# tranorrepository/cluster_tools

Measured on AMD Instinct MI355X. Metric: Gvoxels/s RAG+edge features (boundary map, uint64 labels, float32), higher is better.
Workload: dtype u64 labels / f32 samples / f64 stats; 1 GPU; BASELINE configs[2]: 2048^3 boundary map, cell 16, z-slab sharded; edges=15831246, parallelism=z-slab x1, step=rag_features

## Files before the change

cluster_tools_amd/_lib.py:

```python
from __future__ import annotations

import ctypes
import os
import sys
import threading

_HERE = os.path.dirname(os.path.abspath(__file__))
LIB_PATH = os.environ.get('CTG_LIB') or os.path.join(_HERE, 'libctg.so')

CTG_OK = 0
CTG_MEM_HOST = 0
CTG_MEM_DEVICE = 1
CTG_DATA_NONE = 0
CTG_DATA_F32 = 1
CTG_DATA_U8 = 2
CTG_KEEP_STATS = 1
CTG_NO_ADJ_FILTER = 2
CTG_NO_NODES = 4
CTG_DEFER_STATS = 8
CTG_ERR_STALE = -5
CTG_ERR_MISSING = -6
CTG_ASSIGN_DENSE = 0
CTG_ASSIGN_SPARSE = 1
CTG_CC_GREATER = 0
CTG_CC_LESS = 1
CTG_CC_EQUAL = 2
CTG_EDT_SRC_NONZERO = 0
CTG_EDT_SRC_GREATER = 1
CTG_EDT_SRC_EQUAL = 2
CTG_EDT_TO_BACKGROUND = 1
CTG_EDT_2D = 2
CTG_EDT_OUT_D2 = 4
CTG_WS_2D = 1
CTG_MAX_CHANNELS = 24
CTG_N_FEATURES = 10
CTG_NBINS = 40
CTG_WIDE_RECORD_WORDS = 48
CTG_MORPH_COLS = 11
CTG_REGION_COLS = 5
CTG_REGION_SUMS = 0
CTG_REGION_FEATURES = 1
CTG_MGPU_SAMPLES = 1024
CTG_MGPU_ROW_WORDS = 28
CTG_MGPU_MAX_WORLD = 32
CTG_IO_N5 = 0
CTG_IO_ZARR_DOT = 1
CTG_IO_ZARR_SLASH = 2
CTG_IO_RAW = 0
CTG_IO_GZIP = 1
CTG_IO_ZLIB = 2
CTG_SORT_WORDS = 12
CTG_SORT_PATH_GROUP = 5

_lock = threading.Lock()
_lib = None

c_i64p = ctypes.POINTER(ctypes.c_int64)
c_i32p = ctypes.POINTER(ctypes.c_int32)
c_u64p = ctypes.POINTER(ctypes.c_uint64)
c_u32p = ctypes.POINTER(ctypes.c_uint32)
c_dblp = ctypes.POINTER(ctypes.c_double)
c_vp = ctypes.c_void_p

PROTOTYPES = {
    'ctg_version': (ctypes.c_int, []),
    'ctg_init': (ctypes.c_int, [ctypes.c_int]),
    'ctg_last_error': (ctypes.c_char_p, []),
    'ctg_device_count': (ctypes.c_int, [ctypes.POINTER(ctypes.c_int)]),
    'ctg_rag_features': (ctypes.c_int, [c_vp, ctypes.c_int, c_vp, ctypes.c_int, ctypes.c_int, c_vp,
                                        c_vp, c_vp, c_vp, ctypes.c_int, ctypes.c_double, ctypes.c_double,
                                        ctypes.c_int, ctypes.c_int, c_vp, ctypes.POINTER(c_vp)]),
    'ctg_rag_blocks': (ctypes.c_int, [c_vp, ctypes.c_int, c_vp, ctypes.c_int, ctypes.c_int, c_vp, c_vp,
                                      ctypes.c_int, ctypes.c_int64, ctypes.c_int64, ctypes.c_int, ctypes.c_double,
                                      ctypes.c_double, ctypes.c_int, ctypes.c_int, c_vp, ctypes.POINTER(c_vp)]),
    'ctg_result_num_blocks': (ctypes.c_int, [c_vp]),
    'ctg_result_block_offsets': (ctypes.c_int, [c_vp, c_vp, c_vp]),
    'ctg_host_alloc': (c_vp, [ctypes.c_int64]),
    'ctg_host_free': (None, [c_vp]),
    'ctg_unique_labels': (ctypes.c_int, [c_vp, c_vp, c_vp, c_vp, ctypes.c_int, c_vp, ctypes.POINTER(c_vp)]),
    'ctg_merge_stats': (ctypes.c_int, [c_vp, c_vp, c_vp, ctypes.c_int64, ctypes.c_double, ctypes.c_double,
                                       ctypes.c_int, ctypes.c_int, c_vp, ctypes.POINTER(c_vp)]),
    'ctg_mgpu_slab': (ctypes.c_int, [ctypes.c_int64, ctypes.c_int, ctypes.c_int, c_vp, ctypes.c_int, c_vp]),
    'ctg_mgpu_sample': (ctypes.c_int, [c_vp, c_vp, c_vp]),
    'ctg_mgpu_split': (ctypes.c_int, [c_vp, c_vp, ctypes.c_int, c_vp, c_vp]),
    'ctg_mgpu_pack': (ctypes.c_int, [c_vp, c_vp, ctypes.c_int, ctypes.c_int, c_vp, c_vp]),
    'ctg_mgpu_merge': (ctypes.c_int, [c_vp, c_vp, c_vp, ctypes.c_int, ctypes.c_int, ctypes.c_double,
                                      ctypes.c_double, c_vp, ctypes.POINTER(c_vp)]),
    'ctg_merge_feature_rows': (ctypes.c_int, [c_vp, c_vp, ctypes.c_int64, ctypes.c_int64, ctypes.c_int64, c_vp,
                                              ctypes.c_int, c_vp]),
    'ctg_unique_pairs': (ctypes.c_int, [c_vp, ctypes.c_int64, ctypes.c_int, c_vp, ctypes.POINTER(c_vp)]),
    'ctg_unique_values': (ctypes.c_int, [c_vp, ctypes.c_int64, ctypes.c_int, c_vp, ctypes.POINTER(c_vp)]),
    'ctg_label_overlaps': (ctypes.c_int, [c_vp, ctypes.c_int, c_vp, ctypes.c_int, c_vp, c_vp, c_vp, ctypes.c_int,
                                          ctypes.c_uint64, ctypes.c_int, c_vp, ctypes.POINTER(c_vp)]),
    'ctg_merge_overlaps': (ctypes.c_int, [c_vp, c_vp, ctypes.c_int64, ctypes.c_int, c_vp, ctypes.POINTER(c_vp)]),
    'ctg_max_overlaps': (ctypes.c_int, [c_vp, ctypes.c_uint64, ctypes.c_uint64, c_vp, c_vp, ctypes.c_int, c_vp]),
    'ctg_result_copy_counts': (ctypes.c_int, [c_vp, c_vp, ctypes.c_int]),
    'ctg_morphology': (ctypes.c_int, [c_vp, ctypes.c_int, c_vp, c_vp, c_vp, c_vp, ctypes.c_int, c_vp,
                                      ctypes.POINTER(c_vp)]),
    'ctg_merge_morphology': (ctypes.c_int, [c_vp, ctypes.c_int64, ctypes.c_int, c_vp, ctypes.POINTER(c_vp)]),
    'ctg_result_copy_moments': (ctypes.c_int, [c_vp, c_vp, ctypes.c_int]),
    'ctg_morphology_rows': (ctypes.c_int, [c_vp, ctypes.c_uint64, ctypes.c_uint64, c_vp, c_vp, ctypes.c_int, c_vp]),
    'ctg_region_features': (ctypes.c_int, [c_vp, ctypes.c_int, c_vp, ctypes.c_int, c_vp, c_vp, c_vp, ctypes.c_int,
                                           ctypes.c_uint64, ctypes.c_int, c_vp, ctypes.POINTER(c_vp)]),
    'ctg_merge_region_features': (ctypes.c_int, [c_vp, ctypes.c_int64, ctypes.c_int, c_vp, ctypes.POINTER(c_vp)]),
    'ctg_region_rows': (ctypes.c_int, [c_vp, ctypes.c_uint64, ctypes.c_uint64, ctypes.c_int, ctypes.c_double, c_vp,
                                       c_vp, ctypes.c_int, c_vp]),
    'ctg_result_copy_region': (ctypes.c_int, [c_vp, c_vp, c_vp, c_vp, ctypes.c_int]),
    'ctg_assignment_dense': (ctypes.c_int, [c_vp, ctypes.c_int64, ctypes.c_int, c_vp, ctypes.POINTER(c_vp)]),
    'ctg_assignment_sparse': (ctypes.c_int, [c_vp, c_vp, ctypes.c_int64, ctypes.c_int, c_vp, ctypes.POINTER(c_vp)]),
    'ctg_assignment_info': (ctypes.c_int, [c_vp, c_i64p, c_u64p, ctypes.POINTER(ctypes.c_int)]),
    'ctg_assignment_free': (None, [c_vp]),
    'ctg_apply_assignment': (ctypes.c_int, [c_vp, c_vp, ctypes.c_int, ctypes.c_int64, c_vp, c_vp, ctypes.c_int64,
                                            ctypes.c_int, c_vp, c_vp, c_vp, ctypes.c_int, c_vp]),
    'ctg_threshold_components': (ctypes.c_int, [c_vp, ctypes.c_int, c_vp, c_vp, c_vp, c_vp, ctypes.c_float,
                                                ctypes.c_int, ctypes.c_int, ctypes.c_int, c_vp, ctypes.c_int, c_vp,
                                                c_u64p]),
    'ctg_merge_assignments': (ctypes.c_int, [c_vp, ctypes.c_int64, ctypes.c_uint64, c_vp, ctypes.c_int, c_vp, c_u64p]),
    'ctg_distance_transform': (ctypes.c_int, [c_vp, ctypes.c_int, ctypes.c_int, c_vp, c_vp, c_vp, ctypes.c_double,
                                              ctypes.c_uint64, c_vp, ctypes.c_int, c_vp, ctypes.c_int, c_vp, c_vp]),
    'ctg_seeded_watershed': (ctypes.c_int, [c_vp, c_vp, ctypes.c_int, c_vp, c_vp, c_vp, ctypes.c_int, ctypes.c_uint64,
                                            c_vp, ctypes.c_int, c_vp, c_vp]),
    'ctg_map_edge_ids': (ctypes.c_int, [c_vp, ctypes.c_int64, c_vp, ctypes.c_int64, c_vp, ctypes.c_int, c_vp]),
    'ctg_result_num_edges': (ctypes.c_int64, [c_vp]),
    'ctg_result_num_nodes': (ctypes.c_int64, [c_vp]),
    'ctg_result_copy_edges': (ctypes.c_int, [c_vp, c_vp, ctypes.c_int]),
    'ctg_result_copy_nodes': (ctypes.c_int, [c_vp, c_vp, ctypes.c_int]),
    'ctg_result_copy_features': (ctypes.c_int, [c_vp, c_vp, ctypes.c_int]),
    'ctg_result_copy_stats': (ctypes.c_int, [c_vp, c_vp, c_vp, ctypes.c_int]),
    'ctg_result_device_edges': (c_vp, [c_vp]),
    'ctg_result_device_features': (c_vp, [c_vp]),
    'ctg_result_info': (ctypes.c_int, [c_vp, c_i64p, c_i64p]),
    'ctg_free': (None, [c_vp]),
    'ctg_synth_volume': (ctypes.c_int, [c_vp, c_vp, c_vp, ctypes.c_int64, c_vp, ctypes.c_int, ctypes.c_uint64,
                                        ctypes.c_uint64, ctypes.c_double, c_vp]),
    'ctg_synth_affinities': (ctypes.c_int, [c_vp, c_vp, c_vp, ctypes.c_int, c_vp, c_vp]),
    'ctg_filter_conv_axis': (ctypes.c_int, [c_vp, c_vp, c_vp, ctypes.c_int, ctypes.c_int, c_vp, ctypes.c_int, c_vp]),
    'ctg_filter_combine': (ctypes.c_int, [ctypes.c_int, c_vp, c_vp, c_vp, c_vp, ctypes.c_int64, c_vp]),
    'ctg_sym_eigenvalues': (ctypes.c_int, [c_vp, ctypes.c_int, ctypes.c_int64, c_vp, c_vp]),
    'ctg_trim': (ctypes.c_int, []),
    'ctg_io_read_box': (ctypes.c_int, [ctypes.c_char_p, ctypes.c_int, ctypes.c_int, ctypes.c_int, ctypes.c_int,
                                       c_vp, c_vp, ctypes.c_int, c_vp, c_vp, c_vp, ctypes.c_int, c_vp]),
    'ctg_io_read_varlen': (ctypes.c_int, [ctypes.c_char_p, ctypes.c_int, ctypes.c_int, ctypes.c_int64, c_vp,
                                          ctypes.c_int, c_vp, c_vp, ctypes.c_int]),
    'ctg_io_free': (None, [c_vp]),
    'ctg_io_cache_clear': (None, []),
    'ctg_io_cache_stats': (None, [ctypes.c_void_p]),
    'ctg_io_cache_drop': (None, [ctypes.c_char_p]),
    'ctg_io_write_chunks': (ctypes.c_int, [ctypes.c_char_p, ctypes.c_int, ctypes.c_int, ctypes.c_int, ctypes.c_int,
                                           ctypes.c_int64, c_vp, c_vp, c_vp, c_vp, ctypes.c_int, ctypes.c_int,
                                           ctypes.c_int, ctypes.c_int]),
    'ctg_set_profiling': (ctypes.c_int, [ctypes.c_int]),
    'ctg_last_timings': (ctypes.c_int, [c_dblp, ctypes.c_int]),
    'ctg_last_sort': (ctypes.c_int, [c_i64p, ctypes.c_int]),
    'ctg_diag_bounds': (ctypes.c_int, [c_vp]),
}


class BlockDesc(ctypes.Structure):
    _fields_ = [('label_offset', ctypes.c_int64), ('data_offset', ctypes.c_int64),
                ('shape', ctypes.c_int64 * 3), ('own_begin', ctypes.c_int64 * 3), ('own_end', ctypes.c_int64 * 3),
                ('graph_begin', ctypes.c_int64 * 3), ('graph_end', ctypes.c_int64 * 3)]


class CtgError(RuntimeError):
    """Raised for every non-zero ctg status (pybind11 raises RuntimeError for
    nifty's C++ exceptions; cluster_tasks.py:114-159 treats both as a failed
    job)."""


def load():
    global _lib
    with _lock:
        if _lib is not None:
            return _lib
        if not os.path.exists(LIB_PATH):
            raise CtgError(
                "libctg.so not found at %s: build it with `python -c 'import __graft_entry__ as g; g.build()'` "
                "or `make -C cluster_tools_amd/csrc` (the HIP path has no CPU fallback)" % LIB_PATH)
        lib = ctypes.CDLL(LIB_PATH)
        for name, (res, args) in PROTOTYPES.items():
            if os.environ.get('CTG_LIB') and not hasattr(lib, name):
                continue
            fn = getattr(lib, name)
            fn.restype = res
            fn.argtypes = args
        _lib = lib
        return lib


def check(rc, what=''):
    if rc != CTG_OK:
        msg = load().ctg_last_error()
        msg = msg.decode() if msg else 'unknown error'
        raise CtgError('%s failed (status %d): %s' % (what or 'ctg call', rc, msg))


_inited = set()


def init_device(device=None):
    lib = load()
    if device is None:
        torch = sys.modules.get('torch')
        if torch is not None and torch.cuda.is_initialized():
            device = torch.cuda.current_device()
        else:
            device = int(os.environ.get('CTG_DEVICE', '0'))
    check(lib.ctg_init(int(device)), 'ctg_init(%d)' % device)
    _inited.add(int(device))
    return int(device)
```

cluster_tools_amd/csrc/ctg_api.hip:

```cpp
#include <hip/hip_runtime.h>
#include <cstdlib>
#include <cstring>
#include <rocprim/device/device_radix_sort.hpp>
#include <rocprim/device/device_select.hpp>

#include <algorithm>
#include <cstdio>

#include "ctg_api.h"

namespace ctg {

static thread_local std::string g_err;
void set_error(const std::string& msg) { g_err = msg; }

ResultPtr new_result(int device) {
    ResultPtr r(new ctg_result());
    r->device = device;
    return r;
}

ResultPtr empty_result(int device) {
    ResultPtr r = new_result(device);
    r->edges = (uint64_t*)dev_alloc(16);
// ... 42 lines not shown
    DevBuf<uint64_t> sorted(std::max<int64_t>(n, 1) * 8);
    if (!sorted) return hipErrorOutOfMemory;
    hipError_t e = with_temp(w.temp, [&](void* t, size_t& tb) {
        return rocprim::radix_sort_keys(t, tb, in, (uint64_t*)sorted, (size_t)n, 0u, end_bit, s);
    });
    if (e != hipSuccess) return e;
    return with_temp(w.temp, [&](void* t, size_t& tb) {
        return rocprim::unique(t, tb, (uint64_t*)sorted, out, count_dev, (size_t)n, rocprim::equal_to<uint64_t>(), s);
    });
}

int read_word(Workspace& w, SmallSlot i, hipStream_t s, int64_t* v) {
    CTG_CHECK(hipMemcpyAsync(w.small_host + i, w.small + i, 4, hipMemcpyDeviceToHost, s));
    CTG_CHECK(hipStreamSynchronize(s));
    *v = w.small_host[i];
    return CTG_OK;
}

int read_phase_times(Workspace& w, hipStream_t s) {
    CTG_CHECK(hipStreamSynchronize(s));
    float ms = 0.f;
    for (int i = 0; i < 6; ++i) {
        hipEventElapsedTime(&ms, w.ev[i], w.ev[i + 1]);
        w.last_ms[i] = ms;
    }
    hipEventElapsedTime(&ms, w.ev[0], w.ev[6]);
    w.last_ms[6] = ms;
    return CTG_OK;
}

hipError_t map_back(const ctg_result* U, ctg_result* r, hipStream_t s) {
    hipError_t e = launch_gather_labels(U->nodes, r->edges, 2 * r->n_edges, s);
    if (e == hipSuccess) e = launch_gather_labels(U->nodes, r->nodes, r->n_nodes, s);
    return e;
}

}

using namespace ctg;

static int reduce_pairs(ApiCall& c, ReduceJob& J, const uint64_t* dk, const char* who, ctg_result** out) {
    Workspace& w = c.w();
    hipStream_t s = c.s;
    DensePairs dp;
    StreamWait wait{s};
    CTG_CHECK(hipMemsetAsync(w.counters, 0, sizeof(Counters), s));
    CTG_CHECK(launch_max_pairs(J.n, dk, &w.counters->max_v, s));
    CTG_CHECK(hipMemcpyAsync(w.counters_host, w.counters, sizeof(Counters), hipMemcpyDeviceToHost, s));
    CTG_CHECK(hipStreamSynchronize(s));
    J.pairs = dk;
    J.max_v = w.counters_host->max_v;
    if (J.max_v >> 32) {
        const int rc = dp.build(dk, J.n, s);
        if (rc) return rc;
        J.pairs = dp.dense;
        J.max_v = (uint64_t)std::max<int64_t>(dp.U->n_nodes - 1, 0);
    }
    c.r = new_result(c.dev);
    hipError_t e = reduce_records(w, J, s, c.r.get());
    if (e == hipSuccess) e = dp.map_back(c.r.get(), s);
    if (e == hipSuccess) e = hipStreamSynchronize(s);
    const int rc = hip_status(e, who, CTG_ERR_HIP);
    if (rc) return rc;
    wait.disarm();
    return c.end(false, out);
}

extern "C" {

int ctg_version(void) { return 1; }

const char* ctg_last_error(void) { return g_err.c_str(); }

int ctg_device_count(int* count) {
    CTG_CHECK(hipGetDeviceCount(count));
    return CTG_OK;
}

int ctg_init(int device) {
    int n = 0;
    std::lock_guard<std::recursive_mutex> init_lock(device_mutex(device));
    CTG_CHECK(hipGetDeviceCount(&n));
    if (device < 0 || device >= n) {
        set_error("ctg_init: invalid device " + std::to_string(device));
        return CTG_ERR_ARG;
    }
    CTG_CHECK(hipSetDevice(device));
    CTG_CHECK(ws_init(ws(device)));
    return CTG_OK;
}

int ctg_diag_bounds(uint64_t* out) {
#ifdef CTG_DIAG
    if (!out) return CTG_ERR_ARG;
    CTG_CHECK(hipDeviceSynchronize());
    hipError_t (*take[8])(unsigned long long*) = {bounds_take_api,    bounds_take_scan, bounds_take_sort,
                                                   bounds_take_reduce, bounds_take_mgpu, bounds_take_overlap,
                                                   bounds_take_morph,  bounds_take_region};
    out[0] = out[1] = out[2] = out[3] = 0;
    int found = 0;
    for (int f = 0; f < 8; ++f) {
        unsigned long long h[3] = {0, 0, 0};
        CTG_CHECK(take[f](h));
        if (h[0] && !found) {
            out[0] = (uint64_t)f + 1;
            out[1] = h[0];
            out[2] = h[1];
            out[3] = h[2];
            found = 1;
        }
    }
    return found;
#else
    (void)out;
    set_error("ctg_diag_bounds: bounds checks exist only in CTG_DIAG builds (make variant EXTRA=-DCTG_DIAG)");
    return CTG_ERR_UNSUPPORTED;
#endif
}

int ctg_set_profiling(int on) {
    ws(current_device()).profiling = on;
    return CTG_OK;
}

int ctg_last_timings(double* ms, int n) {
    Workspace& w = ws(current_device());
    for (int i = 0; i < n && i < 8; ++i) ms[i] = w.last_ms[i];
    return CTG_OK;
}

int ctg_last_sort(int64_t* out, int n) {
    if (!out || n < 0) {
        set_error("ctg_last_sort: null argument");
        return CTG_ERR_ARG;
    }
    const SortReport& r = ws(current_device()).last_sort;
    int64_t v[CTG_SORT_WORDS];
    v[CTG_SORT_PATH] = r.path;
    v[CTG_SORT_PACKED] = r.packed;
    v[CTG_SORT_GROUP_TRIED] = r.group_tried;
    v[CTG_SORT_GROUP_DONE] = r.group_done;
    v[CTG_SORT_GROUP_WHY] = r.group_tried && !r.group_done ? (int)r.group.why : 0;
    v[CTG_SORT_GROUP_SHIFT] = r.group.shift;
    v[CTG_SORT_GROUP_BUCKETS] = r.group.nbk;
    v[CTG_SORT_GROUP_LARGEST] = r.largest;
    v[CTG_SORT_IB] = r.ib;
    v[CTG_SORT_NB] = r.nb;
    v[CTG_SORT_UB] = r.ub;
    v[CTG_SORT_N] = r.n;
    for (int i = 0; i < n && i < CTG_SORT_WORDS; ++i) out[i] = v[i];
    return CTG_OK;
}

int ctg_result_num_blocks(const ctg_result* r) { return r ? (int)std::max<size_t>(r->edge_off.size(), 1) - 1 : -1; }

int ctg_result_block_offsets(const ctg_result* r, int64_t* edge_off, int64_t* node_off) {
    if (!r || r->edge_off.empty()) {
        set_error("ctg_result_block_offsets: not a batched-blocks result");
        return CTG_ERR_ARG;
    }
    const size_t nb = r->edge_off.size();
    if (edge_off) std::memcpy(edge_off, r->edge_off.data(), nb * 8);
    if (node_off) {
        if (r->node_off.size() == nb) std::memcpy(node_off, r->node_off.data(), nb * 8);
        else std::memset(node_off, 0, nb * 8);
    }
    return CTG_OK;
}

int ctg_unique_labels(const uint64_t* labels, const int64_t* shape, const int64_t* begin, const int64_t* end,
                      int mem, void* stream, ctg_result** out) {
    ApiCall c;
    if (!labels || !shape || !out) {
        set_error("ctg_unique_labels: null argument");
        return CTG_ERR_ARG;
    }
    *out = nullptr;
    CallBox box;
    int rc = box_of("ctg_unique_labels", shape, begin, end, 0, &box);
    if (rc || (rc = c.begin(stream)) != CTG_OK) return rc;
    Workspace& w = c.w();
    hipStream_t s = c.s;
    const int64_t V = shape[0] * shape[1] * shape[2];
    const void* dl = nullptr;
    if ((rc = stage_in(w.stage[0], labels, (size_t)V * 8, mem, s, &dl)) != CTG_OK) return rc;
    if (box.voxels == 0) return c.empty(empty_result, out);
    c.r = new_result(c.dev);
    DevBuf<uint64_t> nodes;
    rc = unique_candidates(
        w, candidate_cap_first(box.voxels), box.voxels, 64u, s, "ctg_unique_labels: out of device memory",
        "ctg_unique_labels: candidate buffer overflow",
        [&](uint64_t* cand, unsigned long long* count, int64_t cap) {
            return launch_unique_tiles((const uint64_t*)dl, shape, box.b, box.e, cand, count, cap, s);
        },
        nodes, &c.r->n_nodes);
    if (rc) return rc;
    c.r->nodes = nodes.release();
    c.r->edges = (uint64_t*)dev_alloc(16);
    return c.end(false, out);
}

int ctg_unique_values(const uint64_t* values, int64_t n, int mem, void* stream, ctg_result** out) {
    ApiCall c;
    if (!out || n < 0 || (n > 0 && !values)) {
        set_error("ctg_unique_values: bad arguments");
        return CTG_ERR_ARG;
    }
    *out = nullptr;
    int rc = c.begin(stream);
    if (rc) return rc;
    if (n == 0) return c.empty(empty_result, out);
    Workspace& w = c.w();
    hipStream_t s = c.s;
    ResultPtr& r = c.r = new_result(c.dev);
    r->edges = (uint64_t*)dev_alloc(16);
    r->nodes = (uint64_t*)dev_alloc(n * 8);
    if (!r->nodes) {
        set_error("ctg_unique_values: out of device memory");
        return CTG_ERR_NOMEM;
    }
    DevInput<uint64_t> in;
    StreamWait wait{s};
    if ((rc = in.put(values, (size_t)n * 8, mem, s, "ctg_unique_values")) != CTG_OK) return rc;
    CTG_CHECK(sort_unique_u64(w, in, n, r->nodes, w.small + SLOT_NODES, s));
    if ((rc = read_word(w, SLOT_NODES, s, &r->n_nodes)) != CTG_OK) return rc;
    wait.disarm();
    return c.end(false, out);
}

int ctg_merge_stats(const uint64_t* keys, const double* sums, const uint32_t* records, int64_t n, double hist_lo,
                    double hist_hi, int keep_stats, int mem, void* stream, ctg_result** out) {
    ApiCall c;
    if (!out || n < 0 || (n > 0 && (!keys || !sums || !records))) {
        set_error("ctg_merge_stats: bad arguments");
        return CTG_ERR_ARG;
    }
    *out = nullptr;
    int rc = c.begin(stream);
    if (rc) return rc;
    if (n == 0) return c.empty(empty_result, out);
    hipStream_t s = c.s;
    DevInput<uint64_t> dk;
    DevInput<double> ds;
    DevInput<uint32_t> dr;
    StreamWait wait{s};
    rc = dk.put(keys, (size_t)n * 16, mem, s, "ctg_merge_stats");
    if (!rc) rc = ds.put(sums, (size_t)n * 16, mem, s, "ctg_merge_stats");
    if (!rc) rc = dr.put(records, (size_t)n * WREC_WORDS * 4, mem, s, "ctg_merge_stats");
    if (rc) return rc;
    ReduceJob J{};
    J.n = n;
    J.R.key = nullptr;
    J.R.sums = (double2*)ds.p;
    J.R.hist = (uint32_t*)dr.p;
    J.R.cap = n;
    J.wide = 1;
    J.stats = 1;
    J.need_adj = 1;
    J.ignore_label = 0;
    J.keep_stats = keep_stats;
    J.scale = (double)NBINS / (hist_hi - hist_lo);
    J.offset = hist_lo;
    if ((rc = reduce_pairs(c, J, dk, "ctg_merge_stats", out)) == CTG_OK) wait.disarm();
    return rc;
}

int ctg_merge_feature_rows(const uint64_t* ids, const double* rows, int64_t n, int64_t id_begin, int64_t id_end,
                           double* out, int mem, void* stream) {
    ApiCall c;
    if (n < 0 || id_end < id_begin || (n > 0 && (!ids || !rows)) || (id_end > id_begin && !out)) {
        set_error("ctg_merge_feature_rows: bad arguments");
        return CTG_ERR_ARG;
    }
    if (id_end - id_begin > 0xFFFFFFFFll || n > 0xFFFFFFFFll) {
        set_error("ctg_merge_feature_rows: more than 2^32 edges or rows in one call");
        return CTG_ERR_UNSUPPORTED;
    }
    const int64_t E = id_end - id_begin;
    if (E == 0) return CTG_OK;
    int rc = c.begin(stream);
    if (rc) return rc;
    Workspace& w = c.w();
    hipStream_t s = c.s;
    const bool host = mem == CTG_MEM_HOST;
    DevInput<uint64_t> di;
    DevInput<double> dr;
    DevBuf<double> own_o;
    StreamWait wait{s};
    double* dout = out;
    rc = di.put(ids, (size_t)n * 8, mem, s, "ctg_merge_feature_rows");
    if (!rc) rc = dr.put(rows, (size_t)n * N_FEATURES * 8, mem, s, "ctg_merge_feature_rows");
    if (rc) return rc;
    if (host && !(dout = own_o.alloc(E * N_FEATURES * 8))) {
        set_error("ctg_merge_feature_rows: out of device memory");
        return CTG_ERR_NOMEM;
    }
    CTG_CHECK(hipMemsetAsync(dout, 0, E * N_FEATURES * 8, s));
    if (n) {
        DevBuf<uint32_t> k_in(n * 4), k_out(n * 4), i_in(n * 4), i_out(n * 4);
        if (!k_in || !k_out || !i_in || !i_out) {
            set_error("ctg_merge_feature_rows: out of device memory");
            return CTG_ERR_NOMEM;
        }
        CTG_CHECK(hipMemsetAsync(w.small + SLOT_BAD_ID, 0, 4, s));
        CTG_CHECK(launch_row_keys(n, di, (uint64_t)id_begin, (uint64_t)id_end, k_in, i_in, w.small + SLOT_BAD_ID, s));
        const unsigned kb = (unsigned)bits_for((uint64_t)std::max<int64_t>(E - 1, 1));
// ... 198 lines not shown
```

cluster_tools_amd/csrc/ctg_api_scan.hip:

```cpp
#include <hip/hip_runtime.h>
#include <cstdio>
#include <cstdlib>
#include <cstring>

#include "ctg_api.h"

using namespace ctg;

struct ScanSwitches {
    int tile_z = 0;
    bool rec_fresh = false;
    int tile_z_narrow = 0;
    bool tail_tiles = true;
    int narrow_rows = -1;
    bool skip_adj = true;
    bool nn3 = true;
    int ablate = 0;
};

static ScanSwitches scan_switches(bool whole_array, bool boundary_map) {
    ScanSwitches sw;
    if (const char* t = getenv("CTG_TILE_Z")) sw.tile_z = std::max(1, atoi(t));
    sw.rec_fresh = getenv("CTG_REC_FRESH") != nullptr;
    if (!whole_array) return sw;
    if (const char* t = getenv("CTG_TILE_Z_NARROW")) sw.tile_z_narrow = std::max(1, atoi(t));
    if (const char* t = getenv("CTG_TAIL_TILES")) sw.tail_tiles = t[0] != '0';
    if (boundary_map)
        if (const char* t = getenv("CTG_NARROW_ROWS")) sw.narrow_rows = atoi(t) ? 1 : 0;
    if (const char* t = getenv("CTG_SKIP_ADJ")) sw.skip_adj = atoi(t) != 0;
    if (const char* t = getenv("CTG_NN3")) sw.nn3 = t[0] != '0';
#ifdef CTG_DIAG
    if (const char* t = getenv("CTG_ABLATE")) sw.ablate = atoi(t);
#endif
    return sw;
}

static int stage_volumes(Workspace& w, const void* labels, size_t lbytes, const void* data, size_t dbytes, int mem,
                         hipStream_t s, const void** dl, const void** dd) {
    const int rc = stage_in(w.stage[0], labels, lbytes, mem, s, dl);
    return rc ? rc : stage_in(w.stage[1], data, dbytes, mem, s, dd);
}

static ChannelClass scan_common(ScanParams& P, const void* dl, const void* dd, int label_bits, int data_kind,
                                int n_channels, const int32_t* offsets, double hist_lo, double hist_hi) {
    std::memset(&P, 0, sizeof(P));
    P.labels = dl;
    P.data = dd;
    P.label_bits = label_bits;
    P.data_kind = dd ? data_kind : CTG_DATA_NONE;
    P.n_channels = dd ? n_channels : 0;
    for (int c = 0; c < P.n_channels; ++c)
        for (int k = 0; k < 3; ++k) P.offsets[c][k] = offsets[3 * c + k];
    const ChannelClass cc = classify_channels(P.offsets, P.n_channels);
    P.lr_mask = cc.lr_mask;
    P.scale = (double)NBINS / (hist_hi - hist_lo);
    P.offset = hist_lo;
    P.fast40 = (hist_lo == 0.0 && P.scale == 40.0) ? 1 : 0;
    P.check_planes = 8;
    P.xcd_remap = 1;
    return cc;
}

static int scan_records(Workspace& w, const ScanParams& P, int64_t V, hipStream_t s, const ScanSwitches& sw, Ev& ev,
                        RegionPrefix& pre, bool* overflow, const char* who) {
    *overflow = false;
    if (sw.rec_fresh) {
        CTG_CHECK(hipStreamSynchronize(s));
        free_records(w);
    }
    int64_t need = record_slots_first(w.rec.cap, V);
#ifdef CTG_DIAG
    static const char* wg_path = getenv("CTG_WG_TIMES");
    ScanParams PW = P;
    size_t wg_n = 0;
    if (wg_path && !P.blocks) {
        const int64_t rows = std::min(scan_tile_rows(), scan_tile_rows_narrow());
        const int64_t tz = std::max(1, std::min(std::min(P.tile_z, P.tile_z_narrow > 0 ? P.tile_z_narrow : P.tile_z),
                                                std::max(8, P.tile_z / 4)));
        wg_n = (size_t)((P.shape[2] + 63) / 64) * (size_t)((P.shape[1] + rows - 1) / rows) *
               (size_t)((P.shape[0] + tz - 1) / tz);
        CTG_CHECK(hipMalloc(&PW.wg_times, wg_n * 16));
        CTG_CHECK(hipMemsetAsync(PW.wg_times, 0, wg_n * 16, s));
    }
#else
    const ScanParams& PW = P;
#endif
    for (int attempt = 0; attempt < 4; ++attempt) {
        CTG_CHECK(ensure_records(w, need, 0));
        CTG_CHECK(hipMemsetAsync(w.counters, 0, sizeof(Counters), s));
        ev.mark(0);
        CTG_CHECK(launch_face_scan(PW, w.rec, w.counters, s));
        ev.mark(1);
        CTG_CHECK(hipMemcpyAsync(w.counters_host, w.counters, sizeof(Counters), hipMemcpyDeviceToHost, s));
        CTG_CHECK(hipStreamSynchronize(s));
        if (w.counters_host->label_overflow) {
            *overflow = true;
            return CTG_OK;
        }
        const RegionFold f = fold_regions(w.counters_host->rcount);
        pre = f.pre;
        w.counters_host->n_records = f.total;
        if (f.total >= (1ull << 32)) {
            set_error(std::string(who) + ": more than 2^32 records");
            return CTG_ERR_NOMEM;
        }
        if ((int64_t)f.fullest <= w.rec.rcap) break;
        need = record_slots_regrow(f.fullest);
        if (attempt == 3) {
            set_error(std::string(who) + ": record buffer overflow");
            return CTG_ERR_NOMEM;
        }
    }
    if (P.ablate & 256)
        fprintf(stderr, "stamps total %llu fold %llu flush %llu wait %llu drain %llu floor %llu\n",
                w.counters_host->pad[2], w.counters_host->pad[3], w.counters_host->pad[4], w.counters_host->pad[5],
                w.counters_host->pad[7], w.counters_host->pad[0]);
#ifdef CTG_DIAG
    if (PW.wg_times) {
        std::vector<unsigned long long> h(wg_n * 2);
        CTG_CHECK(hipMemcpy(h.data(), PW.wg_times, wg_n * 16, hipMemcpyDeviceToHost));
        CTG_CHECK(hipFree(PW.wg_times));
        if (FILE* f = fopen(wg_path, "wb")) {
            fwrite(h.data(), 16, wg_n, f);
            fclose(f);
        }
        fprintf(stderr, "wg_times %s: %zu slots, flushes %llu, records %llu\n", wg_path, wg_n,
                w.counters_host->pad[6], w.counters_host->n_records);
    }
#endif
    w.last_records = (int64_t)w.counters_host->n_records;
    w.last_direct = (int64_t)w.counters_host->n_direct;
    return CTG_OK;
}

static ReduceJob scan_job(const Workspace& w, const ScanParams& P, const RegionPrefix& pre, bool scanned,
                          int ignore_label, int flags, ctg_result* r) {
    ReduceJob J{};
    J.n = r->n_records = scanned ? (int64_t)w.counters_host->n_records : 0;
    r->n_direct = scanned ? (int64_t)w.counters_host->n_direct : 0;
    J.keys = w.rec.key;
    J.regions = &pre;
    J.R = w.rec;
    J.stats = P.data_kind != CTG_DATA_NONE;
    J.ignore_label = ignore_label;
    J.keep_stats = (flags & CTG_KEEP_STATS) ? 1 : 0;
    J.max_v = scanned ? w.counters_host->max_v : 0;
    J.scale = P.scale;
    J.offset = P.offset;
    return J;
}

static int keep_zero_first(ctg_result* U, hipStream_t s) {
    uint64_t first = 0;
    if (U->n_nodes > 0) {
        CTG_CHECK(hipMemcpyAsync(&first, U->nodes, 8, hipMemcpyDeviceToHost, s));
        CTG_CHECK(hipStreamSynchronize(s));
    }
    if (U->n_nodes > 0 && first == 0) return CTG_OK;
    DevBuf<uint64_t> t((size_t)(U->n_nodes + 1) * 8);
    if (!t) {
        set_error("out of device memory for the dense relabelling table");
        return CTG_ERR_NOMEM;
    }
    CTG_CHECK(hipMemsetAsync(t, 0, 8, s));
    if (U->n_nodes)
        CTG_CHECK(hipMemcpyAsync(t + 1, U->nodes, (size_t)U->n_nodes * 8, hipMemcpyDeviceToDevice, s));
    dev_free(U->nodes);
    U->nodes = t.release();
    U->n_nodes += 1;
    return CTG_OK;
}

template <class Rerun>
static int rag_dense_relabel(const uint64_t* l64, int64_t n, const int64_t* shape, int ignore_label, int64_t limit,
                             const char* who, const char* limit_msg, void* stream, Rerun&& rerun, ctg_result** out) {
    hipStream_t s = (hipStream_t)stream;
    ResultPtr U, r;
    int rc = nested(U, [&](ctg_result** u) {
        return shape ? ctg_unique_labels(l64, shape, nullptr, nullptr, CTG_MEM_DEVICE, stream, u)
                     : ctg_unique_values(l64, n, CTG_MEM_DEVICE, stream, u);
    });
    if (rc) return rc;
    if (ignore_label && (rc = keep_zero_first(U.get(), s)) != CTG_OK) return rc;
    if (U->n_nodes > limit) {
        set_error(std::string(who) + limit_msg);
        return CTG_ERR_UNSUPPORTED;
    }
    DevBuf<uint32_t> dense(std::max<int64_t>(n, 1) * 4);
    if (!dense) {
        set_error(std::string(who) + ": out of device memory for the dense relabelling");
        return CTG_ERR_NOMEM;
    }
    CTG_CHECK(launch_remap_dense(l64, n, U->nodes, U->n_nodes, dense, s));
    rc = nested(r, [&](ctg_result** rr) { return rerun((const uint32_t*)dense, rr); });
    dense.reset();
    if (rc) return rc;
    CTG_CHECK(map_back(U.get(), r.get(), s));
    CTG_CHECK(hipStreamSynchronize(s));
    *out = r.release();
    return CTG_OK;
}

static int validate_features(const void* labels, int label_bits, const void* data, int data_kind, int n_channels,
                             const int32_t* offsets, const int64_t* shape, const int64_t* own_begin,
                             const int64_t* own_end, double hist_lo, double hist_hi, ctg_result** out) {
    const char* bad = nullptr;
    if (!out || !shape || !labels) {
        set_error("ctg_rag_features: null argument");
        return CTG_ERR_ARG;
    }
    *out = nullptr;
    if (label_bits != 32 && label_bits != 64) bad = "label_bits must be 32 or 64";
    else if (n_channels < 0 || n_channels > CTG_MAX_CHANNELS || (n_channels > 0 && !offsets))
        bad = "bad channel/offset arguments";
    else if (data && data_kind != CTG_DATA_F32 && data_kind != CTG_DATA_U8)
        bad = "data_kind must be CTG_DATA_F32 or CTG_DATA_U8";
    else if (!(hist_hi > hist_lo)) bad = "hist_hi must be > hist_lo";
    else
        for (int k = 0; k < 3; ++k)
            if (shape[k] < 0 || (own_begin && (own_begin[k] < 0)) || (own_end && own_end[k] < 0))
                bad = "negative shape/own_begin/own_end";
    if (!bad) return CTG_OK;
    set_error(std::string("ctg_rag_features: ") + bad);
    return CTG_ERR_ARG;
}

static void plan_whole_tiles(ScanParams& P, const int64_t* shape, const int64_t* own_begin, const int64_t* own_end,
                             const ScanSwitches& sw) {
    for (int k = 0; k < 3; ++k) {
        P.shape[k] = shape[k];
        P.own_begin[k] = own_begin ? own_begin[k] : 0;
        P.own_end[k] = own_end ? std::min(own_end[k], shape[k]) : shape[k];
    }
    const TileDepths td = scan_tile_depths(shape, scan_tile_rows(), scan_tile_rows_narrow());
    P.tile_z = td.tile_z;
    P.tile_z_narrow = td.tile_z_narrow;
    if (sw.tile_z) P.tile_z_narrow = P.tile_z = sw.tile_z;
    if (sw.tile_z_narrow) P.tile_z_narrow = sw.tile_z_narrow;
    P.ablate = sw.ablate;
    P.tail_tiles = sw.tail_tiles;
}

static int density_probe(Workspace& w, ScanParams& P, int mode, hipStream_t s) {
    P.narrow_rows = mode;
    if (mode != 2) return CTG_OK;
    P.density = w.small + SLOT_DENSITY;
    CTG_CHECK(hipMemsetAsync(w.small + SLOT_DENSITY, 0, 2 * sizeof(uint32_t), s));
    CTG_CHECK(launch_density(P.labels, P.label_bits, P.shape, 512, w.small + SLOT_DENSITY, s));
    return CTG_OK;
}

struct AdjFilter {
    hipStream_t s;
    ResultPtr graph;
    DevBuf<unsigned long long> bloom;
    StreamWait wait{s, false};
};

static int adjacency_filter(ScanParams& P, const int64_t* shape, const int64_t* own_begin, const int64_t* own_end,
                            double hist_lo, double hist_hi, void* stream, AdjFilter& f) {
    hipStream_t s = f.s;
    int rc = nested(f.graph, [&](ctg_result** g) {
        return ctg_rag_features(P.labels, P.label_bits, nullptr, CTG_DATA_NONE, 0, nullptr, shape, own_begin, own_end, 0,
                                hist_lo, hist_hi, 0, CTG_MEM_DEVICE, stream, g);
    });
    if (rc) return rc;
    const ctg_result* g = f.graph.get();
    uint64_t mx = 0;
    if (g->n_edges > 0) {
        CTG_CHECK(hipMemcpyAsync(&mx, g->nodes + g->n_nodes - 1, 8, hipMemcpyDeviceToHost, s));
        CTG_CHECK(hipStreamSynchronize(s));
    }
    if (mx >> 32) return CTG_OK;
    const uint32_t blocks = bloom_blocks(g->n_edges);
    if (!f.bloom.alloc((size_t)blocks * 64)) {
        set_error("ctg_rag_features: out of memory (adjacency filter)");
        return CTG_ERR_NOMEM;
    }
    f.wait.arm();
    if ((rc = hip_status(launch_build_bloom(g->edges, g->n_edges, f.bloom, blocks - 1, s), "ctg_rag_features",
                         CTG_ERR_HIP)) != CTG_OK)
        return rc;
    P.bloom = f.bloom;
    P.bloom_mask = blocks - 1;
    return CTG_OK;
}

static void plan_scan_channels(ScanParams& P, const ChannelClass& cc, int flags, const ScanSwitches& sw) {
    const ChannelPlan cp = plan_channels(cc, P.n_channels, !(flags & CTG_NO_ADJ_FILTER), P.bloom != nullptr,
                                         sw.skip_adj, sw.nn3);
    P.skip_adj_marks = cp.skip_adj_marks;
    P.nn3 = cp.nn3;
    P.nn_mix = cp.nn_mix;
    if (cp.nn3 || cp.nn_mix)
        for (int a = 0; a < 3; ++a) P.nn_ch[a] = cc.nn_ch[a];
    if (cp.nn_mix) {
        P.n_loop = cc.n_loop;
        for (int i = 0; i < cc.n_loop; ++i) P.loop_ch[i] = cc.loop_ch[i];
    }
}

static int64_t single_label_index(const ScanParams& P) {
    for (int k = 0; k < 3; ++k)
        if (P.own_begin[k] >= P.own_end[k]) return -1;
    return (P.own_begin[0] * P.shape[1] + P.own_begin[1]) * P.shape[2] + P.own_begin[2];
}
static hipError_t widen_single_label(const ScanParams& P, int64_t at, hipStream_t s, ctg_result* r) {
    if (P.label_bits != 32 || r->n_records != 0 || at < 0) return hipSuccess;
    uint32_t l32 = 0;
    hipError_t e = hipMemcpyAsync(&l32, (const uint32_t*)P.labels + at, 4, hipMemcpyDeviceToHost, s);
    if (e == hipSuccess) e = hipStreamSynchronize(s);
    const uint64_t l64 = l32;
    if (e == hipSuccess) e = hipMemcpyAsync(r->nodes, &l64, 8, hipMemcpyHostToDevice, s);
    if (e == hipSuccess) e = hipStreamSynchronize(s);
    r->n_nodes = 1;
    return e;
}

static int block_plan_error(const BlockPlan& plan) {
    const std::string block = "ctg_rag_blocks: block " + std::to_string(plan.bad_block);
    if (plan.error == BlockPlan::BOX_OUTSIDE) set_error(block + ": box outside its array");
    else if (plan.error == BlockPlan::ARRAY_OUTSIDE) set_error(block + ": array outside the arena");
    else set_error("ctg_rag_blocks: too many tiles in one call");
    return CTG_ERR_ARG;
}

struct BlockTables {
    hipStream_t s;
    DevBuf<BlockGeom> geom;
    DevBuf<uint32_t> prefix;
    StreamWait wait{s};
};

static int upload_block_tables(const BlockPlan& plan, int n_blocks, hipStream_t s, BlockTables& t, ScanParams& P) {
    P.tile_z = plan.tile_z;
    P.tag_shift = plan.tag_shift;
    P.label_hi_mask = plan.label_hi_mask;
    P.n_blocks = n_blocks;
    P.batch_tiles = plan.prefix[n_blocks];
    t.geom.alloc(sizeof(BlockGeom) * n_blocks);
    t.prefix.alloc((n_blocks + 1) * 4);
    if (!t.geom || !t.prefix) {
        set_error("ctg_rag_blocks: out of device memory");
        return CTG_ERR_NOMEM;
    }
    CTG_CHECK(hipMemcpyAsync(t.geom, plan.geom.data(), sizeof(BlockGeom) * n_blocks, hipMemcpyHostToDevice, s));
    CTG_CHECK(hipMemcpyAsync(t.prefix, plan.prefix.data(), (n_blocks + 1) * 4, hipMemcpyHostToDevice, s));
    P.blocks = t.geom;
    P.tile_prefix = t.prefix;
    return CTG_OK;
}

static hipError_t block_edge_offsets(const ScanParams& P, int tag_bits, uint64_t umask, hipStream_t s, ctg_result* r) {
    const int n_blocks = P.n_blocks;
    r->edge_off.assign(n_blocks + 1, 0);
    r->edge_off[n_blocks] = r->n_edges;
    if (!tag_bits || !r->n_edges) return hipSuccess;
    DevBuf<int64_t> bounds((n_blocks + 1) * 8);
    if (!bounds) return hipErrorOutOfMemory;
    CTG_TRY(launch_block_bounds(r->n_edges, r->edges, 2, n_blocks, P.tag_shift, bounds, s));
    CTG_TRY(hipMemcpyAsync(r->edge_off.data(), bounds, (n_blocks + 1) * 8, hipMemcpyDeviceToHost, s));
    CTG_TRY(launch_clear_bits(r->n_edges, r->edges, 2, umask, s));
    return hipStreamSynchronize(s);
}

static int block_nodes(Workspace& w, const ScanParams& P, const BlockPlan& plan, hipStream_t s, ctg_result* r) {
    const int n_blocks = P.n_blocks;
    const int64_t n_tiles = plan.uprefix.back();
    const char* nomem = "ctg_rag_blocks: out of device memory for the block nodes";
    DevBuf<uint32_t> dprefix((n_blocks + 1) * 4);
    DevBuf<int64_t> bounds((n_blocks + 1) * 8);
    if (!dprefix || !bounds) {
        set_error(nomem);
        return CTG_ERR_NOMEM;
    }
    CTG_CHECK(hipMemcpyAsync(dprefix, plan.uprefix.data(), (n_blocks + 1) * 4, hipMemcpyHostToDevice, s));
    DevBuf<uint64_t> nodes;
    int64_t N = 0;
    const int rc = unique_candidates(
        w, candidate_cap_first(plan.own_voxels), INT64_MAX, 32u + (unsigned)plan.tag_bits, s, nomem,
        "ctg_rag_blocks: node candidate buffer overflow",
        [&](uint64_t* cand, unsigned long long* count, int64_t cap) {
            return launch_unique_blocks(P.labels, P.label_bits, P.blocks, dprefix, n_blocks, n_tiles, cand, count, cap, s);
        },
        nodes, &N);
    if (rc) return rc;
    CTG_CHECK(launch_block_bounds(N, nodes, 1, n_blocks, 32, bounds, s));
    r->node_off.assign(n_blocks + 1, 0);
    CTG_CHECK(hipMemcpyAsync(r->node_off.data(), bounds, (n_blocks + 1) * 8, hipMemcpyDeviceToHost, s));
    CTG_CHECK(launch_clear_bits(N, nodes, 1, 0xFFFFFFFFull, s));
    CTG_CHECK(hipStreamSynchronize(s));
    dev_free(r->nodes);
    r->nodes = nodes.release();
    r->n_nodes = N;
    return CTG_OK;
}

static int features_dense_reentry(const void* dl, int label_bits, const void* dd, int data_kind, int n_channels,
                                  const int32_t* offsets, const int64_t* shape, const int64_t* own_begin,
                                  const int64_t* own_end, int ignore_label, double hist_lo, double hist_hi, int flags,
                                  void* stream, ctg_result** out) {
    if (label_bits != 64) {
        set_error("ctg_rag_features: internal label overflow on 32-bit labels");
        return CTG_ERR_HIP;
    }
    const int64_t V = shape[0] * shape[1] * shape[2];
    return rag_dense_relabel(
        (const uint64_t*)dl, V, shape, ignore_label, 0xFFFFFFFFll, "ctg_rag_features",
        ": more than 2^32 distinct labels in one array", stream,
        [&](const uint32_t* dense, ctg_result** r) {
            return ctg_rag_features(dense, 32, dd, data_kind, n_channels, offsets, shape, own_begin, own_end,
                                    ignore_label, hist_lo, hist_hi, flags, CTG_MEM_DEVICE, stream, r);
        },
        out);
}

static int blocks_dense_reentry(const void* dl, int label_bits, const void* dd, int data_kind, int n_channels,
                                const int32_t* offsets, const ctg_block_desc* blocks, int n_blocks,
                                int64_t labels_len, int64_t data_len, int ignore_label, double hist_lo,
                                double hist_hi, int flags, int tag_shift, void* stream, ctg_result** out) {
    hipStream_t s = (hipStream_t)stream;
    const uint64_t* l64 = (const uint64_t*)dl;
    DevBuf<uint64_t> wide;
    if (label_bits == 32) {
        if (!wide.alloc(std::max<int64_t>(labels_len, 1) * 8)) {
            set_error("ctg_rag_blocks: out of device memory widening the labels");
            return CTG_ERR_NOMEM;
        }
        CTG_CHECK(launch_u32_to_u64(labels_len, (const uint32_t*)dl, wide, s));
        l64 = wide;
    }
    return rag_dense_relabel(
        l64, labels_len, nullptr, ignore_label, (int64_t)(1ull << tag_shift), "ctg_rag_blocks",
        ": too many distinct labels for one batch of blocks: call with fewer blocks", stream,
        [&](const uint32_t* dense, ctg_result** r) {
            const int rc = ctg_rag_blocks(dense, 32, dd, data_kind, n_channels, offsets, blocks, n_blocks, labels_len,
                                          data_len, ignore_label, hist_lo, hist_hi, flags, CTG_MEM_DEVICE, stream, r);
            wide.reset();
            return rc;
        },
        out);
}

extern "C" {

int ctg_rag_features(const void* labels, int label_bits, const void* data, int data_kind, int n_channels,
                     const int32_t* offsets, const int64_t* shape, const int64_t* own_begin,
                     const int64_t* own_end, int ignore_label,
                     double hist_lo, double hist_hi, int flags, int mem, void* stream, ctg_result** out) {
    const char* who = "ctg_rag_features";
    ApiCall c;
    int rc = validate_features(labels, label_bits, data, data_kind, n_channels, offsets, shape, own_begin, own_end,
                               hist_lo, hist_hi, out);
    if (rc || (rc = c.begin(stream)) != CTG_OK) return rc;
    Workspace& w = c.w();
    hipStream_t s = c.s;
    const int64_t V = shape[0] * shape[1] * shape[2];
    const size_t dbytes = data ? (size_t)V * (n_channels > 0 ? n_channels : 1) * (data_kind == CTG_DATA_U8 ? 1 : 4) : 0;
    const void *dl = nullptr, *dd = nullptr;
    if ((rc = stage_volumes(w, labels, (size_t)V * (label_bits / 8), data, dbytes, mem, s, &dl, &dd)) != CTG_OK) return rc;
    const bool boundary_map = data && n_channels == 0;
    const ScanSwitches sw = scan_switches(true, boundary_map);

    ScanParams P;
    const ChannelClass cc = scan_common(P, dl, dd, label_bits, data_kind, n_channels, offsets, hist_lo, hist_hi);
    plan_whole_tiles(P, shape, own_begin, own_end, sw);
    if ((rc = density_probe(w, P, narrow_rows_mode(boundary_map, V, sw.narrow_rows), s)) != CTG_OK) return rc;
    AdjFilter adj{s};
    if (cc.long_range && !(flags & CTG_NO_ADJ_FILTER) && V > 0 &&
        (rc = adjacency_filter(P, shape, own_begin, own_end, hist_lo, hist_hi, stream, adj)) != CTG_OK)
        return rc;
    plan_scan_channels(P, cc, flags, sw);

    Ev ev{w, s};
    ev.mark(0);
    if (V == 0) return c.empty(empty_result, out);
    RegionPrefix pre{};
    bool overflow = false;
    if ((rc = scan_records(w, P, V, s, sw, ev, pre, &overflow, who)) != CTG_OK) return rc;
    if (overflow)
        return features_dense_reentry(dl, label_bits, dd, data_kind, n_channels, offsets, shape, own_begin, own_end,
                                      ignore_label, hist_lo, hist_hi, flags, stream, out);
    c.r = new_result(c.dev);
    ReduceJob J = scan_job(w, P, pre, true, ignore_label, flags, c.r.get());
    J.need_adj = need_adj_whole(P.n_channels, P.skip_adj_marks, !(flags & CTG_NO_ADJ_FILTER), P.bloom != nullptr);
    J.defer_stats = (flags & CTG_DEFER_STATS) ? 1 : 0;
    J.min_u = w.counters_host->max_nu ? (uint64_t)(uint32_t)~(uint32_t)w.counters_host->max_nu : 0;
    const int64_t single = single_label_index(P);
    J.single_label_ptr = label_bits == 64 && single >= 0 ? (const uint64_t*)dl + single : nullptr;
    hipError_t e = reduce_records(w, J, s, c.r.get());
    if (e == hipSuccess) e = widen_single_label(P, single, s, c.r.get());
    if ((rc = hip_status(e, who, CTG_ERR_HIP)) != CTG_OK) return rc;
    c.r->partial_adj = J.need_adj == 2 ? 1 : 0;
    return c.end(true, out);
}

int ctg_rag_blocks(const void* labels, int label_bits, const void* data, int data_kind, int n_channels,
                   const int32_t* offsets, const ctg_block_desc* blocks, int n_blocks, int64_t labels_len,
                   int64_t data_len, int ignore_label, double hist_lo, double hist_hi, int flags, int mem,
                   void* stream, ctg_result** out) {
    const char* who = "ctg_rag_blocks";
    ApiCall c;
    if (!out || !labels || !blocks || n_blocks < 1 || n_blocks > (1 << 20) || labels_len < 0 ||
        (label_bits != 32 && label_bits != 64) || (data && data_kind != CTG_DATA_F32 && data_kind != CTG_DATA_U8) ||
        n_channels < 0 || n_channels > CTG_MAX_CHANNELS || (n_channels > 0 && !offsets) || !(hist_hi > hist_lo)) {
        set_error("ctg_rag_blocks: bad arguments");
        return CTG_ERR_ARG;
    }
    *out = nullptr;
    const ScanSwitches sw = scan_switches(false, false);
    const BlockPlan plan = plan_blocks(blocks, n_blocks, data != nullptr, n_channels, labels_len, data_len,
                                       scan_max_x(), scan_tile_rows(), unique_tile_y(), sw.tile_z);
    if (plan.error == BlockPlan::BOX_OUTSIDE || plan.error == BlockPlan::ARRAY_OUTSIDE) return block_plan_error(plan);
    int rc = c.begin(stream);
    if (rc) return rc;
    Workspace& w = c.w();
    hipStream_t s = c.s;
    const void *dl = nullptr, *dd = nullptr;
    if ((rc = stage_volumes(w, labels, (size_t)labels_len * (label_bits / 8), data,
                            data ? (size_t)data_len * (data_kind == CTG_DATA_U8 ? 1 : 4) : 0, mem, s, &dl, &dd)) != CTG_OK)
        return rc;
    if (plan.error != BlockPlan::OK) return block_plan_error(plan);

    ScanParams P;
    scan_common(P, dl, dd, label_bits, data_kind, n_channels, offsets, hist_lo, hist_hi);
    BlockTables tables{s};
    if ((rc = upload_block_tables(plan, n_blocks, s, tables, P)) != CTG_OK) return rc;

    Ev ev{w, s};
    ev.mark(0);
    RegionPrefix pre{};
    bool overflow = false;
    const bool scanned = P.batch_tiles > 0;
    if (scanned && (rc = scan_records(w, P, plan.voxels, s, sw, ev, pre, &overflow, who)) != CTG_OK) return rc;
    if (overflow)
        return blocks_dense_reentry(dl, label_bits, dd, data_kind, n_channels, offsets, blocks, n_blocks, labels_len,
                                    data_len, ignore_label, hist_lo, hist_hi, flags, P.tag_shift, stream, out);
    c.r = new_result(c.dev);
    ctg_result* r = c.r.get();
    ReduceJob J = scan_job(w, P, pre, scanned, ignore_label, flags, r);
    J.need_adj = need_adj_blocks(P.n_channels);
    J.ub = plan.tag_bits ? 32 : 0;
    J.umask = plan.tag_bits ? (1ull << P.tag_shift) - 1ull : ~0ull;
    J.skip_nodes = 1;
    hipError_t e = reduce_records(w, J, s, r);
    if (e == hipSuccess) e = block_edge_offsets(P, plan.tag_bits, J.umask, s, r);
    if ((rc = hip_status(e, who, CTG_ERR_HIP)) != CTG_OK) return rc;
    if (flags & CTG_NO_NODES) r->node_off.assign(n_blocks + 1, 0);
    else if ((rc = block_nodes(w, P, plan, s, r)) != CTG_OK) return rc;
    return c.end(scanned, out);
}

}
```

cluster_tools_amd/csrc/ctg_internal.h:

```cpp
#pragma once
#include <hip/hip_runtime.h>
#include <cstdint>
#include <cstddef>
#include <memory>
#include <atomic>
#include <mutex>
#include <string>
#include <utility>
#include <vector>

#include "../../include/ctg.h"
#include "ctg_buffers.h"
#include "ctg_plan.h"

namespace ctg {

#ifdef CTG_DIAG
static __device__ unsigned long long ctg_oob[4];
__device__ __forceinline__ void oob_note(unsigned long long* d, uint64_t i, uint64_t n, int line) {
    if (i >= n && atomicCAS(d, 0ull, (unsigned long long)line) == 0ull) {
        d[1] = i;
        d[2] = n;
    }
}
#define CTG_IDX(i, n) ::ctg::oob_note(::ctg::ctg_oob, (uint64_t)(i), (uint64_t)(n), __LINE__)
#define CTG_BOUNDS_TAKE(tag)                                                      \
    hipError_t bounds_take_##tag(unsigned long long* h) {                       \
        hipError_t e_ = hipMemcpyFromSymbol(h, HIP_SYMBOL(ctg_oob), 24);          \
        if (e_ != hipSuccess || h[0] == 0) return e_;                             \
        const unsigned long long z_[4] = {0, 0, 0, 0};                            \
        return hipMemcpyToSymbol(HIP_SYMBOL(ctg_oob), z_, 32);                    \
    }
#else
#define CTG_IDX(i, n) ((void)0)
#define CTG_BOUNDS_TAKE(tag)
#endif

constexpr int WAVE = 64;
#ifndef CTG_SCAN_THREADS
#define CTG_SCAN_THREADS 512
#endif
constexpr int SCAN_THREADS = CTG_SCAN_THREADS;
constexpr int TILE_Y = 8;
#ifndef CTG_TABLE_CAP
#define CTG_TABLE_CAP SCAN_THREADS
#endif
constexpr int TABLE_CAP = CTG_TABLE_CAP;
static_assert(TABLE_CAP % 4 == 0 && TABLE_CAP <= SCAN_THREADS, "table capacity");
constexpr int NBINS = 40;
constexpr int NSLOTS = NBINS + 2;
constexpr int HWORDS = 21;
constexpr int NREC_WORDS = 24;
constexpr int NREC_STRIDE = 32;
constexpr int NREC_OFF = 4;
constexpr int NREC_PIV = 28;
constexpr int WREC_WORDS = 48;
constexpr int WREC_PIV = 45;
constexpr uint32_t PIV_EMPTY = 0xFFFFFFFFu;
constexpr uint32_t ADJ_FLAG = 0x80000000u;
constexpr uint64_t EMPTY_KEY = ~0ull;
constexpr int N_FEATURES = 10;
constexpr int64_t RECORD_LIMIT = 0xFFFFFFFFll;

__host__ __device__ inline uint32_t f2ord(float f) {
    uint32_t b;
    __builtin_memcpy(&b, &f, 4);
    return (b & 0x80000000u) ? ~b : (b | 0x80000000u);
}
__host__ __device__ inline float ord2f(uint32_t o) {
    uint32_t b = (o & 0x80000000u) ? (o & 0x7FFFFFFFu) : ~o;
    float f;
    __builtin_memcpy(&f, &b, 4);
    return f;
}
constexpr uint32_t ORD_POS_INF = 0xFF800000u;
constexpr uint32_t ORD_NEG_INF = 0x007FFFFFu;

__host__ __device__ inline int hist_slot(double x, double scale, double offset) {
    double m = scale * (x - offset);
    if (m == (double)NBINS) return NBINS;
    if (!(m < (double)NBINS)) return (m != m) ? 0 : NBINS + 1;
    if (m <= -1.0) return 0;
    return (int)m + 1;
}

__host__ __device__ inline uint32_t hash_key(uint64_t k) {
    k ^= k >> 33;
    k *= 0xff51afd7ed558ccdull;
    k ^= k >> 33;
    return (uint32_t)k;
}

#ifdef __HIPCC__
__device__ __forceinline__ uint64_t shfl_up_u64(uint64_t v) {
    const uint32_t lo = __shfl_up((uint32_t)v, 1, WAVE), hi = __shfl_up((uint32_t)(v >> 32), 1, WAVE);
    return ((uint64_t)hi << 32) | lo;
}
__device__ __forceinline__ uint64_t shfl_down_u64(uint64_t v, int o) {
    const uint32_t lo = __shfl_down((uint32_t)v, o, WAVE), hi = __shfl_down((uint32_t)(v >> 32), o, WAVE);
    return ((uint64_t)hi << 32) | lo;
}
__device__ __forceinline__ uint64_t bcast0_u64(uint64_t v) {
    const uint32_t lo = __shfl((uint32_t)v, 0, WAVE), hi = __shfl((uint32_t)(v >> 32), 0, WAVE);
    return ((uint64_t)hi << 32) | lo;
}
#endif

__host__ __device__ inline uint64_t bloom_hash(uint64_t k) {
    k ^= k >> 33;
    k *= 0xff51afd7ed558ccdull;
    k ^= k >> 29;
    k *= 0xc4ceb9fe1a85ec53ull;
    return k ^ (k >> 32);
}
__host__ __device__ inline uint64_t bloom_bits(uint64_t h) {
    return (1ull << (h & 63)) | (1ull << ((h >> 6) & 63)) | (1ull << ((h >> 12) & 63)) | (1ull << ((h >> 18) & 63));
}
__host__ __device__ inline uint32_t bloom_block(uint32_t owner, uint32_t block_mask) {
    return ((uint32_t)(bloom_hash(owner) >> 24) & block_mask) * 8u;
}
__host__ __device__ inline uint32_t bloom_word(uint32_t block, uint64_t h) { return block + ((uint32_t)(h >> 40) & 7u); }

struct RecordBuf {
    uint64_t* key = nullptr;
    double2* sums = nullptr;
    uint32_t* hist = nullptr;
    int64_t cap = 0;
    int64_t rcap = 0;
};

struct ScanParams {
    const void* labels;
    const void* data;
    int label_bits;
    int data_kind;
    int n_channels;
    int offsets[CTG_MAX_CHANNELS][3];
    int64_t shape[3];
    int64_t own_begin[3];
    int64_t own_end[3];
    double scale, offset;
    double u8_scale;
    int tile_z;
    int tile_z_narrow;
    int check_planes;
    int fast40;
    int ablate;
    const unsigned long long* bloom;
    uint32_t bloom_mask;
    int64_t ntiles[3];
    int xcd_remap;
    int skip_adj_marks;
    int nn3;
    int nn_ch[3];
    int nn_mix;
    int n_loop;
    int loop_ch[CTG_MAX_CHANNELS];
    uint32_t lr_mask;
    int narrow_rows;
    const uint32_t* density;
    const BlockGeom* blocks;
    const uint32_t* tile_prefix;
    int n_blocks;
    int64_t batch_tiles;
    int tag_shift;
    uint32_t label_hi_mask;
    unsigned long long* wg_times;
    int tail_tiles;
    int64_t main_tiles;
    int tail_z0, tile_z_tail;
};

struct Counters {
    unsigned long long n_records;
    unsigned long long n_direct;
    unsigned long long label_overflow;
    unsigned long long max_v;
    unsigned long long max_nu;
    unsigned long long pad[8];
    unsigned long long rcount[NREG];
};

struct Perm {
    const uint32_t* p32;
    const uint64_t* p64;
    int ib;
    __device__ __forceinline__ uint32_t operator()(uint32_t r) const {
        return p64 ? (uint32_t)(p64[r] & ((1ull << ib) - 1ull)) : p32[r];
    }
};

struct DeferredStats {
    int on = 0;
    const uint32_t* offs = nullptr;
    const uint32_t* runs = nullptr;
    Perm perm{nullptr, nullptr, 0};
    const uint32_t* hist = nullptr;
    uint64_t gen = 0;
    int64_t n_runs = 0, n_rec = 0, rec_cap = 0;
};

struct ReduceOut {
    uint64_t* edges;
    double* feats;
    uint32_t* keep;
    uint32_t* wstats;
    double2* wsums;
    uint32_t* count_out;
    int ablate;
    int64_t n_rec;
};

constexpr int BK_SMALL_WORDS = 5 * 4096 + 16;
constexpr int GS_SMALL_WORDS = 5 * 65536 + 16;

enum SmallSlot : int {
    SLOT_RUNS = 0,
    SLOT_EDGES = 1,
    SLOT_NODES = 2,
    SLOT_BAD_ID = 3,
    SLOT_DENSITY = 4,
    SLOT_GROUP_SORT = 16,
    SLOT_MERGE = 20,
    SLOT_HEAVY = 40,
    SMALL_WORDS = 64
};
struct MergeCounts {
    uint32_t keys;
    uint32_t rows;
};
static_assert(SLOT_RUNS >= 0 && SLOT_RUNS + 1 <= SLOT_EDGES && SLOT_EDGES + 1 <= SLOT_NODES &&
                  SLOT_NODES + 1 <= SLOT_BAD_ID && SLOT_BAD_ID + 1 <= SLOT_DENSITY &&
                  SLOT_DENSITY + 2 <= SLOT_GROUP_SORT && SLOT_GROUP_SORT + 1 <= SLOT_MERGE &&
                  SLOT_MERGE + (int)(sizeof(MergeCounts) / 4) <= SLOT_HEAVY && SLOT_HEAVY + 1 <= SMALL_WORDS,
              "the scalar slots overlap or pass SMALL_WORDS");

struct Workspace {
    std::atomic<bool> ready{false};
    int device = -1;
    uint64_t gen = 1;
    RecordBuf rec;
    SortScratch sort;
    GrowBuf temp;
    Counters* counters = nullptr;
    Counters* counters_host = nullptr;
    unsigned int* small = nullptr;
    unsigned int* small_host = nullptr;
    uint32_t* bsort = nullptr;
    uint32_t* gsort = nullptr;
    uint64_t* mgpu_spl = nullptr;
    hipEvent_t mgpu_spl_ev = nullptr;
    GrowBuf stage[2];
    hipStream_t copy_stream = nullptr;
    hipEvent_t ev[7] = {};
    double last_ms[8] = {0};
    int64_t last_records = 0, last_direct = 0;
    SortReport last_sort;
    int profiling = 0;
};

Workspace& ws(int device);
hipError_t ws_init(Workspace& w);
int current_device();
void set_error(const std::string& msg);
void free_records(Workspace& w);
hipError_t ensure_records(Workspace& w, int64_t need, int wide);

std::recursive_mutex& device_mutex(int device);
struct DevLock {
    std::lock_guard<std::recursive_mutex> g;
    DevLock() : g(device_mutex(current_device())) {}
};

template <class F>
hipError_t with_temp(GrowBuf& temp, F&& call) {
    size_t bytes = 0;
    hipError_t e = call(nullptr, bytes);
    if (e != hipSuccess) return e;
    if (!temp.reserve(bytes + 256)) return hipErrorOutOfMemory;
    bytes = temp.bytes;
    return call(temp.p, bytes);
}

struct Ev {
    Workspace& w;
    hipStream_t s;
    void mark(int i) {
        if (w.profiling) hipEventRecord(w.ev[i], s);
    }
};

hipError_t launch_face_scan(const ScanParams& P, const RecordBuf& R, Counters* C, hipStream_t s);
int64_t scan_max_x();
int scan_tile_rows();
int scan_tile_rows_narrow();
hipError_t launch_density(const void* L, int label_bits, const int64_t* shape, int n_rows, uint32_t* out,
                          hipStream_t s);
hipError_t launch_unique_tiles(const uint64_t* L, const int64_t* shape, const int64_t* b, const int64_t* e,
                               uint64_t* out, unsigned long long* count, int64_t cap, hipStream_t s);
hipError_t launch_unique_blocks(const void* L, int label_bits, const BlockGeom* blocks, const uint32_t* tile_prefix,
                                int n_blocks, int64_t n_tiles, uint64_t* out, unsigned long long* count, int64_t cap,
                                hipStream_t s);
int unique_tile_y();
hipError_t bucket_sort_keys(const uint64_t* keys, uint64_t* tmp, uint64_t* out, int64_t n, int lo_bit, int hi_bit,
                            uint64_t kmin, uint64_t kmax, uint32_t* small, GrowBuf& temp, uint32_t* nbk_out,
                            hipStream_t s);
hipError_t bucket_runs(const uint64_t* sorted, int64_t n, int lo_bit, uint32_t nbk, uint32_t* small, uint64_t* uniq,
                       uint32_t* runs, uint32_t* roffs, uint32_t* dE, hipStream_t s);
hipError_t bucket_sort_pairs(const uint64_t* keys, const uint32_t* vals, uint64_t* ktmp, uint32_t* vtmp,
                             uint64_t* kout, uint32_t* vout, int64_t n, int hi_bit, uint32_t* small, GrowBuf& temp,
                             uint32_t* nbk_out, hipStream_t s);
hipError_t group_sort_runs(const uint64_t* key, int64_t rcap, const RegionPrefix& pre, int64_t n, int nb, int ub,
                           int ib, uint64_t min_label, uint64_t max_label, uint32_t* small, uint32_t* host_word,
                           uint64_t* items, uint32_t* perm, uint64_t* uniq, uint32_t* runs, uint32_t* roffs,
                           uint32_t* dE, bool* done, SortReport* rep, hipStream_t s);
hipError_t launch_pack_keys(int64_t n, const uint64_t* key, int nb, uint64_t* sk, uint32_t* idx, hipStream_t s);
hipError_t launch_pack_regions(const uint64_t* key, int64_t rcap, const RegionPrefix& pre, int nb, int ib, uint64_t* sk,
                               uint32_t* idx, hipStream_t s);
hipError_t launch_pack_pairs(int64_t n, const uint64_t* uv, int nb, uint64_t* sk, uint32_t* idx, hipStream_t s);
hipError_t launch_max_pairs(int64_t n, const uint64_t* uv, unsigned long long* out, hipStream_t s);
hipError_t launch_reduce(int64_t E, const uint32_t* dE, const uint64_t* uniq, const uint32_t* runs,
                         const uint32_t* offs, const uint32_t* perm32, const uint64_t* perm64, int ib,
                         const RecordBuf& R, int wide, int stats, int nb, uint64_t umask, int need_adj,
                         int ignore_label, double scale, double offset, const ReduceOut& O, hipStream_t s,
                         uint32_t* heavy = nullptr, uint32_t* n_heavy = nullptr);
hipError_t launch_block_bounds(int64_t n, const uint64_t* col, int stride, int n_blocks, int shift, int64_t* bounds,
                               hipStream_t s);
hipError_t launch_clear_bits(int64_t n, uint64_t* col, int stride, uint64_t mask, hipStream_t s);
hipError_t launch_compact(int64_t E, const uint32_t* dE, const uint32_t* keep, const uint32_t* pos,
                          const ReduceOut& in, const ReduceOut& out, uint32_t* dkept, hipStream_t s);
hipError_t launch_endpoints(int64_t E, const uint64_t* uniq, int nb, uint32_t* out, hipStream_t s);
hipError_t launch_u32_to_u64(int64_t n, const uint32_t* in, uint64_t* out, hipStream_t s);
hipError_t launch_mark_nodes(int64_t E, const uint32_t* dE, const uint64_t* uniq, int nb, uint32_t* bits,
                             int64_t W, uint32_t wbase, hipStream_t s);
hipError_t launch_bits_to_nodes(int64_t W, const uint32_t* bits, const uint32_t* off, uint64_t* nodes, uint32_t* dN,
                                int64_t cap, uint32_t wbase, hipStream_t s);
hipError_t launch_build_bloom(const uint64_t* edges, int64_t E, unsigned long long* words, uint32_t mask,
                              hipStream_t s);
hipError_t launch_find_edges(const uint64_t* ge, int64_t n, const uint64_t* q, int64_t m, int64_t* out,
                             hipStream_t s);
hipError_t launch_remap_dense(const uint64_t* L, int64_t V, const uint64_t* U, int64_t n, uint32_t* out,
                              hipStream_t s);
hipError_t launch_gather_labels(const uint64_t* U, uint64_t* x, int64_t n, hipStream_t s);
hipError_t launch_remap_dense64(const uint64_t* L, int64_t V, const uint64_t* U, int64_t n, uint64_t* out,
                                hipStream_t s);
hipError_t launch_row_keys(int64_t n, const uint64_t* ids, uint64_t begin, uint64_t end, uint32_t* key,
                           uint32_t* idx, uint32_t* bad, hipStream_t s);
hipError_t launch_merge_feature_rows(int64_t n, const uint32_t* key, const uint32_t* idx, const double* rows,
                                     double* out, hipStream_t s);
hipError_t launch_synth(uint64_t* labels, float* boundary, const int64_t* shape, int64_t z_offset,
                        const int64_t* gshape, int cell, uint64_t seed, uint64_t label_offset, double noise_amp,
                        hipStream_t s);
hipError_t launch_synth_aff(const float* b, float* out, const int64_t* shape, int n_channels, const int32_t* off,
                            hipStream_t s);
#ifdef CTG_DIAG
hipError_t bounds_take_api(unsigned long long* h);
hipError_t bounds_take_reduce(unsigned long long* h);
hipError_t bounds_take_sort(unsigned long long* h);
hipError_t bounds_take_mgpu(unsigned long long* h);
hipError_t bounds_take_scan(unsigned long long* h);
hipError_t bounds_take_overlap(unsigned long long* h);
hipError_t bounds_take_morph(unsigned long long* h);
hipError_t bounds_take_region(unsigned long long* h);
#endif

}

struct ctg_result {
    int device = -1;
    std::vector<int64_t> edge_off, node_off;
    int64_t n_edges = 0;
    int64_t n_nodes = 0;
    uint64_t* edges = nullptr;
    uint64_t* nodes = nullptr;
    double* features = nullptr;
    uint32_t* stats = nullptr;
    double2* stat_sums = nullptr;
    uint64_t* counts = nullptr;
    int64_t* row_off = nullptr;
    uint64_t* moments = nullptr;
    uint64_t* reg_count = nullptr;
    double* reg_sum = nullptr;
    float* reg_minmax = nullptr;
    int64_t n_records = 0;
    int64_t n_direct = 0;
    int partial_adj = 0;
    ctg::DeferredStats defer;
    std::vector<void*> owned;
};

struct ctg_assignment {
    int device = -1;
    int kind = CTG_ASSIGN_DENSE;
    int64_t n = 0;
    uint64_t max_value = 0;
    uint64_t* table = nullptr;
    uint64_t size = 0;
};

namespace ctg {

struct ResultFree {
    void operator()(ctg_result* r) const { ctg_free(r); }
};
using ResultPtr = std::unique_ptr<ctg_result, ResultFree>;
ResultPtr new_result(int device);
ResultPtr empty_result(int device);

struct ReduceJob {
    int64_t n;
    const uint64_t* keys;
    const uint64_t* pairs;
    RecordBuf R;
    int wide, stats, need_adj, ignore_label, keep_stats;
    uint64_t max_v;
    uint64_t min_u = 0;
    double scale, offset;
    const uint64_t* single_label_ptr;
    const RegionPrefix* regions;
    int ub = 0;
    uint64_t umask = ~0ull;
    int skip_nodes = 0;
    int defer_stats = 0;
};
hipError_t reduce_records(Workspace& w, const ReduceJob& J, hipStream_t s, ctg_result* res);

hipError_t overlap_tables(Workspace& w, const void* A, int abits, const void* B, int bbits, const int64_t* shape,
                          const int64_t* b, const int64_t* e, int with_ignore, uint64_t ignore, hipStream_t s,
                          ctg_result* r, unsigned* overflow);
hipError_t overlap_reduce(Workspace& w, const uint64_t* key, const uint64_t* cnt, int64_t n, hipStream_t s,
                          ctg_result* r);
template <typename ValueT>
hipError_t sort_and_number(Workspace& w, const uint64_t* key, const ValueT* val, int64_t n, unsigned end_bit,
                           hipStream_t s, uint64_t* ks, ValueT* vs, uint64_t* scan, uint64_t* last);
hipError_t launch_overlap_pack(int64_t n, const uint64_t* pairs, uint64_t* key, hipStream_t s);
hipError_t launch_overlap_map_back(int64_t E, uint64_t* pairs, const uint64_t* Ua, int64_t na, const uint64_t* Ub,
                                   int64_t nb, hipStream_t s);
hipError_t launch_overlap_find(const uint64_t* U, int64_t n, uint64_t x, uint32_t* out, hipStream_t s);
hipError_t launch_overlap_argmax(const ctg_result* r, uint64_t lb, uint64_t le, uint64_t* out_l, uint64_t* out_c,
                                 hipStream_t s);

constexpr int MORPH_WORDS = 10;
hipError_t morph_tables(Workspace& w, const void* A, int bits, const int64_t* shape, const int64_t* b,
                        const int64_t* e, const int64_t* origin, hipStream_t s, ctg_result* r, unsigned* overflow);
hipError_t morph_merge(Workspace& w, const double* rows, int64_t n, hipStream_t s, ctg_result* r, int* bad);
// ... 155 lines not shown
```

cluster_tools_amd/csrc/ctg_plan.h:

```cpp
#pragma once
#include <algorithm>
#include <cstdint>
#include <cstdlib>
#include <vector>

#include "../../include/ctg.h"

#ifndef CTG_HD
#ifdef __HIPCC__
#define CTG_HD __host__ __device__
#else
#define CTG_HD
#endif
#endif

namespace ctg {

constexpr int TILE_X = 64;

inline int bits_for(uint64_t v) {
    int b = 1;
    while (b < 64 && (v >> b)) ++b;
    return b;
}
inline int bits_u(int64_t v) { return v <= 0 ? 0 : bits_for((uint64_t)v); }

struct CallBox {
    enum Error { OK, OUTSIDE, TOO_LARGE } error;
    int64_t b[3], e[3];
    int64_t voxels;
};

inline CallBox call_box(const int64_t* shape, const int64_t* begin, const int64_t* end, int64_t max_voxels) {
    CallBox c{};
    for (int k = 0; k < 3; ++k) {
        c.b[k] = begin ? begin[k] : 0;
        c.e[k] = end ? end[k] : shape[k];
        if (shape[k] < 0 || c.b[k] < 0 || c.e[k] > shape[k] || c.b[k] > c.e[k]) {
            c.error = CallBox::OUTSIDE;
            return c;
        }
    }
    c.voxels = (c.e[0] - c.b[0]) * (c.e[1] - c.b[1]) * (c.e[2] - c.b[2]);
    c.error = max_voxels > 0 && c.voxels >= max_voxels ? CallBox::TOO_LARGE : CallBox::OK;
    return c;
}

struct VolBox {
    int64_t s_z, s_y;
    int64_t base;
    uint32_t n[3];
};

inline VolBox vol_box(const int64_t* shape, const CallBox& c) {
    VolBox v{};
    v.s_z = shape[1] * shape[2];
    v.s_y = shape[2];
    v.base = c.b[0] * v.s_z + c.b[1] * v.s_y + c.b[2];
    for (int k = 0; k < 3; ++k) v.n[k] = (uint32_t)(c.e[k] - c.b[k]);
    return v;
}

struct TileDepths {
    int tile_z;
    int tile_z_narrow;
};

inline TileDepths scan_tile_depths(const int64_t* shape, int64_t rows_wide, int64_t rows_narrow) {
    constexpr int NARROW_TILE_Z = 16;
    const int64_t cols = ((shape[2] + TILE_X - 1) / TILE_X) * ((shape[1] + rows_wide - 1) / rows_wide);
    int tz = cols * ((shape[0] + 63) / 64) >= 32768 ? 64 : 32;
    if (cols * ((shape[0] + 127) / 128) >= 6144) tz = 128;
    while (tz > 8 && cols * ((shape[0] + tz - 1) / tz) < 1024) tz /= 2;
    const int64_t cols_n = ((shape[2] + TILE_X - 1) / TILE_X) * ((shape[1] + rows_narrow - 1) / rows_narrow);
    int tzn = std::min(tz, NARROW_TILE_Z);
    while (tzn < tz && cols_n * ((shape[0] + tzn - 1) / tzn) > 65536) tzn *= 2;
    return {tz, tzn};
}

inline int narrow_rows_mode(bool boundary_map, int64_t V, int nr_switch) {
    if (!boundary_map || (V < (1ll << 28) && nr_switch < 0)) return 0;
    return nr_switch < 0 ? 2 : (nr_switch ? 1 : 0);
}

struct BlockGeom {
    int64_t label_offset;
    int64_t data_offset;
    int32_t shape[3];
    int32_t own_begin[3], own_end[3];
    int32_t graph_begin[3], graph_end[3];
    int32_t ntx, nty, ntz;
};

struct BlockPlan {
    enum Error { OK, BOX_OUTSIDE, ARRAY_OUTSIDE, TOO_MANY_TILES } error = OK;
    int bad_block = -1;
    int64_t own_voxels = 0, voxels = 0;
    int tile_z = 0;
    int tag_bits = 0, tag_shift = 32;
    uint32_t label_hi_mask = 0;
    std::vector<BlockGeom> geom;
    std::vector<uint32_t> prefix;
    std::vector<uint32_t> uprefix;
};

inline BlockPlan plan_blocks(const ctg_block_desc* blocks, int n_blocks, bool has_data, int n_channels,
                             int64_t labels_len, int64_t data_len, int64_t max_x, int scan_rows, int unique_rows,
                             int tile_z_switch) {
    BlockPlan p;
    const int nch = has_data ? std::max(1, n_channels) : 0;
    int64_t zmax = 1;
    for (int b = 0; b < n_blocks; ++b) {
        const ctg_block_desc& d = blocks[b];
        int64_t V = 1, ov = 1;
        p.bad_block = b;
        for (int k = 0; k < 3; ++k) {
            V *= d.shape[k];
            if (d.shape[k] < 0 || d.shape[k] > (k == 2 ? max_x : 0x7FFFFFFF) || d.own_begin[k] < 0 ||
                d.own_end[k] > d.shape[k] || d.graph_begin[k] < 0 || d.graph_end[k] > d.shape[k]) {
                p.error = BlockPlan::BOX_OUTSIDE;
                return p;
            }
        }
        if (d.label_offset < 0 || d.label_offset + V > labels_len ||
            (has_data && (d.data_offset < 0 || d.data_offset + V * nch > data_len))) {
            p.error = BlockPlan::ARRAY_OUTSIDE;
            return p;
        }
        for (int k = 0; k < 3; ++k) ov *= std::max<int64_t>(0, d.own_end[k] - d.own_begin[k]);
        p.own_voxels += ov;
        p.voxels += V;
        zmax = std::max(zmax, d.shape[0]);
    }
    p.bad_block = -1;
    p.tile_z = tile_z_switch > 0 ? tile_z_switch : (int)std::min<int64_t>(zmax, 128);
    p.tag_bits = bits_u(n_blocks - 1);
    p.tag_shift = 32 - p.tag_bits;
    p.label_hi_mask = p.tag_bits ? ~((1u << p.tag_shift) - 1u) : 0u;
    p.geom.resize(n_blocks);
    p.prefix.assign(n_blocks + 1, 0);
    p.uprefix.assign(n_blocks + 1, 0);
    for (int b = 0; b < n_blocks; ++b) {
        const ctg_block_desc& d = blocks[b];
        BlockGeom& g = p.geom[b];
        g.label_offset = d.label_offset;
        g.data_offset = has_data ? d.data_offset : 0;
        int64_t oe[3];
        for (int k = 0; k < 3; ++k) {
            g.shape[k] = (int32_t)d.shape[k];
            g.own_begin[k] = (int32_t)d.own_begin[k];
            g.own_end[k] = (int32_t)d.own_end[k];
            g.graph_begin[k] = (int32_t)d.graph_begin[k];
            g.graph_end[k] = (int32_t)d.graph_end[k];
            oe[k] = std::max<int64_t>(0, d.own_end[k] - d.own_begin[k]);
        }
        g.ntx = (int32_t)((d.shape[2] + TILE_X - 1) / TILE_X);
        g.nty = (int32_t)((d.shape[1] + scan_rows - 1) / scan_rows);
        g.ntz = (int32_t)((d.shape[0] + p.tile_z - 1) / p.tile_z);
        const int64_t nt = (int64_t)g.ntx * g.nty * g.ntz;
        const int64_t ut = ((oe[2] + 63) / 64) * ((oe[1] + unique_rows - 1) / unique_rows) * ((oe[0] + 15) / 16);
        if ((int64_t)p.prefix[b] + nt > 0x7FFFFFFFll || (int64_t)p.uprefix[b] + ut > 0x7FFFFFFFll) {
            p.error = BlockPlan::TOO_MANY_TILES;
            return p;
        }
        p.prefix[b + 1] = p.prefix[b] + (uint32_t)nt;
        p.uprefix[b + 1] = p.uprefix[b] + (uint32_t)ut;
    }
    return p;
}

constexpr int NREG = 64;

struct RegionPrefix {
    uint32_t off[NREG + 1];
};

inline int64_t record_slots_first(int64_t cap, int64_t V) {
    const int64_t need = std::max<int64_t>(cap, std::max<int64_t>(1 << 16, V / 24));
    return (need + NREG - 1) / NREG * NREG;
}
inline int64_t record_slots_regrow(uint64_t fullest) { return ((int64_t)(fullest * 5 / 4) + 1024) * NREG; }

struct RegionFold {
    RegionPrefix pre;
    uint64_t total, fullest;
};
inline RegionFold fold_regions(const unsigned long long* rcount) {
    RegionFold f{};
    for (int r = 0; r < NREG; ++r) {
        f.pre.off[r] = (uint32_t)f.total;
        f.total += rcount[r];
        f.fullest = std::max<uint64_t>(f.fullest, rcount[r]);
    }
    f.pre.off[NREG] = (uint32_t)f.total;
    return f;
}

inline int64_t candidate_cap_first(int64_t n) {
    return std::max<int64_t>(1, std::min<int64_t>(n, std::max<int64_t>(1 << 16, n / 8)));
}
inline int64_t candidate_cap_regrow(int64_t m, int64_t bound) { return std::min<int64_t>(bound, m + 1024); }

inline uint32_t bloom_blocks(int64_t n_edges) {
    const int64_t bits = n_edges * 48;
    uint32_t blocks = 128;
    while ((int64_t)blocks * 512 < bits) blocks *= 2;
    return blocks;
}

constexpr int64_t TAKE_CHUNK = 4096;

inline uint64_t take_capacity(int64_t n) {
    uint64_t cap = 64;
    while (cap < 2 * (uint64_t)std::max<int64_t>(n, 0)) cap *= 2;
    return cap;
}

inline int take_count_slots(int64_t n_seg) { return n_seg <= 4096 ? 64 : 1; }

struct TakeChunks {
    enum Error { OK, BAD_SEGMENTS, TOO_MANY_CHUNKS } error = OK;
    std::vector<uint32_t> prefix;
};

inline TakeChunks take_chunk_prefix(const int64_t* seg_begin, int64_t n_seg, int64_t n, int64_t chunk) {
    TakeChunks t;
    const int64_t whole[2] = {0, n};
    if (!seg_begin) {
        seg_begin = whole;
        n_seg = 1;
    }
    if (n_seg < 0 || n < 0 || (n_seg == 0 && n != 0) || (n_seg > 0 && (seg_begin[0] != 0 || seg_begin[n_seg] != n))) {
        t.error = TakeChunks::BAD_SEGMENTS;
        return t;
    }
    t.prefix.assign((size_t)n_seg + 1, 0);
// ... 392 lines not shown
```

cluster_tools_amd/csrc/ctg_scan.hip:

```cpp
#include <type_traits>

#include "ctg_stats.h"
#include "ctg_tile_table.h"

#ifndef CTG_ROWS
#define CTG_ROWS 4
#endif

namespace ctg {

enum { MODE_GRAPH = 0, MODE_BOUNDARY = 1, MODE_AFFINITY = 2, MODE_AFF_NN = 3, MODE_AFF_MIX = 4 };

constexpr bool raw_sites(int mode) { return mode != MODE_AFFINITY && mode != MODE_AFF_MIX; }

constexpr bool scalar_loads(int mode) { return raw_sites(mode); }
constexpr int64_t SCALAR_LOAD_SPAN = 0xFFFFFFFFll;

constexpr int ROWS_WIDE = CTG_ROWS;
#ifndef CTG_ROWS_NARROW
#define CTG_ROWS_NARROW 1
#endif
constexpr int ROWS_NARROW = CTG_ROWS_NARROW;
#ifndef CTG_AFF_ROWS
#define CTG_AFF_ROWS CTG_ROWS
// ... 495 lines not shown
#pragma unroll
    for (int i = 0; i < NPER; ++i) {
        mm[i] = make_uint2(ORD_POS_INF, ORD_NEG_INF);
        if (MODE != MODE_GRAPH && slot[i] >= 0)
            mm[i] = make_uint2(__hip_atomic_load(&T.w[slot[i]][22], __ATOMIC_RELAXED, __HIP_MEMORY_SCOPE_WORKGROUP),
                               __hip_atomic_load(&T.w[slot[i]][23], __ATOMIC_RELAXED, __HIP_MEMORY_SCOPE_WORKGROUP));
    }
#if CTG_PAIR_FOLD
    if constexpr ((MODE == MODE_BOUNDARY || MODE == MODE_AFF_NN) && !BATCH) {
        fold_grouped<MODE, FAST40, BATCH, StageT, NPER>(T, e, slot, pv, mm, lane, R, C, scale, offset, ablate);
        return;
    }
#endif
#pragma unroll
    for (int i = 0; i < NPER; ++i)
        if (slot[i] != -2)
            fold_stats<MODE, FAST40, BATCH, StageT>(T, e[i], slot[i], pv[i], mm[i], R, C, scale, offset, need,
                                                    ablate);
}

__device__ __forceinline__ uint64_t stamp_now() {
    uint64_t t;
    asm volatile("s_memtime %0\n\ts_waitcnt lgkmcnt(0)" : "=s"(t)::"memory");
    return t;
}

__device__ __forceinline__ uint32_t swap1(uint32_t v) {
    return (uint32_t)__builtin_amdgcn_update_dpp((int)v, (int)v, 0xB1, 0xf, 0xf, false);
}

__device__ __forceinline__ uint32_t shl1(uint32_t v, uint32_t edge) {
    return (uint32_t)__builtin_amdgcn_update_dpp((int)edge, (int)v, 0x130, 0xf, 0xf, false);
}

#define FLUSH_TABLE table_flush_waves

template <typename LabelT, typename DataT, int MODE, bool FAST40, bool BATCH, int ROWS>
#ifndef CTG_SCAN_MIN_WAVES
#define CTG_SCAN_MIN_WAVES 4
#endif
__global__ __launch_bounds__(SCAN_THREADS, CTG_SCAN_MIN_WAVES) void k_face_scan(ScanParams P, RecordBuf R, Counters* C) {
    constexpr bool BND = MODE == MODE_BOUNDARY;
    constexpr bool AFF = MODE == MODE_AFFINITY || MODE == MODE_AFF_MIX;
    constexpr bool NN3 = MODE == MODE_AFF_NN;
    constexpr bool MIX = MODE == MODE_AFF_MIX;
    constexpr bool NNF = NN3 || MIX;
    constexpr uint32_t NN_MARK = MIX ? MARK_ONE_ADJ : MARK_ONE;
    constexpr bool STATS = MODE != MODE_GRAPH;
    using StageT = typename std::conditional<STATS, uint4, uint2>::type;
    __shared__ Table T;
    constexpr int NP = (ROWS == ROWS_NARROW && ROWS_NARROW != ROWS_WIDE && MODE == MODE_BOUNDARY && !BATCH)
                           ? CTG_NPER_NARROW : NPER;
    constexpr int STAGE_CAP = WAVE * NP;
    __shared__ StageT stage_all[WAVES][STAGE_CAP];
    if constexpr (!BATCH) {
        if (P.narrow_rows == 2) {
            const bool narrow = (uint64_t)P.density[0] * 100u > (uint64_t)P.density[1] * 14u;
            if (narrow != (ROWS == ROWS_NARROW)) return;
        }
    }
    const int tid = threadIdx.x;
    const int lane = tid & (WAVE - 1);
    const int wave = __builtin_amdgcn_readfirstlane(tid >> 6);
    StageT* stage = stage_all[wave];
#ifdef CTG_DIAG
    const unsigned long long t_wg0 = P.wg_times ? __builtin_amdgcn_s_memrealtime() : 0ull;
#endif
    for (int e = tid; e < TABLE_CAP; e += SCAN_THREADS) entry_reset(T, e);
    if (tid == 0) {
        T.used = 0;
        T.ncompact = 0;
        T.maxv = 0;
        T.maxnu = 0;
        T.flush_req = 0;
        T.live = WAVES;
    }
    __syncthreads();

    uint32_t t;
    {
        const uint32_t nwg = gridDim.x, id = blockIdx.x;
        t = id;
        if (P.xcd_remap) {
            const uint32_t xcd = id % 8, j = id / 8;
            const uint32_t M = (uint32_t)min((int64_t)nwg, P.main_tiles);
            const uint32_t mq = M / 8, mr = M % 8, wq = nwg / 8, wr = nwg % 8;
            const uint32_t mx = mq + (xcd < mr ? 1u : 0u), mstart = xcd * mq + min(xcd, mr);
            t = j < mx ? mstart + j : M + (xcd * wq + min(xcd, wr) - mstart) + (j - mx);
        }
    }
    constexpr bool batch = BATCH;
    int Z, Y, X;
    int obz, oez, oby, oey, obx, oex;
    int gbz, gez, gby, gey, gbx, gex;
    uint32_t ntx, nty, tag = 0;
    int64_t l_off = 0, d_off = 0;
    if constexpr (BATCH) {
        int lo = 0, hi = P.n_blocks;
        while (hi - lo > 1) {
            const int mid = (lo + hi) >> 1;
            if (P.tile_prefix[mid] <= t) lo = mid;
            else hi = mid;
        }
        const BlockGeom& G = P.blocks[lo];
        t -= P.tile_prefix[lo];
        Z = G.shape[0]; Y = G.shape[1]; X = G.shape[2];
        obz = G.own_begin[0]; oez = G.own_end[0]; oby = G.own_begin[1]; oey = G.own_end[1];
        obx = G.own_begin[2]; oex = G.own_end[2];
        gbz = G.graph_begin[0]; gez = G.graph_end[0]; gby = G.graph_begin[1]; gey = G.graph_end[1];
        gbx = G.graph_begin[2]; gex = G.graph_end[2];
        ntx = (uint32_t)G.ntx;
        nty = (uint32_t)G.nty;
        l_off = G.label_offset;
        d_off = G.data_offset;
        tag = P.tag_shift < 32 ? (uint32_t)lo << P.tag_shift : 0u;
    } else {
        Z = (int)P.shape[0]; Y = (int)P.shape[1]; X = (int)P.shape[2];
        obz = (int)P.own_begin[0]; oez = (int)P.own_end[0];
        oby = (int)P.own_begin[1]; oey = (int)P.own_end[1];
        obx = (int)P.own_begin[2]; oex = (int)P.own_end[2];
        gbz = gez = gby = gey = gbx = gex = 0;
        ntx = (uint32_t)P.ntiles[0];
        nty = (uint32_t)P.ntiles[1];
    }
    const int64_t sz = (int64_t)Y * X;
    int tdepth = P.tile_z, zbase = 0, zlim = Z;
    if constexpr (!BATCH) {
        if ((int64_t)t >= P.main_tiles) {
            t -= (uint32_t)P.main_tiles;
            tdepth = P.tile_z_tail;
            zbase = P.tail_z0;
        } else {
            zlim = min(Z, P.tail_z0);
        }
    }
    const int tx = (int)(t % ntx);
    const int ty = (int)((t / ntx) % nty);
    const int tz = (int)(t / (ntx * nty));
    const int x0 = tx * TILE_X;
    const int x = x0 + lane;
    const int yw = ty * (ROWS * WAVES) + wave * ROWS;
    const int z0 = zbase + tz * tdepth;
    const int z1 = min(z0 + tdepth, zlim);
    const LabelT* L = (const LabelT*)P.labels + l_off;
    const DataT* D = (const DataT*)P.data + d_off;
    const double scale = P.scale, offset = P.offset;
#ifdef CTG_DIAG
    const int ablate = P.ablate;
#else
    constexpr int ablate = 0;
#endif
    const uint32_t hi_mask = BATCH ? P.label_hi_mask : 0u;
    const bool inx = x < X;
    const bool own_x_lo = x >= obx && x < oex;
    const bool lane_xf = inx && x + 1 < X && x + 1 >= obx && x + 1 < oex;
    const bool lane_yz = inx && own_x_lo;
    const bool g_x_lo = batch && inx && x >= gbx && x < gex;
    const bool glane_xf = g_x_lo && x + 1 < gex;
    const bool glane_yz = g_x_lo;
    const uint64_t m_xf = __builtin_amdgcn_ballot_w64(lane_xf), m_yz = __builtin_amdgcn_ballot_w64(lane_yz);
    const uint64_t m_gxf = __builtin_amdgcn_ballot_w64(glane_xf), m_gyz = __builtin_amdgcn_ballot_w64(glane_yz);
    uint32_t row_x = 0, row_y = 0, grow_x = 0, grow_y = 0;
#pragma unroll
    for (int r = 0; r < ROWS; ++r) {
        const int y = yw + r;
        if (y < Y && y >= oby && y < oey) row_x |= 1u << r;
        if (y + 1 < Y && y + 1 >= oby && y + 1 < oey) row_y |= 1u << r;
        if (batch && y < Y && y >= gby && y < gey) grow_x |= 1u << r;
        if (batch && y + 1 < gey && y >= gby) grow_y |= 1u << r;
    }
    if constexpr (scalar_loads(MODE)) {
        row_x = (uint32_t)__builtin_amdgcn_readfirstlane((int)row_x);
        row_y = (uint32_t)__builtin_amdgcn_readfirstlane((int)row_y);
        grow_x = (uint32_t)__builtin_amdgcn_readfirstlane((int)grow_x);
        grow_y = (uint32_t)__builtin_amdgcn_readfirstlane((int)grow_y);
    }
    const bool adj_marks = AFF && (batch || !P.skip_adj_marks);
    const int xh = x0 + TILE_X;

    uint32_t Lc[ROWS + 1];
    LabelT Ln[ROWS + 1];
    float Dc[ROWS + 1], Dn[ROWS + 1];
    float Dyc[ROWS + 1], Dyn[ROWS + 1], Dzn[ROWS];
    uint32_t XLc = 0;
    LabelT XLn = 0;
    float XDc = 0.f, XDn = 0.f;
    uint32_t ovf = 0;

    auto narrow = [&](LabelT l) -> uint32_t {
        if constexpr (sizeof(LabelT) == 8) ovf |= (uint32_t)(l >> 32);
        if constexpr (BATCH) ovf |= (uint32_t)l & hi_mask;
        return (uint32_t)l;
    };
    const int xcl = min(x, X - 1);
    const int xhc = min(xh, X - 1);
    const int64_t csz = (int64_t)Z * sz;
    const int ywc = min(yw, Y - 1);
    const int rmaxc = Y - 1 - ywc;
    const uint64_t lbase = scalar_loads(MODE) ? uniform64((uint64_t)(L + (int64_t)ywc * X)) : 0;
    const uint64_t dbase = scalar_loads(MODE) && (BND || NN3)
                               ? uniform64((uint64_t)(D + (NN3 ? (int64_t)P.nn_ch[2] * csz : 0) + (int64_t)ywc * X))
                               : 0;
    const uint64_t aybase = scalar_loads(MODE) && NN3 ? uniform64((uint64_t)(D + (int64_t)P.nn_ch[1] * csz + (int64_t)ywc * X)) : 0;
    const uint64_t azbase = scalar_loads(MODE) && NN3 ? uniform64((uint64_t)(D + (int64_t)P.nn_ch[0] * csz + (int64_t)ywc * X)) : 0;
    const uint32_t win = (uint32_t)__builtin_amdgcn_readfirstlane((min(ROWS, rmaxc) + 1) * X);
    const uint32_t xh_el = (uint32_t)(min(min(lane, ROWS - 1), rmaxc) * X + xhc);
    uint32_t rofs[ROWS + 1];
#pragma unroll
    for (int r = 0; r <= ROWS; ++r) rofs[r] = (uint32_t)__builtin_amdgcn_readfirstlane(min(r, rmaxc) * X);
    auto load_plane = [&](int z, LabelT (&Lb)[ROWS + 1], float (&Db)[ROWS + 1], LabelT& XL, float& XD,
                          float (&Dyb)[ROWS + 1], float (&Dzb)[ROWS], bool with_z) {
        if constexpr (scalar_loads(MODE)) {
            const uint64_t pz = (uint64_t)z * (uint64_t)sz;
            const BufRsrc Lr = buf_rsrc(lbase + pz * sizeof(LabelT), win * (uint32_t)sizeof(LabelT));
            const BufRsrc Dr = buf_rsrc(dbase + pz * sizeof(DataT), win * (uint32_t)sizeof(DataT));
            const uint32_t xl = (uint32_t)xcl * (uint32_t)sizeof(LabelT), xd = (uint32_t)xcl * (uint32_t)sizeof(DataT);
#pragma unroll
            for (int r = 0; r <= ROWS; ++r) {
                Lb[r] = buf_label<LabelT>(Lr, xl, rofs[r] * (uint32_t)sizeof(LabelT));
                if constexpr (BND || NN3) Db[r] = buf_val<DataT, false>(Dr, xd, rofs[r] * (uint32_t)sizeof(DataT));
                else Db[r] = 0.f;
            }
            if constexpr (NN3) {
                const BufRsrc Yr = buf_rsrc(aybase + pz * sizeof(DataT), win * (uint32_t)sizeof(DataT));
#pragma unroll
                for (int r = 1; r <= ROWS; ++r)
                    Dyb[r] = buf_val<DataT, true>(Yr, xd, rofs[r] * (uint32_t)sizeof(DataT));
                if (with_z) {
                    const BufRsrc Zr = buf_rsrc(azbase + pz * sizeof(DataT), win * (uint32_t)sizeof(DataT));
#pragma unroll
                    for (int r = 0; r < ROWS; ++r)
                        Dzb[r] = buf_val<DataT, true>(Zr, xd, rofs[r] * (uint32_t)sizeof(DataT));
                }
            }
            XL = buf_label<LabelT>(Lr, xh_el * (uint32_t)sizeof(LabelT), 0u);
            if constexpr (BND || NN3) XD = buf_val<DataT, false>(Dr, xh_el * (uint32_t)sizeof(DataT), 0u);
            else XD = 0.f;
            return;
        }
        const LabelT* Lz = L + (int64_t)z * sz + (int64_t)yw * X;
        const DataT* Dz = BND ? D + (int64_t)z * sz + (int64_t)yw * X
                              : NN3 ? D + (int64_t)P.nn_ch[2] * csz + (int64_t)z * sz + (int64_t)yw * X : nullptr;
        const int rmax = Y - 1 - yw;
#pragma unroll
        for (int r = 0; r <= ROWS; ++r) {
            const int rr = min(r, rmax);
            Lb[r] = Lz[(int64_t)rr * X + xcl];
            if constexpr (BND || NN3) Db[r] = load_val<DataT>(Dz, (int64_t)rr * X + xcl);
            else Db[r] = 0.f;
        }
        if constexpr (NN3) {
            const DataT* Ay = D + (int64_t)P.nn_ch[1] * csz + (int64_t)z * sz + (int64_t)yw * X;
            const DataT* Az = D + (int64_t)P.nn_ch[0] * csz + (int64_t)z * sz + (int64_t)yw * X;
#pragma unroll
            for (int r = 1; r <= ROWS; ++r) Dyb[r] = load_val_stream<DataT>(Ay, (int64_t)min(r, rmax) * X + xcl);
            if (with_z) {
#pragma unroll
                for (int r = 0; r < ROWS; ++r) Dzb[r] = load_val_stream<DataT>(Az, (int64_t)min(r, rmax) * X + xcl);
            }
        }
        const int hr = min(min(lane, ROWS - 1), rmax);
        XL = Lz[(int64_t)hr * X + xhc];
        if constexpr (BND || NN3) XD = load_val<DataT>(Dz, (int64_t)hr * X + xhc);
        else XD = 0.f;
    };

    bool need = false;
    int nbuf = 0;
    uint32_t wsamp = 0;
    const bool stamps = (ablate & 256) != 0;
    uint64_t t_fold = 0, t_flush = 0, t_wait = 0, t_drain = 0, t_floor = 0;
    const uint64_t t_start = stamps ? stamp_now() : 0;
    auto poll = [&]() {
        if (__ballot(need)) {
            if (lane == 0) atomicOr(&T.flush_req, 1u);
            need = false;
        }
        const uint32_t fr = (uint32_t)__builtin_amdgcn_readfirstlane(
            (int)__hip_atomic_load(&T.flush_req, __ATOMIC_RELAXED, __HIP_MEMORY_SCOPE_WORKGROUP));
        if (fr) {
            const uint64_t t0 = stamps ? stamp_now() : 0;
            FLUSH_TABLE<MODE>(T, R, C);
            wsamp = 0;
            if (stamps) t_flush += stamp_now() - t0;
        }
    };
    auto flush_stage = [&]() {
        if (nbuf) {
            if constexpr (STATS) {
                const uint32_t add = (BND || AFF) ? 2u * (uint32_t)nbuf : (uint32_t)nbuf;
                if (wsamp + add > WAVE_SAMPLE_BUDGET) {
                    need = true;
                    poll();
                }
                wsamp += add;
            }
            const uint64_t t0 = stamps ? stamp_now() : 0;
            fold_batch<MODE, FAST40, BATCH, StageT, NP>(T, stage, nbuf, lane, tag, R, C, scale, offset, need,
                                                        ablate);
            nbuf = 0;
            if (stamps) {
                uint64_t a, b, c, d;
                asm volatile("s_memtime %0\n\ts_waitcnt lgkmcnt(0)\n\ts_memtime %1\n\ts_waitcnt lgkmcnt(0)\n\t"
                             "s_memtime %2\n\ts_waitcnt lgkmcnt(0)\n\ts_memtime %3\n\ts_waitcnt lgkmcnt(0)"
                             : "=&s"(a), "=&s"(b), "=&s"(c), "=&s"(d)::"memory");
                t_drain += b - a;
                t_floor += d - c;
            }
            if (stamps) t_fold += stamp_now() - t0;
            poll();
        }
    };
    auto push_m = [&](uint64_t m, bool act, uint32_t a, uint32_t b, uint32_t za, uint32_t zb) {
        const int k = __popcll(m);
        if (nbuf + k > STAGE_CAP) flush_stage();
        const int rank = __builtin_amdgcn_mbcnt_hi((uint32_t)(m >> 32), __builtin_amdgcn_mbcnt_lo((uint32_t)m, 0));
        if (act) {
            const uint32_t u = raw_sites(MODE) ? a : (BATCH ? (min(a, b) | tag) : min(a, b));
            const uint32_t v = raw_sites(MODE) ? b : max(a, b);
            if constexpr (STATS) stage[nbuf + rank] = make_uint4(u, v, za, zb);
            else stage[nbuf + rank] = make_uint2(u, v);
        }
        nbuf += k;
    };
#define PUSH(cmp, lanes, member, ...)                                      \
    do {                                                                   \
        const bool c_ = (cmp);                                             \
        push_m(__builtin_amdgcn_ballot_w64(c_) & (lanes), c_ && (member), __VA_ARGS__); \
    } while (0)

    if (z0 < z1) {
        load_plane(z0, Ln, Dc, XLn, XDc, Dyc, Dzn, false);
#pragma unroll
        for (int r = 0; r <= ROWS; ++r) Lc[r] = narrow(Ln[r]);
        XLc = narrow(XLn);
    }
    __builtin_amdgcn_s_waitcnt(0x0F70);
    for (int z = z0; z < z1; ++z) {
        const bool hz = z + 1 < Z;
        load_plane(hz ? z + 1 : z, Ln, Dn, XLn, XDn, Dyn, Dzn, true);
        const bool zlo = z >= obz && z < oez;
        const bool zup = hz && z + 1 >= obz && z + 1 < oez;
        const bool zg = batch && z >= gbz && z < gez;
        const bool gzup = zg && z + 1 < gez;
        const uint32_t s_xo = (uint32_t)__builtin_amdgcn_readfirstlane((int)(zlo ? row_x : 0u));
        const uint32_t s_yo = (uint32_t)__builtin_amdgcn_readfirstlane((int)(zlo ? row_y : 0u));
        const uint32_t s_zo = (uint32_t)__builtin_amdgcn_readfirstlane((int)(zup ? row_x : 0u));
        const uint32_t s_xg = (uint32_t)__builtin_amdgcn_readfirstlane((int)(zg ? grow_x : 0u));
        const uint32_t s_yg = (uint32_t)__builtin_amdgcn_readfirstlane((int)(zg ? grow_y : 0u));
        const uint32_t s_zg = (uint32_t)__builtin_amdgcn_readfirstlane((int)(gzup ? grow_x : 0u));
        if constexpr (MIX) {
            const int rmax = Y - 1 - yw;
            const DataT* Ax = D + (int64_t)P.nn_ch[2] * csz + (int64_t)z * sz + (int64_t)yw * X;
            const DataT* Ay = D + (int64_t)P.nn_ch[1] * csz + (int64_t)z * sz + (int64_t)yw * X;
#pragma unroll
            for (int r = 0; r < ROWS; ++r) Dc[r] = load_val_stream<DataT>(Ax, (int64_t)min(r, rmax) * X + xcl);
            XDc = load_val<DataT>(Ax, (int64_t)min(min(lane, ROWS - 1), rmax) * X + xhc);
#pragma unroll
            for (int r = 1; r <= ROWS; ++r) Dyc[r] = load_val_stream<DataT>(Ay, (int64_t)min(r, rmax) * X + xcl);
        }
        if (ablate & 8) {
            uint32_t chk = 0;
#pragma unroll
            for (int r = 0; r < ROWS; ++r) chk ^= Lc[r] ^ (uint32_t)Ln[r] ^ __float_as_uint(Dc[r] + Dn[r]);
            if (chk == 0x9E3779B9u && XLc == 7u) atomicAdd(&C->pad[0], 1ull);
        } else {
#pragma unroll
            for (int r = 0; r < ROWS; ++r) {
                const uint32_t lc = Lc[r];
                const uint32_t lx = shl1(lc, (uint32_t)__builtin_amdgcn_readlane((int)XLc, r));
                const bool xo = (s_xo >> r) & 1u, xg = BATCH && ((s_xg >> r) & 1u);
                if ((xo || xg) && (!AFF || adj_marks || NNF)) {
                    const float dx = (BND || NNF) ? __uint_as_float(shl1(__float_as_uint(Dc[r]),
                                                                         (uint32_t)__builtin_amdgcn_readlane(
                                                                             (int)__float_as_uint(XDc), r)))
                                                  : 0.f;
                    const bool own = xo && lane_xf;
                    if constexpr (NNF) {
                        PUSH(lc != lx, m_xf, own, lc, lx, __float_as_uint(dx), NN_MARK);
                    } else {
                        PUSH(lc != lx, (xo ? m_xf : 0ull) | (xg ? m_gxf : 0ull), own || (xg && glane_xf), lc, lx,
                             (own || !BATCH) ? __float_as_uint(Dc[r]) : MARK_ADJ,
                             (AFF || (BATCH && !own)) ? MARK_ADJ : __float_as_uint(dx));
                    }
                }
                const bool yo = (s_yo >> r) & 1u, yg = BATCH && ((s_yg >> r) & 1u);
                if ((yo || yg) && (!AFF || adj_marks || NNF)) {
                    const bool own = yo && lane_yz;
                    if constexpr (NNF) {
                        PUSH(lc != Lc[r + 1], m_yz, own, lc, Lc[r + 1], __float_as_uint(Dyc[r + 1]), NN_MARK);
                    } else {
                        PUSH(lc != Lc[r + 1], (yo ? m_yz : 0ull) | (yg ? m_gyz : 0ull), own || (yg && glane_yz), lc,
                             Lc[r + 1],
                             (own || !BATCH) ? __float_as_uint(Dc[r]) : MARK_ADJ,
                             (AFF || (BATCH && !own)) ? MARK_ADJ : __float_as_uint(Dc[r + 1]));
                    }
                }
            }
            if constexpr (AFF) {
                if (zlo && row_x) {
                    const int64_t iz = (int64_t)z * sz + (int64_t)yw * X + x;
                    const int n_loop = MIX ? P.n_loop : P.n_channels;
                    for (int c0 = 0; c0 < n_loop; c0 += AFF_G) {
                        constexpr int K = AFF_G * ROWS;
                        uint32_t lq[K];
                        float av[K];
                        bool act[K];
#pragma unroll
                        for (int j = 0; j < AFF_G; ++j) {
                            const bool has = c0 + j < n_loop;
                            const int c = MIX ? (has ? P.loop_ch[c0 + j] : 0) : c0 + j;
                            const int qz = has ? z + P.offsets[c][0] : -1, oy = has ? P.offsets[c][1] : 0;
                            const int qx = has ? x + P.offsets[c][2] : -1;
                            const bool okzx = lane_yz && qz >= 0 && qz < Z && qx >= 0 && qx < X;
#pragma unroll
                            for (int r = 0; r < ROWS; ++r) {
                                const int k = j * ROWS + r;
                                const int qy = yw + r + oy;
                                act[k] = (row_x >> r & 1u) && okzx && qy >= 0 && qy < Y;
                                lq[k] = Lc[r];
                                av[k] = 0.f;
                                if (act[k]) {
                                    lq[k] = load_lo(L, (int64_t)qz * sz + (int64_t)qy * X + qx);
                                    av[k] = load_val_stream<DataT>(D, (int64_t)c * Z * sz + iz + (int64_t)r * X);
                                }
                            }
                        }
#pragma unroll
                        for (int k = 0; k < K; ++k) act[k] = act[k] && lq[k] != Lc[k % ROWS];
                        const uint32_t glr = MIX ? (1u << AFF_G) - 1u : (P.lr_mask >> c0) & ((1u << AFF_G) - 1u);
                        if (glr && P.bloom != nullptr && !(ablate & 512)) {
                            uint64_t hb[K];
                            unsigned long long wb[K];
                            uint32_t blk[ROWS];
#pragma unroll
                            for (int r = 0; r < ROWS; ++r) blk[r] = bloom_block(Lc[r], P.bloom_mask);
#pragma unroll
                            for (int k = 0; k < K; ++k) {
                                hb[k] = bloom_hash(((uint64_t)Lc[k % ROWS] << 32) | lq[k]);
                                wb[k] = (act[k] && (glr >> (k / ROWS) & 1u)) ? P.bloom[bloom_word(blk[k % ROWS], hb[k])]
                                                                             : ~0ull;
                            }
#pragma unroll
                            for (int k = 0; k < K; ++k)
                                act[k] = act[k] && (wb[k] & bloom_bits(hb[k])) == bloom_bits(hb[k]);
                        }
#pragma unroll
                        for (int j = 0; j < AFF_G; ++j) {
                            if (c0 + j >= n_loop) break;
                            const uint32_t mk = (P.bloom != nullptr && !(glr >> j & 1u)) ? MARK_ONE_ADJ : MARK_ONE;
                            if (mk == MARK_ONE && P.bloom != nullptr) {
#pragma unroll
                                for (int r = 0; r < ROWS; ++r) {
                                    const int k = j * ROWS + r;
                                    const uint32_t sv = __float_as_uint(av[k]);
                                    const uint32_t nq = swap1(lq[k]), ns = swap1(sv), nact = swap1(act[k] ? 1u : 0u);
                                    const bool pair = act[k] && nact && nq == lq[k] && ns < MARK_ONE_ADJ &&
                                                      sv < MARK_ONE_ADJ;
                                    const bool lead = (lane & 1) == 0;
                                    const bool same_c = swap1(Lc[r]) == Lc[r];
                                    const bool pr = pair && same_c;
                                    PUSH(act[k] && !(pr && !lead), ~0ull, true, Lc[r], lq[k], sv,
                                         (pr && lead) ? ns : MARK_ONE);
                                }
                            } else {
#pragma unroll
                                for (int r = 0; r < ROWS; ++r)
                                    PUSH(act[j * ROWS + r], ~0ull, true, Lc[r], lq[j * ROWS + r],
                                         __float_as_uint(av[j * ROWS + r]), mk);
                            }
                        }
                    }
                }
            }
            if constexpr (MIX) {
                const int rmax = Y - 1 - yw;
                const DataT* Az = D + (int64_t)P.nn_ch[0] * csz + (int64_t)(hz ? z + 1 : z) * sz + (int64_t)yw * X;
#pragma unroll
                for (int r = 0; r < ROWS; ++r) Dzn[r] = load_val_stream<DataT>(Az, (int64_t)min(r, rmax) * X + xcl);
            }
            if (stamps) {
                const uint64_t tw = stamp_now();
                __builtin_amdgcn_s_waitcnt(0x0F70);
                t_wait += stamp_now() - tw;
            }
            if ((s_zo | s_zg) && (!AFF || adj_marks || NNF)) {
#pragma unroll
                for (int r = 0; r < ROWS; ++r) {
                    const bool zo = (s_zo >> r) & 1u, zgr = BATCH && ((s_zg >> r) & 1u);
                    if (zo || zgr) {
                        const bool own = zo && lane_yz;
                        const uint32_t ln = (uint32_t)Ln[r];
                        if constexpr (NNF) {
                            PUSH(Lc[r] != ln, m_yz, own, Lc[r], ln, __float_as_uint(Dzn[r]), NN_MARK);
                        } else {
                            PUSH(Lc[r] != ln, (zo ? m_yz : 0ull) | (zgr ? m_gyz : 0ull), own || (zgr && glane_yz),
                                 Lc[r], ln, (own || !BATCH) ? __float_as_uint(Dc[r]) : MARK_ADJ,
                                 (AFF || (BATCH && !own)) ? MARK_ADJ : __float_as_uint(Dn[r]));
                        }
                    }
                }
            }
        }
        poll();
        __builtin_amdgcn_s_waitcnt(0x0F70);
#pragma unroll
        for (int r = 0; r <= ROWS; ++r) {
            Lc[r] = narrow(Ln[r]);
            Dc[r] = Dn[r];
            if constexpr (NN3) {
                if (r >= 1) Dyc[r] = Dyn[r];
            }
        }
        XLc = narrow(XLn);
        XDc = XDn;
    }
#undef PUSH
    if (__ballot(ovf != 0) && lane == 0) atomicAdd(&C->label_overflow, 1ull);
    flush_stage();
    poll();
    if (lane == 0) atomicSub(&T.live, 1u);
    while (true) {
        const uint32_t fr = (uint32_t)__builtin_amdgcn_readfirstlane(
            (int)__hip_atomic_load(&T.flush_req, __ATOMIC_RELAXED, __HIP_MEMORY_SCOPE_WORKGROUP));
        if (fr) {
            FLUSH_TABLE<MODE>(T, R, C);
            continue;
        }
        const uint32_t lv = (uint32_t)__builtin_amdgcn_readfirstlane(
            (int)__hip_atomic_load(&T.live, __ATOMIC_RELAXED, __HIP_MEMORY_SCOPE_WORKGROUP));
        if (lv == 0) break;
        __builtin_amdgcn_s_sleep(2);
    }
    FLUSH_TABLE<MODE>(T, R, C);
    if (tid == 0 && T.maxv) atomicMax(&C->max_v, T.maxv);
    if (tid == 0 && T.maxnu) atomicMax(&C->max_nu, T.maxnu);
#ifdef CTG_DIAG
    if (P.wg_times && tid == 0) {
        P.wg_times[2 * (size_t)blockIdx.x] = t_wg0;
        P.wg_times[2 * (size_t)blockIdx.x + 1] = __builtin_amdgcn_s_memrealtime();
    }
#endif
    if (stamps && lane == 0) {
        atomicAdd(&C->pad[2], (unsigned long long)(stamp_now() - t_start));
        atomicAdd(&C->pad[3], (unsigned long long)t_fold);
        atomicAdd(&C->pad[4], (unsigned long long)t_flush);
        atomicAdd(&C->pad[5], (unsigned long long)t_wait);
        atomicAdd(&C->pad[7], (unsigned long long)t_drain);
        atomicAdd(&C->pad[0], (unsigned long long)t_floor);
    }
}

template <typename LabelT, typename DataT, int MODE, int NR>
static hipError_t launch_scan_r(const ScanParams& P, const RecordBuf& R, Counters* C, hipStream_t s) {
    ScanParams Q = P;
    int64_t nwg = P.batch_tiles;
    if (!P.blocks) {
        if (NR == ROWS_NARROW && ROWS_NARROW != ROWS_WIDE && P.tile_z_narrow > 0) Q.tile_z = P.tile_z_narrow;
        Q.ntiles[0] = (P.shape[2] + TILE_X - 1) / TILE_X;
        Q.ntiles[1] = (P.shape[1] + NR * WAVES - 1) / (NR * WAVES);
        Q.ntiles[2] = (P.shape[0] + Q.tile_z - 1) / Q.tile_z;
        nwg = Q.ntiles[0] * Q.ntiles[1] * Q.ntiles[2];
        Q.main_tiles = nwg;
        Q.tail_z0 = (int)P.shape[0];
        Q.tile_z_tail = Q.tile_z;
        const int64_t layer = Q.ntiles[0] * Q.ntiles[1], nz = Q.ntiles[2];
        if (P.tail_tiles && nwg >= 1024 && Q.tile_z >= 16) {
            const int tzt = std::max(8, Q.tile_z / 4);
            int64_t tl = std::min<int64_t>((512 + layer - 1) / layer, nz / 4);
            if (tl < 1 && nz >= 2 && (P.shape[0] - (nz - 1) * Q.tile_z) * 4 <= Q.tile_z) tl = 1;
            if (tl >= 1) {
                const int64_t zt0 = (nz - tl) * Q.tile_z;
                Q.main_tiles = layer * (nz - tl);
                Q.tail_z0 = (int)zt0;
                Q.tile_z_tail = tzt;
                nwg = Q.main_tiles + layer * ((P.shape[0] - zt0 + tzt - 1) / tzt);
            }
        }
    } else {
        Q.main_tiles = nwg;
    }
    if (nwg <= 0) return hipSuccess;
    if (nwg > 0x7FFFFFFF) return hipErrorInvalidValue;
    if (scalar_loads(MODE) && !P.blocks && P.shape[2] > scan_max_x()) return hipErrorInvalidValue;
    dim3 grid((unsigned)nwg);
    constexpr unsigned pad = 0;
    if (P.blocks) {
        if (P.fast40)
            hipLaunchKernelGGL((k_face_scan<LabelT, DataT, MODE, true, true, NR>), grid, dim3(SCAN_THREADS), pad, s, Q,
                               R, C);
        else
            hipLaunchKernelGGL((k_face_scan<LabelT, DataT, MODE, false, true, NR>), grid, dim3(SCAN_THREADS), pad, s,
                               Q, R, C);
    } else if (P.fast40) {
        hipLaunchKernelGGL((k_face_scan<LabelT, DataT, MODE, true, false, NR>), grid, dim3(SCAN_THREADS), pad, s, Q,
                           R, C);
    } else {
        hipLaunchKernelGGL((k_face_scan<LabelT, DataT, MODE, false, false, NR>), grid, dim3(SCAN_THREADS), pad, s, Q,
                           R, C);
    }
    return hipGetLastError();
}

template <typename LabelT, typename DataT, int MODE>
static hipError_t launch_scan_t(const ScanParams& P, const RecordBuf& R, Counters* C, hipStream_t s) {
    if constexpr (MODE == MODE_BOUNDARY) {
        if (P.narrow_rows == 2 && !P.blocks) {
            const hipError_t e = launch_scan_r<LabelT, DataT, MODE, ROWS_WIDE>(P, R, C, s);
            return e != hipSuccess ? e : launch_scan_r<LabelT, DataT, MODE, ROWS_NARROW>(P, R, C, s);
        }
        if (P.narrow_rows == 1 && !P.blocks) return launch_scan_r<LabelT, DataT, MODE, ROWS_NARROW>(P, R, C, s);
    }
    if constexpr (MODE == MODE_AFFINITY || MODE == MODE_AFF_MIX)
        if (!P.blocks) return launch_scan_r<LabelT, DataT, MODE, ROWS_AFF>(P, R, C, s);
    return launch_scan_r<LabelT, DataT, MODE, ROWS_WIDE>(P, R, C, s);
}

template <typename LabelT>
static hipError_t launch_scan_l(const ScanParams& P, const RecordBuf& R, Counters* C, hipStream_t s) {
    if (P.data_kind == CTG_DATA_NONE || P.data == nullptr)
        return launch_scan_t<LabelT, float, MODE_GRAPH>(P, R, C, s);
    const bool aff = P.n_channels > 0;
    const bool nn3 = aff && P.nn3 && !P.blocks;
    const bool mix = aff && P.nn_mix && !P.blocks;
    if (P.data_kind == CTG_DATA_U8)
        return nn3 ? launch_scan_t<LabelT, uint8_t, MODE_AFF_NN>(P, R, C, s)
               : mix ? launch_scan_t<LabelT, uint8_t, MODE_AFF_MIX>(P, R, C, s)
               : aff ? launch_scan_t<LabelT, uint8_t, MODE_AFFINITY>(P, R, C, s)
                     : launch_scan_t<LabelT, uint8_t, MODE_BOUNDARY>(P, R, C, s);
    return nn3 ? launch_scan_t<LabelT, float, MODE_AFF_NN>(P, R, C, s)
           : mix ? launch_scan_t<LabelT, float, MODE_AFF_MIX>(P, R, C, s)
           : aff ? launch_scan_t<LabelT, float, MODE_AFFINITY>(P, R, C, s)
                 : launch_scan_t<LabelT, float, MODE_BOUNDARY>(P, R, C, s);
}

hipError_t launch_face_scan(const ScanParams& P, const RecordBuf& R, Counters* C, hipStream_t s) {
    if (P.label_bits == 32) return launch_scan_l<uint32_t>(P, R, C, s);
    return launch_scan_l<uint64_t>(P, R, C, s);
}

template <typename LabelT>
__global__ __launch_bounds__(256) void k_density(const LabelT* __restrict__ L, int64_t Z, int64_t Y, int64_t X,
                                                 uint32_t* __restrict__ out) {
    const int64_t i = blockIdx.x;
    const int64_t z = (i * 7919) % Z, y = (i * 104729 + 17) % Y;
    const LabelT* row = L + (z * Y + y) * X;
    uint32_t ch = 0, pairs = 0;
    for (int64_t x = threadIdx.x; x + 1 < X; x += 256) {
        ch += row[x] != row[x + 1];
        ++pairs;
    }
    for (int o = 32; o > 0; o >>= 1) {
        ch += __shfl_xor(ch, o, 64);
        pairs += __shfl_xor(pairs, o, 64);
    }
    if ((threadIdx.x & 63) == 0) {
        atomicAdd(&out[0], ch);
        atomicAdd(&out[1], pairs);
    }
}

hipError_t launch_density(const void* L, int label_bits, const int64_t* shape, int n_rows, uint32_t* out,
                          hipStream_t s) {
    if (label_bits == 32)
        hipLaunchKernelGGL(k_density<uint32_t>, dim3(n_rows), dim3(256), 0, s, (const uint32_t*)L, shape[0], shape[1],
                           shape[2], out);
    else
        hipLaunchKernelGGL(k_density<uint64_t>, dim3(n_rows), dim3(256), 0, s, (const uint64_t*)L, shape[0], shape[1],
                           shape[2], out);
    return hipGetLastError();
}

int64_t scan_max_x() { return SCALAR_LOAD_SPAN / (8 * (std::max(ROWS_WIDE, ROWS_NARROW) + 1)); }
int scan_tile_rows() { return WG_ROWS; }
int scan_tile_rows_narrow() { return ROWS_NARROW * WAVES; }

constexpr int USET_CAP = 2048;

template <typename LabelT, typename KeptT>
struct UniqueSet {
    using Key = uint64_t;
    static constexpr Key EMPTY = EMPTY_KEY;
    static constexpr int CAP = USET_CAP;
    static constexpr bool SET = true, HOLES = false;
    const LabelT* __restrict__ L;
    uint64_t tag;
    uint64_t* keys;
    uint64_t* __restrict__ out;
    unsigned long long* count;
    __device__ Key load(int64_t p, bool in) const { return in ? (tag | (KeptT)L[p]) : EMPTY_KEY; }
    __device__ bool valid(Key, bool in) const { return in; }
    __device__ Key key(Key k) const { return k; }
    __device__ uint32_t overflow(Key) const { return 0u; }
    __device__ NoFold fold(Key, bool, uint64_t, int) const { return {}; }
    __device__ int head(uint32_t, int, int, int, NoFold) const { return 0; }
    __device__ void add(uint32_t, int) const {}
    __device__ void put_flush(uint64_t slot, int, Key key, const TileBox&) const { out[slot] = key; }
    __device__ void clear(int e) const { keys[e] = EMPTY; }
};

__global__ __launch_bounds__(TT_THREADS) void k_unique_tiles(const uint64_t* L, int64_t Y, int64_t X,
                                                              int64_t bz, int64_t by, int64_t bx,
                                                              int64_t ez, int64_t ey, int64_t ex,
                                                              uint64_t* out, unsigned long long* count,
                                                              int64_t cap) {
    __shared__ uint64_t set[USET_CAP];
    const UniqueSet<uint64_t, uint64_t> pol{L, 0ull, set, out, count};
    tile_table_scan(pol, tile_of_grid(Y, X, bz, by, bx, ez, ey, ex), cap);
}

template <typename LabelT>
__global__ __launch_bounds__(TT_THREADS) void k_unique_blocks(const LabelT* __restrict__ L,
                                                               const BlockGeom* __restrict__ blocks,
                                                               const uint32_t* __restrict__ tile_prefix,
                                                               int n_blocks, uint64_t* __restrict__ out,
                                                               unsigned long long* count, int64_t cap) {
    __shared__ uint64_t set[USET_CAP];
    uint32_t t = blockIdx.x;
    int lo = 0, hi = n_blocks;
    while (hi - lo > 1) {
        const int mid = (lo + hi) >> 1;
        if (tile_prefix[mid] <= t) lo = mid;
        else hi = mid;
    }
    const BlockGeom& G = blocks[lo];
    t -= tile_prefix[lo];
    const int bz = G.own_begin[0], by = G.own_begin[1], bx = G.own_begin[2];
    const int ez = G.own_end[0], ey = G.own_end[1], ex = G.own_end[2];
    const uint32_t ntx = (uint32_t)(ex - bx + 63) / 64, nty = (uint32_t)(ey - by + TILE_Y - 1) / TILE_Y;
    const TileBox box{G.shape[1], G.shape[2], bx + (int64_t)(t % ntx) * WAVE,
                      by + (int64_t)((t / ntx) % nty) * TILE_Y, bz + (int64_t)(t / (ntx * nty)) * TT_TILE_Z,
                      ez, ey, ex};
    const UniqueSet<LabelT, uint32_t> pol{L + G.label_offset, (uint64_t)lo << 32, set, out, count};
    tile_table_scan(pol, box, cap);
}

hipError_t launch_unique_blocks(const void* L, int label_bits, const BlockGeom* blocks, const uint32_t* tile_prefix,
                                int n_blocks, int64_t n_tiles, uint64_t* out, unsigned long long* count, int64_t cap,
                                hipStream_t s) {
    if (n_tiles <= 0) return hipSuccess;
    if (label_bits == 32)
        hipLaunchKernelGGL(k_unique_blocks<uint32_t>, dim3((unsigned)n_tiles), dim3(TT_THREADS), 0, s,
                           (const uint32_t*)L, blocks, tile_prefix, n_blocks, out, count, cap);
    else
        hipLaunchKernelGGL(k_unique_blocks<uint64_t>, dim3((unsigned)n_tiles), dim3(TT_THREADS), 0, s,
                           (const uint64_t*)L, blocks, tile_prefix, n_blocks, out, count, cap);
    return hipGetLastError();
}

int unique_tile_y() { return TILE_Y; }

hipError_t launch_unique_tiles(const uint64_t* L, const int64_t* shape, const int64_t* b, const int64_t* e,
                               uint64_t* out, unsigned long long* count, int64_t cap, hipStream_t s) {
    dim3 grid((unsigned)((e[2] - b[2] + 63) / 64), (unsigned)((e[1] - b[1] + TILE_Y - 1) / TILE_Y),
              (unsigned)((e[0] - b[0] + 15) / 16));
    hipLaunchKernelGGL(k_unique_tiles, grid, dim3(TT_THREADS), 0, s, L, shape[1], shape[2], b[0], b[1], b[2],
                       e[0], e[1], e[2], out, count, cap);
    return hipGetLastError();
}

CTG_BOUNDS_TAKE(scan)

}
```

cluster_tools_amd/rag.py:

```python
from __future__ import annotations

import collections
import contextlib
import ctypes
import sys
import threading

import numpy as np

from . import _lib as L

N_FEATURES = L.CTG_N_FEATURES
NBINS = L.CTG_NBINS
WIDE_WORDS = L.CTG_WIDE_RECORD_WORDS
NSLOTS = NBINS + 2
MORPH_COLS = L.CTG_MORPH_COLS
MORPH_WORDS = 10
REGION_COLS = L.CTG_REGION_COLS
REGION_FEATURE_NAMES = ('count', 'mean', 'minimum', 'maximum')


def _region_form(form):
    try:
        return {'sums': L.CTG_REGION_SUMS, 'features': L.CTG_REGION_FEATURES}[form]
# ... 923 lines not shown
            raise ValueError('a threshold needs a float32 source, got %s (a label source takes label=)' % src.dtype)
        return src, L.CTG_EDT_SRC_GREATER, bits
    if kind != 'b':
        raise ValueError('a source without threshold or label must be uint8 or bool, got %s' % src.dtype)
    return src, L.CTG_EDT_SRC_NONZERO, bits


def _edt_pitch(pitch):
    if pitch is None:
        return None
    p = [float(v) for v in pitch]
    if len(p) != 3:
        raise ValueError('pitch must have 3 entries (z, y, x), got %d' % len(p))
    if not all(np.isfinite(v) and v > 0 for v in p):
        raise ValueError('every pitch must be finite and positive, got %r' % (tuple(p),))
    return p


def distance_transform(src, pitch=None, threshold=None, label=None, to_background=False, two_d=False, begin=None,
                       end=None, out=None, stream=None, squared=False):
    src, kind, bits = _edt_source(src, threshold, label)
    on_dev = _is_torch(src)
    shape = tuple(src.shape)
    if len(shape) != 3:
        raise ValueError('src must be 3-D, got shape %s' % (shape,))
    p = _edt_pitch(pitch)
    b, e, oshape = _box(shape, begin, end)
    out = _dense_out(out, oshape, on_dev, src, 'float64' if squared else 'float32', 'src')
    lib = L.load()
    L.init_device()
    info = (ctypes.c_uint64 * 4)()
    flags = (L.CTG_EDT_TO_BACKGROUND if to_background else 0) | (L.CTG_EDT_2D if two_d else 0) | \
        (L.CTG_EDT_OUT_D2 if squared else 0)
    rc = lib.ctg_distance_transform(_ptr(src), kind, bits, _shape_arr(shape), _shape_arr(b), _shape_arr(e),
                                    float(threshold or 0.0), int(label or 0),
                                    (ctypes.c_double * 3)(*p) if p is not None else None, flags, _ptr(out),
                                    _mem(on_dev), _stream(stream, on_dev), info)
    L.check(rc, 'ctg_distance_transform')
    return out, EdtInfo(int(info[0]), int(info[1]), int(info[2]),
                        float(np.array([info[3]], dtype=np.uint64).view(np.float64)[0]))


WsInfo = collections.namedtuple('WsInfo', 'max_id n_zero rounds n_dropped')
WS_MAX_VOXELS = 1 << 30


def seeded_watershed(hmap, seeds, size_filter=0, two_d=False, begin=None, end=None, out=None, stream=None):
    on_dev = _is_torch(hmap)
    if _is_torch(seeds) != on_dev:
        raise ValueError('hmap and seeds must both be numpy arrays or both CUDA tensors')
    if on_dev:
        import torch
        if not (hmap.is_cuda and hmap.is_contiguous()) or hmap.dtype != torch.float32:
            raise ValueError('hmap must be a contiguous float32 CUDA tensor')
        if not (seeds.is_cuda and seeds.is_contiguous()) or seeds.is_floating_point() or \
                seeds.dtype == torch.bool or seeds.element_size() not in (4, 8):
            raise ValueError('seeds must be a contiguous CUDA tensor of 32- or 64-bit integers')
        bits = seeds.element_size() * 8
    else:
        hmap = np.asarray(hmap)
        seeds = np.asarray(seeds)
        if hmap.dtype != np.float32:
            raise TypeError('hmap must be float32, got %s' % hmap.dtype)
        if seeds.dtype not in (np.uint32, np.int32, np.uint64, np.int64):
            raise TypeError('seeds must be 32- or 64-bit integers, got %s' % seeds.dtype)
        bits = seeds.dtype.itemsize * 8
    shape = tuple(hmap.shape)
    if len(shape) != 3:
        raise ValueError('hmap must be 3-D, got shape %s' % (shape,))
    if tuple(seeds.shape) != shape:
        raise ValueError('seeds shape %s != hmap shape %s' % (tuple(seeds.shape), shape))
    if not 0 <= int(size_filter) < 1 << 64:
        raise ValueError('size_filter must be a uint64 value, got %r' % (size_filter,))
    b, e, oshape = _box(shape, begin, end)
    if oshape[0] * oshape[1] * oshape[2] > WS_MAX_VOXELS:
        raise ValueError('a box holds at most 2^30 voxels, got %s' % (oshape,))
    in_place = out is seeds
    if in_place and (bits != 64 or oshape != shape):
        raise ValueError('out may be the seeds only where they are 64-bit and the box is the whole array')
    if not on_dev:
        if np.isnan(hmap[b[0]:e[0], b[1]:e[1], b[2]:e[2]]).any():
            raise ValueError('the heights of the box hold a NaN')
        hmap = np.ascontiguousarray(hmap)
        if in_place and not seeds.flags.c_contiguous:
            raise ValueError('seeds written in place must be contiguous')
        seeds = np.ascontiguousarray(seeds)
        if in_place:
            out = seeds
    out = _dense_out(out, oshape, on_dev, hmap, 'int64', 'hmap')
    lib = L.load()
    L.init_device()
    info = (ctypes.c_uint64 * 4)()
    rc = lib.ctg_seeded_watershed(_ptr(hmap), _ptr(seeds), bits, _shape_arr(shape), _shape_arr(b), _shape_arr(e),
                                  L.CTG_WS_2D if two_d else 0, int(size_filter), _ptr(out),
                                  _mem(on_dev), _stream(stream, on_dev), info)
    L.check(rc, 'ctg_seeded_watershed')
    return out, WsInfo(int(info[0]), int(info[1]), int(info[2]), int(info[3]))


def synth_volume(shape, cell=10, seed=0, z_offset=0, global_shape=None, label_offset=0, noise_amp=0.1,
                 with_boundary=True, device=None):
    import torch
    lib = L.load()
    dev = L.init_device(device)
    labels = torch.empty(tuple(shape), dtype=torch.int64, device='cuda:%d' % dev)
    bnd = torch.empty(tuple(shape), dtype=torch.float32, device='cuda:%d' % dev) if with_boundary else None
    rc = lib.ctg_synth_volume(_ptr(labels), _ptr(bnd), _shape_arr(shape), int(z_offset), _shape_arr(global_shape),
                              int(cell), int(seed), int(label_offset), float(noise_amp),
                              ctypes.c_void_p(torch.cuda.current_stream().cuda_stream))
    L.check(rc, 'ctg_synth_volume')
    return labels, bnd


def synth_affinities(boundary, offsets):
    import torch
    lib = L.load()
    off = _check_offsets(offsets)
    shape = tuple(boundary.shape)
    affs = torch.empty((off.shape[0],) + shape, dtype=torch.float32, device=boundary.device)
    rc = lib.ctg_synth_affinities(_ptr(boundary), _ptr(affs), _shape_arr(shape), off.shape[0],
                                  off.ctypes.data_as(ctypes.c_void_p),
                                  ctypes.c_void_p(torch.cuda.current_stream().cuda_stream))
    L.check(rc, 'ctg_synth_affinities')
    return affs


def trim_cache():
    L.init_device()
    L.check(L.load().ctg_trim(), 'ctg_trim')


def set_profiling(on=True):
    L.check(L.load().ctg_set_profiling(int(bool(on))), 'ctg_set_profiling')


def last_timings():
    buf = (ctypes.c_double * 8)()
    L.check(L.load().ctg_last_timings(buf, 8), 'ctg_last_timings')
    return dict(zip(['scan', 'pack', 'sort', 'segment', 'reduce', 'nodes', 'total', 'narrow'], list(buf)))


SORT_PATHS = ('bucket_keys', 'onesweep_keys', 'bucket_pairs', 'onesweep_pairs_wide', 'onesweep_pairs_default',
              'group')
SORT_DECLINES = ('none', 'n_range', 'key_bits', 'item_bits', 'low_bits', 'bucket_cap')


def last_sort():
    buf = (ctypes.c_int64 * L.CTG_SORT_WORDS)()
    L.check(L.load().ctg_last_sort(buf, L.CTG_SORT_WORDS), 'ctg_last_sort')
    v = list(buf)
    return dict(path=SORT_PATHS[v[0]] if v[0] >= 0 else None, packed=v[1], group_tried=v[2], group_done=v[3],
                group_decline=SORT_DECLINES[v[4]], group_shift=v[5], group_buckets=v[6], largest_bucket=v[7],
                ib=v[8], nb=v[9], ub=v[10], n=v[11])
```

include/ctg.h:

```cpp
#ifndef CTG_H_
#define CTG_H_

#include <stdint.h>

#ifdef __cplusplus
extern "C" {
#endif

#define CTG_OK 0
#define CTG_ERR_ARG -1
#define CTG_ERR_HIP -2
#define CTG_ERR_NOMEM -3
#define CTG_ERR_UNSUPPORTED -4
#define CTG_ERR_STALE -5

#define CTG_MEM_HOST 0
#define CTG_MEM_DEVICE 1

#define CTG_DATA_NONE 0
#define CTG_DATA_F32 1
#define CTG_DATA_U8 2

#define CTG_KEEP_STATS 1
#define CTG_NO_NODES 4
// ... 54 lines not shown
int ctg_mgpu_sample(const ctg_result* local, int64_t* meta, void* stream);
int ctg_mgpu_split(const ctg_result* local, const int64_t* meta_all, int world_size, int64_t* counts, void* stream);
int ctg_mgpu_pack(const ctg_result* local, const int64_t* counts_all, int world_size, int rank, int64_t* send,
                  void* stream);
int ctg_mgpu_merge(ctg_result* local, const int64_t* recv, const int64_t* counts_all, int world_size, int rank,
                   double hist_lo, double hist_hi, void* stream, ctg_result** out);

int ctg_merge_feature_rows(const uint64_t* ids, const double* rows, int64_t n, int64_t id_begin, int64_t id_end,
                           double* out, int mem, void* stream);

int ctg_unique_pairs(const uint64_t* pairs, int64_t n, int mem, void* stream, ctg_result** out);

int ctg_label_overlaps(const void* labels, int label_bits, const void* values, int value_bits,
                       const int64_t* shape, const int64_t* begin, const int64_t* end,
                       int with_ignore, uint64_t ignore_label, int mem, void* stream, ctg_result** out);

int ctg_merge_overlaps(const uint64_t* pairs, const uint64_t* counts, int64_t n, int mem, void* stream,
                       ctg_result** out);

int ctg_max_overlaps(const ctg_result* r, uint64_t label_begin, uint64_t label_end, uint64_t* out_labels,
                     uint64_t* out_counts, int mem, void* stream);

#define CTG_MORPH_COLS 11
int ctg_morphology(const void* labels, int label_bits, const int64_t* shape,
                   const int64_t* begin, const int64_t* end, const int64_t* origin,
                   int mem, void* stream, ctg_result** out);

int ctg_merge_morphology(const double* rows, int64_t n, int mem, void* stream, ctg_result** out);

int ctg_result_copy_moments(const ctg_result* r, uint64_t* dst, int mem);

int ctg_morphology_rows(const ctg_result* r, uint64_t label_begin, uint64_t label_end,
                        double* out, double* rows, int mem, void* stream);

#define CTG_REGION_COLS 5
#define CTG_REGION_SUMS 0
#define CTG_REGION_FEATURES 1
int ctg_region_features(const void* labels, int label_bits, const void* data, int data_kind,
                        const int64_t* shape, const int64_t* begin, const int64_t* end,
                        int has_ignore, uint64_t ignore_label, int mem, void* stream, ctg_result** out);

int ctg_merge_region_features(const double* rows, int64_t n, int mem, void* stream, ctg_result** out);

int ctg_region_rows(const ctg_result* r, uint64_t label_begin, uint64_t label_end, int form, double norm,
                    double* out, double* rows, int mem, void* stream);

int ctg_result_copy_region(const ctg_result* r, uint64_t* counts, double* sums, float* minmax, int mem);

#define CTG_ASSIGN_DENSE 0
#define CTG_ASSIGN_SPARSE 1
#define CTG_ERR_MISSING -6
typedef struct ctg_assignment ctg_assignment;
int ctg_assignment_dense(const uint64_t* table, int64_t n, int mem, void* stream, ctg_assignment** out);
int ctg_assignment_sparse(const uint64_t* keys, const uint64_t* values, int64_t n, int mem, void* stream,
                          ctg_assignment** out);
int ctg_assignment_info(const ctg_assignment* a, int64_t* n, uint64_t* max_value, int* kind);
void ctg_assignment_free(ctg_assignment* a);

int ctg_apply_assignment(const ctg_assignment* a, const void* labels, int label_bits, int64_t n,
                         const int64_t* seg_begin, const uint64_t* seg_offset, int64_t n_seg, int allow_missing,
                         uint64_t* out, uint64_t* seg_nonzero, uint64_t* missing, int mem, void* stream);

#define CTG_CC_GREATER 0
#define CTG_CC_LESS 1
#define CTG_CC_EQUAL 2
int ctg_threshold_components(const void* data, int data_kind, const void* mask, const int64_t* shape,
                             const int64_t* begin, const int64_t* end, float threshold, int mode, int normalize,
                             int connectivity, uint64_t* out, int mem, void* stream, uint64_t* n_components);
int ctg_merge_assignments(const uint64_t* pairs, int64_t n, uint64_t n_labels, uint64_t* table, int mem,
                          void* stream, uint64_t* max_id);

#define CTG_EDT_SRC_NONZERO 0
#define CTG_EDT_SRC_GREATER 1
#define CTG_EDT_SRC_EQUAL 2
#define CTG_EDT_TO_BACKGROUND 1
#define CTG_EDT_2D 2
#define CTG_EDT_OUT_D2 4
int ctg_distance_transform(const void* src, int src_kind, int src_bits, const int64_t* shape, const int64_t* begin,
                           const int64_t* end, double threshold, uint64_t label, const double* pitch, int flags,
                           void* out, int mem, void* stream, uint64_t* info);

#define CTG_WS_2D 1
int ctg_seeded_watershed(const float* hmap, const void* seeds, int seed_bits, const int64_t* shape,
                         const int64_t* begin, const int64_t* end, int flags, uint64_t size_filter, uint64_t* out,
                         int mem, void* stream, uint64_t* info);

int ctg_map_edge_ids(const uint64_t* global_edges, int64_t n_global,
                     const uint64_t* query, int64_t n_query, int64_t* out_ids,
                     int mem, void* stream);

int64_t ctg_result_num_edges(const ctg_result* r);
int64_t ctg_result_num_nodes(const ctg_result* r);
int ctg_result_copy_edges(const ctg_result* r, uint64_t* dst, int mem);
int ctg_result_copy_nodes(const ctg_result* r, uint64_t* dst, int mem);
int ctg_result_copy_features(const ctg_result* r, double* dst, int mem);
int ctg_result_copy_stats(const ctg_result* r, double* sums_dst, uint32_t* records_dst, int mem);
int ctg_result_copy_counts(const ctg_result* r, uint64_t* dst, int mem);
const uint64_t* ctg_result_device_edges(const ctg_result* r);
const double* ctg_result_device_features(const ctg_result* r);
int ctg_result_info(const ctg_result* r, int64_t* n_records, int64_t* n_direct);
void ctg_free(ctg_result* r);

int ctg_synth_volume(uint64_t* labels, float* boundary, const int64_t* shape,
                     int64_t z_offset, const int64_t* global_shape, int cell,
                     uint64_t seed, uint64_t label_offset, double noise_amp, void* stream);
int ctg_filter_conv_axis(const float* in, float* out, const int64_t* shape, int ndim, int axis, const float* taps,
                         int n_taps, void* stream);
int ctg_filter_combine(int op, const float* a, const float* b, const float* c, float* out, int64_t n, void* stream);
int ctg_sym_eigenvalues(const float* comps, int dim, int64_t n, float* out, void* stream);

int ctg_synth_affinities(const float* boundary, float* affs, const int64_t* shape,
                         int n_channels, const int32_t* offsets, void* stream);

#define CTG_IO_N5 0
#define CTG_IO_ZARR_DOT 1
#define CTG_IO_ZARR_SLASH 2
#define CTG_IO_RAW 0
#define CTG_IO_GZIP 1
#define CTG_IO_ZLIB 2
int ctg_io_read_box(const char* ds_path, int format, int dtype_size, int big_endian, int ndim, const int64_t* shape,
                    const int64_t* chunks, int compression, const int64_t* begin, const int64_t* end, void* out,
                    int n_threads, const void* fill_value);
int ctg_io_read_varlen(const char* ds_path, int dtype_size, int ndim, int64_t n_chunks, const int64_t* positions,
                       int compression, void** out, int64_t* n_out, int n_threads);
void ctg_io_free(void* p);
void ctg_io_cache_clear(void);
void ctg_io_cache_stats(int64_t* out);
void ctg_io_cache_drop(const char* chunk_path);
int ctg_io_write_chunks(const char* ds_path, int format, int dtype_size, int big_endian, int ndim, int64_t n_chunks,
                        const int64_t* positions, const int64_t* chunk_shapes, const void* const* data,
                        const int64_t* n_elements, int varlen, int compression, int level, int n_threads);

int ctg_trim(void);

int ctg_set_profiling(int on);
int ctg_last_timings(double* ms, int n);

#define CTG_SORT_PATH 0
#define CTG_SORT_PACKED 1
#define CTG_SORT_GROUP_TRIED 2
#define CTG_SORT_GROUP_DONE 3
#define CTG_SORT_GROUP_WHY 4
#define CTG_SORT_GROUP_SHIFT 5
#define CTG_SORT_GROUP_BUCKETS 6
#define CTG_SORT_GROUP_LARGEST 7
#define CTG_SORT_IB 8
#define CTG_SORT_NB 9
#define CTG_SORT_UB 10
#define CTG_SORT_N 11
#define CTG_SORT_WORDS 12
#define CTG_SORT_PATH_GROUP 5
int ctg_last_sort(int64_t* out, int n);

int ctg_diag_bounds(uint64_t* out);

#ifdef __cplusplus
}
#endif
#endif
```

Before: 295.6 Gvoxels/s.

## Specialize face-scan waves fully inside the owned region to skip bounds checks

Splits the face-scan kernel body into an interior specialization, used when a wave's x/y/z tile lies entirely inside the owned region and array bounds. That path drops the per-lane ownership ballots, row masks, clamping and readfirstlane work. It also replaces per-plane base-address multiplication with running pointers advanced each z plane. A scan report API counts interior versus total waves. The cost is a larger kernel from duplicated code via an include file, which may raise register pressure or instruction-cache footprint.

```diff
diff --git a/cluster_tools_amd/_lib.py b/cluster_tools_amd/_lib.py
--- a/cluster_tools_amd/_lib.py
+++ b/cluster_tools_amd/_lib.py
@@ -51,6 +51,7 @@
 CTG_IO_ZLIB = 2
 CTG_SORT_WORDS = 12
 CTG_SORT_PATH_GROUP = 5
+CTG_SCAN_WORDS = 4
 
 _lock = threading.Lock()
 _lib = None
@@ -152,6 +153,7 @@
     'ctg_set_profiling': (ctypes.c_int, [ctypes.c_int]),
     'ctg_last_timings': (ctypes.c_int, [c_dblp, ctypes.c_int]),
     'ctg_last_sort': (ctypes.c_int, [c_i64p, ctypes.c_int]),
+    'ctg_last_scan': (ctypes.c_int, [c_i64p, ctypes.c_int]),
     'ctg_diag_bounds': (ctypes.c_int, [c_vp]),
 }
 
diff --git a/cluster_tools_amd/csrc/ctg_api.hip b/cluster_tools_amd/csrc/ctg_api.hip
--- a/cluster_tools_amd/csrc/ctg_api.hip
+++ b/cluster_tools_amd/csrc/ctg_api.hip
@@ -218,6 +218,21 @@
     return CTG_OK;
 }
 
+int ctg_last_scan(int64_t* out, int n) {
+    if (!out || n < 0) {
+        set_error("ctg_last_scan: null buffer or negative count");
+        return CTG_ERR_ARG;
+    }
+    const ScanReport& r = ws(current_device()).last_scan;
+    int64_t v[CTG_SCAN_WORDS];
+    v[CTG_SCAN_WAVES] = r.waves[0];
+    v[CTG_SCAN_INTERIOR_WAVES] = r.interior[0];
+    v[CTG_SCAN_NARROW_WAVES] = r.waves[1];
+    v[CTG_SCAN_NARROW_INTERIOR_WAVES] = r.interior[1];
+    for (int i = 0; i < n && i < CTG_SCAN_WORDS; ++i) out[i] = v[i];
+    return CTG_OK;
+}
+
 int ctg_result_num_blocks(const ctg_result* r) { return r ? (int)std::max<size_t>(r->edge_off.size(), 1) - 1 : -1; }
 
 int ctg_result_block_offsets(const ctg_result* r, int64_t* edge_off, int64_t* node_off) {
diff --git a/cluster_tools_amd/csrc/ctg_api_scan.hip b/cluster_tools_amd/csrc/ctg_api_scan.hip
--- a/cluster_tools_amd/csrc/ctg_api_scan.hip
+++ b/cluster_tools_amd/csrc/ctg_api_scan.hip
@@ -15,6 +15,7 @@
     int narrow_rows = -1;
     bool skip_adj = true;
     bool nn3 = true;
+    bool interior = true;
     int ablate = 0;
 };
 
@@ -29,6 +30,7 @@
         if (const char* t = getenv("CTG_NARROW_ROWS")) sw.narrow_rows = atoi(t) ? 1 : 0;
     if (const char* t = getenv("CTG_SKIP_ADJ")) sw.skip_adj = atoi(t) != 0;
     if (const char* t = getenv("CTG_NN3")) sw.nn3 = t[0] != '0';
+    if (const char* t = getenv("CTG_SCAN_INTERIOR")) sw.interior = t[0] != '0';
 #ifdef CTG_DIAG
     if (const char* t = getenv("CTG_ABLATE")) sw.ablate = atoi(t);
 #endif
@@ -89,7 +91,7 @@
         CTG_CHECK(ensure_records(w, need, 0));
         CTG_CHECK(hipMemsetAsync(w.counters, 0, sizeof(Counters), s));
         ev.mark(0);
-        CTG_CHECK(launch_face_scan(PW, w.rec, w.counters, s));
+        CTG_CHECK(launch_face_scan(PW, w.rec, w.counters, s, &w.last_scan));
         ev.mark(1);
         CTG_CHECK(hipMemcpyAsync(w.counters_host, w.counters, sizeof(Counters), hipMemcpyDeviceToHost, s));
         CTG_CHECK(hipStreamSynchronize(s));
@@ -239,6 +241,7 @@
     if (sw.tile_z_narrow) P.tile_z_narrow = sw.tile_z_narrow;
     P.ablate = sw.ablate;
     P.tail_tiles = sw.tail_tiles;
+    P.interior = sw.interior;
 }
 
 static int density_probe(Workspace& w, ScanParams& P, int mode, hipStream_t s) {
@@ -532,6 +535,7 @@
     RegionPrefix pre{};
     bool overflow = false;
     const bool scanned = P.batch_tiles > 0;
+    if (!scanned) w.last_scan = ScanReport{};
     if (scanned && (rc = scan_records(w, P, plan.voxels, s, sw, ev, pre, &overflow, who)) != CTG_OK) return rc;
     if (overflow)
         return blocks_dense_reentry(dl, label_bits, dd, data_kind, n_channels, offsets, blocks, n_blocks, labels_len,
diff --git a/cluster_tools_amd/csrc/ctg_internal.h b/cluster_tools_amd/csrc/ctg_internal.h
--- a/cluster_tools_amd/csrc/ctg_internal.h
+++ b/cluster_tools_amd/csrc/ctg_internal.h
@@ -169,6 +169,7 @@
     int tail_tiles;
     int64_t main_tiles;
     int tail_z0, tile_z_tail;
+    int interior;
 };
 
 struct Counters {
@@ -256,6 +257,7 @@
     double last_ms[8] = {0};
     int64_t last_records = 0, last_direct = 0;
     SortReport last_sort;
+    ScanReport last_scan;
     int profiling = 0;
 };
 
@@ -290,7 +292,8 @@
     }
 };
 
-hipError_t launch_face_scan(const ScanParams& P, const RecordBuf& R, Counters* C, hipStream_t s);
+hipError_t launch_face_scan(const ScanParams& P, const RecordBuf& R, Counters* C, hipStream_t s,
+                            ScanReport* rep = nullptr);
 int64_t scan_max_x();
 int scan_tile_rows();
 int scan_tile_rows_narrow();
diff --git a/cluster_tools_amd/csrc/ctg_plan.h b/cluster_tools_amd/csrc/ctg_plan.h
--- a/cluster_tools_amd/csrc/ctg_plan.h
+++ b/cluster_tools_amd/csrc/ctg_plan.h
@@ -82,6 +82,43 @@
     if (!boundary_map || (V < (1ll << 28) && nr_switch < 0)) return 0;
     return nr_switch < 0 ? 2 : (nr_switch ? 1 : 0);
 }
+
+CTG_HD constexpr bool scan_axis_interior(int64_t n, int64_t ob, int64_t oe, int64_t a, int64_t b) {
+    return ob <= a && b < oe && b < n;
+}
+CTG_HD constexpr bool scan_wave_interior(const int64_t* shape, const int64_t* own_begin, const int64_t* own_end,
+                                         int64_t x0, int64_t yw, int64_t rows, int64_t z0, int64_t z1) {
+    return scan_axis_interior(shape[2], own_begin[2], own_end[2], x0, x0 + TILE_X) &&
+           scan_axis_interior(shape[1], own_begin[1], own_end[1], yw, yw + rows) &&
+           scan_axis_interior(shape[0], own_begin[0], own_end[0], z0, z1);
+}
+
+struct ScanTilePlan {
+    int64_t ntx, nty, rows, waves;
+    int64_t tile_z, main_layers, tail_z0, tile_z_tail, tail_layers;
+    constexpr int64_t n_waves() const { return ntx * nty * waves * (main_layers + tail_layers); }
+};
+inline int64_t scan_interior_waves(const int64_t* shape, const int64_t* own_begin, const int64_t* own_end,
+                                   const ScanTilePlan& t) {
+    int64_t nx = 0, ny = 0, nz = 0;
+    for (int64_t tx = 0; tx < t.ntx; ++tx)
+        nx += scan_axis_interior(shape[2], own_begin[2], own_end[2], tx * TILE_X, tx * TILE_X + TILE_X);
+    for (int64_t w = 0; w < t.nty * t.waves; ++w)
+        ny += scan_axis_interior(shape[1], own_begin[1], own_end[1], w * t.rows, w * t.rows + t.rows);
+    const int64_t zlim = std::min(shape[0], t.tail_z0);
+    for (int64_t tz = 0; tz < t.main_layers; ++tz)
+        nz += scan_axis_interior(shape[0], own_begin[0], own_end[0], tz * t.tile_z,
+                                 std::min(tz * t.tile_z + t.tile_z, zlim));
+    for (int64_t tz = 0; tz < t.tail_layers; ++tz)
+        nz += scan_axis_interior(shape[0], own_begin[0], own_end[0], t.tail_z0 + tz * t.tile_z_tail,
+                                 std::min(t.tail_z0 + tz * t.tile_z_tail + t.tile_z_tail, shape[0]));
+    return nx * ny * nz;
+}
+
+struct ScanReport {
+    int64_t waves[2] = {0, 0};
+    int64_t interior[2] = {0, 0};
+};
 
 struct BlockGeom {
     int64_t label_offset;
diff --git a/cluster_tools_amd/csrc/ctg_scan.hip b/cluster_tools_amd/csrc/ctg_scan.hip
--- a/cluster_tools_amd/csrc/ctg_scan.hip
+++ b/cluster_tools_amd/csrc/ctg_scan.hip
@@ -671,26 +671,20 @@
 #endif
     const uint32_t hi_mask = BATCH ? P.label_hi_mask : 0u;
     const bool inx = x < X;
-    const bool own_x_lo = x >= obx && x < oex;
-    const bool lane_xf = inx && x + 1 < X && x + 1 >= obx && x + 1 < oex;
-    const bool lane_yz = inx && own_x_lo;
+    bool lane_xf, lane_yz;
     const bool g_x_lo = batch && inx && x >= gbx && x < gex;
     const bool glane_xf = g_x_lo && x + 1 < gex;
     const bool glane_yz = g_x_lo;
-    const uint64_t m_xf = __builtin_amdgcn_ballot_w64(lane_xf), m_yz = __builtin_amdgcn_ballot_w64(lane_yz);
+    uint64_t m_xf, m_yz;
     const uint64_t m_gxf = __builtin_amdgcn_ballot_w64(glane_xf), m_gyz = __builtin_amdgcn_ballot_w64(glane_yz);
-    uint32_t row_x = 0, row_y = 0, grow_x = 0, grow_y = 0;
+    uint32_t row_x, row_y, grow_x = 0, grow_y = 0;
 #pragma unroll
     for (int r = 0; r < ROWS; ++r) {
         const int y = yw + r;
-        if (y < Y && y >= oby && y < oey) row_x |= 1u << r;
-        if (y + 1 < Y && y + 1 >= oby && y + 1 < oey) row_y |= 1u << r;
         if (batch && y < Y && y >= gby && y < gey) grow_x |= 1u << r;
         if (batch && y + 1 < gey && y >= gby) grow_y |= 1u << r;
     }
     if constexpr (scalar_loads(MODE)) {
-        row_x = (uint32_t)__builtin_amdgcn_readfirstlane((int)row_x);
-        row_y = (uint32_t)__builtin_amdgcn_readfirstlane((int)row_y);
         grow_x = (uint32_t)__builtin_amdgcn_readfirstlane((int)grow_x);
         grow_y = (uint32_t)__builtin_amdgcn_readfirstlane((int)grow_y);
     }
@@ -711,28 +705,75 @@
         if constexpr (BATCH) ovf |= (uint32_t)l & hi_mask;
         return (uint32_t)l;
     };
-    const int xcl = min(x, X - 1);
-    const int xhc = min(xh, X - 1);
+    int xcl, xhc;
     const int64_t csz = (int64_t)Z * sz;
-    const int ywc = min(yw, Y - 1);
-    const int rmaxc = Y - 1 - ywc;
-    const uint64_t lbase = scalar_loads(MODE) ? uniform64((uint64_t)(L + (int64_t)ywc * X)) : 0;
-    const uint64_t dbase = scalar_loads(MODE) && (BND || NN3)
-                               ? uniform64((uint64_t)(D + (NN3 ? (int64_t)P.nn_ch[2] * csz : 0) + (int64_t)ywc * X))
-                               : 0;
-    const uint64_t aybase = scalar_loads(MODE) && NN3 ? uniform64((uint64_t)(D + (int64_t)P.nn_ch[1] * csz + (int64_t)ywc * X)) : 0;
-    const uint64_t azbase = scalar_loads(MODE) && NN3 ? uniform64((uint64_t)(D + (int64_t)P.nn_ch[0] * csz + (int64_t)ywc * X)) : 0;
-    const uint32_t win = (uint32_t)__builtin_amdgcn_readfirstlane((min(ROWS, rmaxc) + 1) * X);
-    const uint32_t xh_el = (uint32_t)(min(min(lane, ROWS - 1), rmaxc) * X + xhc);
+    uint32_t win;
+    uint32_t xh_el;
     uint32_t rofs[ROWS + 1];
-#pragma unroll
-    for (int r = 0; r <= ROWS; ++r) rofs[r] = (uint32_t)__builtin_amdgcn_readfirstlane(min(r, rmaxc) * X);
+    constexpr bool RUNNING = scalar_loads(MODE) && !BATCH;
+    const uint64_t lstep = (uint64_t)sz * sizeof(LabelT), dstep = (uint64_t)sz * sizeof(DataT);
+    uint64_t lbase, dbase, aybase, azbase;
+    uint64_t lcur = 0, dcur = 0, aycur = 0, azcur = 0;
+    auto wave_geometry = [&](bool inner) {
+        if (inner) {
+            lane_xf = lane_yz = true;
+            m_xf = m_yz = ~0ull;
+            row_x = row_y = (1u << ROWS) - 1u;
+        } else {
+            const bool own_x_lo = x >= obx && x < oex;
+            lane_xf = inx && x + 1 < X && x + 1 >= obx && x + 1 < oex;
+            lane_yz = inx && own_x_lo;
+            m_xf = __builtin_amdgcn_ballot_w64(lane_xf);
+            m_yz = __builtin_amdgcn_ballot_w64(lane_yz);
+            row_x = row_y = 0;
+#pragma unroll
+            for (int r = 0; r < ROWS; ++r) {
+                const int y = yw + r;
+                if (y < Y && y >= oby && y < oey) row_x |= 1u << r;
+                if (y + 1 < Y && y + 1 >= oby && y + 1 < oey) row_y |= 1u << r;
+            }
+            if constexpr (scalar_loads(MODE)) {
+                row_x = (uint32_t)__builtin_amdgcn_readfirstlane((int)row_x);
+                row_y = (uint32_t)__builtin_amdgcn_readfirstlane((int)row_y);
+            }
+        }
+        xcl = inner ? x : min(x, X - 1);
+        xhc = inner ? xh : min(xh, X - 1);
+        const int ywc = inner ? yw : min(yw, Y - 1);
+        const int rmaxc = inner ? ROWS : Y - 1 - ywc;
+        lbase = scalar_loads(MODE) ? uniform64((uint64_t)(L + (int64_t)ywc * X)) : 0;
+        dbase = scalar_loads(MODE) && (BND || NN3)
+                    ? uniform64((uint64_t)(D + (NN3 ? (int64_t)P.nn_ch[2] * csz : 0) + (int64_t)ywc * X))
+                    : 0;
+        aybase = scalar_loads(MODE) && NN3 ? uniform64((uint64_t)(D + (int64_t)P.nn_ch[1] * csz + (int64_t)ywc * X)) : 0;
+        azbase = scalar_loads(MODE) && NN3 ? uniform64((uint64_t)(D + (int64_t)P.nn_ch[0] * csz + (int64_t)ywc * X)) : 0;
+        win = inner ? (uint32_t)((ROWS + 1) * X)
+                    : (uint32_t)__builtin_amdgcn_readfirstlane((min(ROWS, rmaxc) + 1) * X);
+        xh_el = (uint32_t)(min(min(lane, ROWS - 1), rmaxc) * X + xhc);
+#pragma unroll
+        for (int r = 0; r <= ROWS; ++r)
+            rofs[r] = inner ? (uint32_t)(r * X) : (uint32_t)__builtin_amdgcn_readfirstlane(min(r, rmaxc) * X);
+        if constexpr (RUNNING) {
+            lcur = lbase + (uint64_t)z0 * lstep;
+            dcur = dbase + (uint64_t)z0 * dstep;
+            aycur = aybase + (uint64_t)z0 * dstep;
+            azcur = azbase + (uint64_t)z0 * dstep;
+        }
+    };
+    auto next_plane = [&](bool step) {
+        lcur += step ? lstep : 0;
+        if constexpr (BND || NN3) dcur += step ? dstep : 0;
+        if constexpr (NN3) {
+            aycur += step ? dstep : 0;
+            azcur += step ? dstep : 0;
+        }
+    };
     auto load_plane = [&](int z, LabelT (&Lb)[ROWS + 1], float (&Db)[ROWS + 1], LabelT& XL, float& XD,
                           float (&Dyb)[ROWS + 1], float (&Dzb)[ROWS], bool with_z) {
         if constexpr (scalar_loads(MODE)) {
-            const uint64_t pz = (uint64_t)z * (uint64_t)sz;
-            const BufRsrc Lr = buf_rsrc(lbase + pz * sizeof(LabelT), win * (uint32_t)sizeof(LabelT));
-            const BufRsrc Dr = buf_rsrc(dbase + pz * sizeof(DataT), win * (uint32_t)sizeof(DataT));
+            const uint64_t pz = RUNNING ? 0 : (uint64_t)z * (uint64_t)sz;
+            const BufRsrc Lr = buf_rsrc(RUNNING ? lcur : lbase + pz * sizeof(LabelT), win * (uint32_t)sizeof(LabelT));
+            const BufRsrc Dr = buf_rsrc(RUNNING ? dcur : dbase + pz * sizeof(DataT), win * (uint32_t)sizeof(DataT));
             const uint32_t xl = (uint32_t)xcl * (uint32_t)sizeof(LabelT), xd = (uint32_t)xcl * (uint32_t)sizeof(DataT);
 #pragma unroll
             for (int r = 0; r <= ROWS; ++r) {
@@ -741,12 +782,12 @@
                 else Db[r] = 0.f;
             }
             if constexpr (NN3) {
-                const BufRsrc Yr = buf_rsrc(aybase + pz * sizeof(DataT), win * (uint32_t)sizeof(DataT));
+                const BufRsrc Yr = buf_rsrc(RUNNING ? aycur : aybase + pz * sizeof(DataT), win * (uint32_t)sizeof(DataT));
 #pragma unroll
                 for (int r = 1; r <= ROWS; ++r)
                     Dyb[r] = buf_val<DataT, true>(Yr, xd, rofs[r] * (uint32_t)sizeof(DataT));
                 if (with_z) {
-                    const BufRsrc Zr = buf_rsrc(azbase + pz * sizeof(DataT), win * (uint32_t)sizeof(DataT));
+                    const BufRsrc Zr = buf_rsrc(RUNNING ? azcur : azbase + pz * sizeof(DataT), win * (uint32_t)sizeof(DataT));
 #pragma unroll
                     for (int r = 0; r < ROWS; ++r)
                         Dzb[r] = buf_val<DataT, true>(Zr, xd, rofs[r] * (uint32_t)sizeof(DataT));
@@ -848,191 +889,17 @@
         push_m(__builtin_amdgcn_ballot_w64(c_) & (lanes), c_ && (member), __VA_ARGS__); \
     } while (0)
 
-    if (z0 < z1) {
-        load_plane(z0, Ln, Dc, XLn, XDc, Dyc, Dzn, false);
-#pragma unroll
-        for (int r = 0; r <= ROWS; ++r) Lc[r] = narrow(Ln[r]);
-        XLc = narrow(XLn);
-    }
-    __builtin_amdgcn_s_waitcnt(0x0F70);
-    for (int z = z0; z < z1; ++z) {
-        const bool hz = z + 1 < Z;
-        load_plane(hz ? z + 1 : z, Ln, Dn, XLn, XDn, Dyn, Dzn, true);
-        const bool zlo = z >= obz && z < oez;
-        const bool zup = hz && z + 1 >= obz && z + 1 < oez;
-        const bool zg = batch && z >= gbz && z < gez;
-        const bool gzup = zg && z + 1 < gez;
-        const uint32_t s_xo = (uint32_t)__builtin_amdgcn_readfirstlane((int)(zlo ? row_x : 0u));
-        const uint32_t s_yo = (uint32_t)__builtin_amdgcn_readfirstlane((int)(zlo ? row_y : 0u));
-        const uint32_t s_zo = (uint32_t)__builtin_amdgcn_readfirstlane((int)(zup ? row_x : 0u));
-        const uint32_t s_xg = (uint32_t)__builtin_amdgcn_readfirstlane((int)(zg ? grow_x : 0u));
-        const uint32_t s_yg = (uint32_t)__builtin_amdgcn_readfirstlane((int)(zg ? grow_y : 0u));
-        const uint32_t s_zg = (uint32_t)__builtin_amdgcn_readfirstlane((int)(gzup ? grow_x : 0u));
-        if constexpr (MIX) {
-            const int rmax = Y - 1 - yw;
-            const DataT* Ax = D + (int64_t)P.nn_ch[2] * csz + (int64_t)z * sz + (int64_t)yw * X;
-            const DataT* Ay = D + (int64_t)P.nn_ch[1] * csz + (int64_t)z * sz + (int64_t)yw * X;
-#pragma unroll
-            for (int r = 0; r < ROWS; ++r) Dc[r] = load_val_stream<DataT>(Ax, (int64_t)min(r, rmax) * X + xcl);
-            XDc = load_val<DataT>(Ax, (int64_t)min(min(lane, ROWS - 1), rmax) * X + xhc);
-#pragma unroll
-            for (int r = 1; r <= ROWS; ++r) Dyc[r] = load_val_stream<DataT>(Ay, (int64_t)min(r, rmax) * X + xcl);
-        }
-        if (ablate & 8) {
-            uint32_t chk = 0;
-#pragma unroll
-            for (int r = 0; r < ROWS; ++r) chk ^= Lc[r] ^ (uint32_t)Ln[r] ^ __float_as_uint(Dc[r] + Dn[r]);
-            if (chk == 0x9E3779B9u && XLc == 7u) atomicAdd(&C->pad[0], 1ull);
+    if constexpr (scalar_loads(MODE) && !BATCH) {
+        if (P.interior && scan_wave_interior(P.shape, P.own_begin, P.own_end, x0, yw, ROWS, z0, z1)) {
+            constexpr bool INTERIOR = true;
+#include "ctg_scan_planes.inc"
         } else {
-#pragma unroll
-            for (int r = 0; r < ROWS; ++r) {
-                const uint32_t lc = Lc[r];
-                const uint32_t lx = shl1(lc, (uint32_t)__builtin_amdgcn_readlane((int)XLc, r));
-                const bool xo = (s_xo >> r) & 1u, xg = BATCH && ((s_xg >> r) & 1u);
-                if ((xo || xg) && (!AFF || adj_marks || NNF)) {
-                    const float dx = (BND || NNF) ? __uint_as_float(shl1(__float_as_uint(Dc[r]),
-                                                                         (uint32_t)__builtin_amdgcn_readlane(
-                                                                             (int)__float_as_uint(XDc), r)))
-                                                  : 0.f;
-                    const bool own = xo && lane_xf;
-                    if constexpr (NNF) {
-                        PUSH(lc != lx, m_xf, own, lc, lx, __float_as_uint(dx), NN_MARK);
-                    } else {
-                        PUSH(lc != lx, (xo ? m_xf : 0ull) | (xg ? m_gxf : 0ull), own || (xg && glane_xf), lc, lx,
-                             (own || !BATCH) ? __float_as_uint(Dc[r]) : MARK_ADJ,
-                             (AFF || (BATCH && !own)) ? MARK_ADJ : __float_as_uint(dx));
-                    }
-                }
-                const bool yo = (s_yo >> r) & 1u, yg = BATCH && ((s_yg >> r) & 1u);
-                if ((yo || yg) && (!AFF || adj_marks || NNF)) {
-                    const bool own = yo && lane_yz;
-                    if constexpr (NNF) {
-                        PUSH(lc != Lc[r + 1], m_yz, own, lc, Lc[r + 1], __float_as_uint(Dyc[r + 1]), NN_MARK);
-                    } else {
-                        PUSH(lc != Lc[r + 1], (yo ? m_yz : 0ull) | (yg ? m_gyz : 0ull), own || (yg && glane_yz), lc,
-                             Lc[r + 1],
-                             (own || !BATCH) ? __float_as_uint(Dc[r]) : MARK_ADJ,
-                             (AFF || (BATCH && !own)) ? MARK_ADJ : __float_as_uint(Dc[r + 1]));
-                    }
-                }
-            }
-            if constexpr (AFF) {
-                if (zlo && row_x) {
-                    const int64_t iz = (int64_t)z * sz + (int64_t)yw * X + x;
-                    const int n_loop = MIX ? P.n_loop : P.n_channels;
-                    for (int c0 = 0; c0 < n_loop; c0 += AFF_G) {
-                        constexpr int K = AFF_G * ROWS;
-                        uint32_t lq[K];
-                        float av[K];
-                        bool act[K];
-#pragma unroll
-                        for (int j = 0; j < AFF_G; ++j) {
-                            const bool has = c0 + j < n_loop;
-                            const int c = MIX ? (has ? P.loop_ch[c0 + j] : 0) : c0 + j;
-                            const int qz = has ? z + P.offsets[c][0] : -1, oy = has ? P.offsets[c][1] : 0;
-                            const int qx = has ? x + P.offsets[c][2] : -1;
-                            const bool okzx = lane_yz && qz >= 0 && qz < Z && qx >= 0 && qx < X;
-#pragma unroll
-                            for (int r = 0; r < ROWS; ++r) {
-                                const int k = j * ROWS + r;
-                                const int qy = yw + r + oy;
-                                act[k] = (row_x >> r & 1u) && okzx && qy >= 0 && qy < Y;
-                                lq[k] = Lc[r];
-                                av[k] = 0.f;
-                                if (act[k]) {
-                                    lq[k] = load_lo(L, (int64_t)qz * sz + (int64_t)qy * X + qx);
-                                    av[k] = load_val_stream<DataT>(D, (int64_t)c * Z * sz + iz + (int64_t)r * X);
-                                }
-                            }
-                        }
-#pragma unroll
-                        for (int k = 0; k < K; ++k) act[k] = act[k] && lq[k] != Lc[k % ROWS];
-                        const uint32_t glr = MIX ? (1u << AFF_G) - 1u : (P.lr_mask >> c0) & ((1u << AFF_G) - 1u);
-                        if (glr && P.bloom != nullptr && !(ablate & 512)) {
-                            uint64_t hb[K];
-                            unsigned long long wb[K];
-                            uint32_t blk[ROWS];
-#pragma unroll
-                            for (int r = 0; r < ROWS; ++r) blk[r] = bloom_block(Lc[r], P.bloom_mask);
-#pragma unroll
-                            for (int k = 0; k < K; ++k) {
-                                hb[k] = bloom_hash(((uint64_t)Lc[k % ROWS] << 32) | lq[k]);
-                                wb[k] = (act[k] && (glr >> (k / ROWS) & 1u)) ? P.bloom[bloom_word(blk[k % ROWS], hb[k])]
-                                                                             : ~0ull;
-                            }
-#pragma unroll
-                            for (int k = 0; k < K; ++k)
-                                act[k] = act[k] && (wb[k] & bloom_bits(hb[k])) == bloom_bits(hb[k]);
-                        }
-#pragma unroll
-                        for (int j = 0; j < AFF_G; ++j) {
-                            if (c0 + j >= n_loop) break;
-                            const uint32_t mk = (P.bloom != nullptr && !(glr >> j & 1u)) ? MARK_ONE_ADJ : MARK_ONE;
-                            if (mk == MARK_ONE && P.bloom != nullptr) {
-#pragma unroll
-                                for (int r = 0; r < ROWS; ++r) {
-                                    const int k = j * ROWS + r;
-                                    const uint32_t sv = __float_as_uint(av[k]);
-                                    const uint32_t nq = swap1(lq[k]), ns = swap1(sv), nact = swap1(act[k] ? 1u : 0u);
-                                    const bool pair = act[k] && nact && nq == lq[k] && ns < MARK_ONE_ADJ &&
-                                                      sv < MARK_ONE_ADJ;
-                                    const bool lead = (lane & 1) == 0;
-                                    const bool same_c = swap1(Lc[r]) == Lc[r];
-                                    const bool pr = pair && same_c;
-                                    PUSH(act[k] && !(pr && !lead), ~0ull, true, Lc[r], lq[k], sv,
-                                         (pr && lead) ? ns : MARK_ONE);
-                                }
-                            } else {
-#pragma unroll
-                                for (int r = 0; r < ROWS; ++r)
-                                    PUSH(act[j * ROWS + r], ~0ull, true, Lc[r], lq[j * ROWS + r],
-                                         __float_as_uint(av[j * ROWS + r]), mk);
-                            }
-                        }
-                    }
-                }
-            }
-            if constexpr (MIX) {
-                const int rmax = Y - 1 - yw;
-                const DataT* Az = D + (int64_t)P.nn_ch[0] * csz + (int64_t)(hz ? z + 1 : z) * sz + (int64_t)yw * X;
-#pragma unroll
-                for (int r = 0; r < ROWS; ++r) Dzn[r] = load_val_stream<DataT>(Az, (int64_t)min(r, rmax) * X + xcl);
-            }
-            if (stamps) {
-                const uint64_t tw = stamp_now();
-                __builtin_amdgcn_s_waitcnt(0x0F70);
-                t_wait += stamp_now() - tw;
-            }
-            if ((s_zo | s_zg) && (!AFF || adj_marks || NNF)) {
-#pragma unroll
-                for (int r = 0; r < ROWS; ++r) {
-                    const bool zo = (s_zo >> r) & 1u, zgr = BATCH && ((s_zg >> r) & 1u);
-                    if (zo || zgr) {
-                        const bool own = zo && lane_yz;
-                        const uint32_t ln = (uint32_t)Ln[r];
-                        if constexpr (NNF) {
-                            PUSH(Lc[r] != ln, m_yz, own, Lc[r], ln, __float_as_uint(Dzn[r]), NN_MARK);
-                        } else {
-                            PUSH(Lc[r] != ln, (zo ? m_yz : 0ull) | (zgr ? m_gyz : 0ull), own || (zgr && glane_yz),
-                                 Lc[r], ln, (own || !BATCH) ? __float_as_uint(Dc[r]) : MARK_ADJ,
-                                 (AFF || (BATCH && !own)) ? MARK_ADJ : __float_as_uint(Dn[r]));
-                        }
-                    }
-                }
-            }
-        }
-        poll();
-        __builtin_amdgcn_s_waitcnt(0x0F70);
-#pragma unroll
-        for (int r = 0; r <= ROWS; ++r) {
-            Lc[r] = narrow(Ln[r]);
-            Dc[r] = Dn[r];
-            if constexpr (NN3) {
-                if (r >= 1) Dyc[r] = Dyn[r];
-            }
-        }
-        XLc = narrow(XLn);
-        XDc = XDn;
+            constexpr bool INTERIOR = false;
+#include "ctg_scan_planes.inc"
+        }
+    } else {
+        constexpr bool INTERIOR = false;
+#include "ctg_scan_planes.inc"
     }
 #undef PUSH
     if (__ballot(ovf != 0) && lane == 0) atomicAdd(&C->label_overflow, 1ull);
@@ -1071,7 +938,8 @@
 }
 
 template <typename LabelT, typename DataT, int MODE, int NR>
-static hipError_t launch_scan_r(const ScanParams& P, const RecordBuf& R, Counters* C, hipStream_t s) {
+static hipError_t launch_scan_r(const ScanParams& P, const RecordBuf& R, Counters* C, hipStream_t s,
+                                ScanReport* rep) {
     ScanParams Q = P;
     int64_t nwg = P.batch_tiles;
     if (!P.blocks) {
@@ -1096,6 +964,14 @@
                 nwg = Q.main_tiles + layer * ((P.shape[0] - zt0 + tzt - 1) / tzt);
             }
         }
+        if (rep && layer > 0) {
+            const ScanTilePlan tp{Q.ntiles[0], Q.ntiles[1], NR, WAVES, Q.tile_z, Q.main_tiles / layer,
+                                  Q.tail_z0, Q.tile_z_tail, (nwg - Q.main_tiles) / layer};
+            const int width = NR == ROWS_NARROW && ROWS_NARROW != ROWS_WIDE ? 1 : 0;
+            rep->waves[width] = tp.n_waves();
+            rep->interior[width] =
+                scalar_loads(MODE) && P.interior ? scan_interior_waves(P.shape, P.own_begin, P.own_end, tp) : 0;
+        }
     } else {
         Q.main_tiles = nwg;
     }
@@ -1122,40 +998,44 @@
 }
 
 template <typename LabelT, typename DataT, int MODE>
-static hipError_t launch_scan_t(const ScanParams& P, const RecordBuf& R, Counters* C, hipStream_t s) {
+static hipError_t launch_scan_t(const ScanParams& P, const RecordBuf& R, Counters* C, hipStream_t s,
+                                ScanReport* rep) {
     if constexpr (MODE == MODE_BOUNDARY) {
         if (P.narrow_rows == 2 && !P.blocks) {
-            const hipError_t e = launch_scan_r<LabelT, DataT, MODE, ROWS_WIDE>(P, R, C, s);
-            return e != hipSuccess ? e : launch_scan_r<LabelT, DataT, MODE, ROWS_NARROW>(P, R, C, s);
-        }
-        if (P.narrow_rows == 1 && !P.blocks) return launch_scan_r<LabelT, DataT, MODE, ROWS_NARROW>(P, R, C, s);
+            const hipError_t e = launch_scan_r<LabelT, DataT, MODE, ROWS_WIDE>(P, R, C, s, rep);
+            return e != hipSuccess ? e : launch_scan_r<LabelT, DataT, MODE, ROWS_NARROW>(P, R, C, s, rep);
+        }
+        if (P.narrow_rows == 1 && !P.blocks)
+            return launch_scan_r<LabelT, DataT, MODE, ROWS_NARROW>(P, R, C, s, rep);
     }
     if constexpr (MODE == MODE_AFFINITY || MODE == MODE_AFF_MIX)
-        if (!P.blocks) return launch_scan_r<LabelT, DataT, MODE, ROWS_AFF>(P, R, C, s);
-    return launch_scan_r<LabelT, DataT, MODE, ROWS_WIDE>(P, R, C, s);
+        if (!P.blocks) return launch_scan_r<LabelT, DataT, MODE, ROWS_AFF>(P, R, C, s, rep);
+    return launch_scan_r<LabelT, DataT, MODE, ROWS_WIDE>(P, R, C, s, rep);
 }
 
 template <typename LabelT>
-static hipError_t launch_scan_l(const ScanParams& P, const RecordBuf& R, Counters* C, hipStream_t s) {
+static hipError_t launch_scan_l(const ScanParams& P, const RecordBuf& R, Counters* C, hipStream_t s,
+                                ScanReport* rep) {
     if (P.data_kind == CTG_DATA_NONE || P.data == nullptr)
-        return launch_scan_t<LabelT, float, MODE_GRAPH>(P, R, C, s);
+        return launch_scan_t<LabelT, float, MODE_GRAPH>(P, R, C, s, rep);
     const bool aff = P.n_channels > 0;
     const bool nn3 = aff && P.nn3 && !P.blocks;
     const bool mix = aff && P.nn_mix && !P.blocks;
     if (P.data_kind == CTG_DATA_U8)
-        return nn3 ? launch_scan_t<LabelT, uint8_t, MODE_AFF_NN>(P, R, C, s)
-               : mix ? launch_scan_t<LabelT, uint8_t, MODE_AFF_MIX>(P, R, C, s)
-               : aff ? launch_scan_t<LabelT, uint8_t, MODE_AFFINITY>(P, R, C, s)
-                     : launch_scan_t<LabelT, uint8_t, MODE_BOUNDARY>(P, R, C, s);
-    return nn3 ? launch_scan_t<LabelT, float, MODE_AFF_NN>(P, R, C, s)
-           : mix ? launch_scan_t<LabelT, float, MODE_AFF_MIX>(P, R, C, s)
-           : aff ? launch_scan_t<LabelT, float, MODE_AFFINITY>(P, R, C, s)
-                 : launch_scan_t<LabelT, float, MODE_BOUNDARY>(P, R, C, s);
-}
-
-hipError_t launch_face_scan(const ScanParams& P, const RecordBuf& R, Counters* C, hipStream_t s) {
-    if (P.label_bits == 32) return launch_scan_l<uint32_t>(P, R, C, s);
-    return launch_scan_l<uint64_t>(P, R, C, s);
+        return nn3 ? launch_scan_t<LabelT, uint8_t, MODE_AFF_NN>(P, R, C, s, rep)
+               : mix ? launch_scan_t<LabelT, uint8_t, MODE_AFF_MIX>(P, R, C, s, rep)
+               : aff ? launch_scan_t<LabelT, uint8_t, MODE_AFFINITY>(P, R, C, s, rep)
+                     : launch_scan_t<LabelT, uint8_t, MODE_BOUNDARY>(P, R, C, s, rep);
+    return nn3 ? launch_scan_t<LabelT, float, MODE_AFF_NN>(P, R, C, s, rep)
+           : mix ? launch_scan_t<LabelT, float, MODE_AFF_MIX>(P, R, C, s, rep)
+           : aff ? launch_scan_t<LabelT, float, MODE_AFFINITY>(P, R, C, s, rep)
+                 : launch_scan_t<LabelT, float, MODE_BOUNDARY>(P, R, C, s, rep);
+}
+
+hipError_t launch_face_scan(const ScanParams& P, const RecordBuf& R, Counters* C, hipStream_t s, ScanReport* rep) {
+    if (rep) *rep = ScanReport{};
+    if (P.label_bits == 32) return launch_scan_l<uint32_t>(P, R, C, s, rep);
+    return launch_scan_l<uint64_t>(P, R, C, s, rep);
 }
 
 template <typename LabelT>
diff --git a/cluster_tools_amd/csrc/ctg_scan_planes.inc b/cluster_tools_amd/csrc/ctg_scan_planes.inc
--- /dev/null
+++ b/cluster_tools_amd/csrc/ctg_scan_planes.inc
@@ -0,0 +1,190 @@
+{
+    wave_geometry(INTERIOR);
+    if (z0 < z1) {
+        load_plane(z0, Ln, Dc, XLn, XDc, Dyc, Dzn, false);
+#pragma unroll
+        for (int r = 0; r <= ROWS; ++r) Lc[r] = narrow(Ln[r]);
+        XLc = narrow(XLn);
+    }
+    __builtin_amdgcn_s_waitcnt(0x0F70);
+    for (int z = z0; z < z1; ++z) {
+        const bool hz = INTERIOR || z + 1 < Z;
+        if constexpr (RUNNING) next_plane(hz);
+        load_plane(hz ? z + 1 : z, Ln, Dn, XLn, XDn, Dyn, Dzn, true);
+        const bool zlo = INTERIOR || (z >= obz && z < oez);
+        const bool zup = INTERIOR || (hz && z + 1 >= obz && z + 1 < oez);
+        const bool zg = batch && z >= gbz && z < gez;
+        const bool gzup = zg && z + 1 < gez;
+        const uint32_t s_xo = INTERIOR ? ~0u : (uint32_t)__builtin_amdgcn_readfirstlane((int)(zlo ? row_x : 0u));
+        const uint32_t s_yo = INTERIOR ? ~0u : (uint32_t)__builtin_amdgcn_readfirstlane((int)(zlo ? row_y : 0u));
+        const uint32_t s_zo = INTERIOR ? ~0u : (uint32_t)__builtin_amdgcn_readfirstlane((int)(zup ? row_x : 0u));
+        const uint32_t s_xg = (uint32_t)__builtin_amdgcn_readfirstlane((int)(zg ? grow_x : 0u));
+        const uint32_t s_yg = (uint32_t)__builtin_amdgcn_readfirstlane((int)(zg ? grow_y : 0u));
+        const uint32_t s_zg = (uint32_t)__builtin_amdgcn_readfirstlane((int)(gzup ? grow_x : 0u));
+        if constexpr (MIX) {
+            const int rmax = Y - 1 - yw;
+            const DataT* Ax = D + (int64_t)P.nn_ch[2] * csz + (int64_t)z * sz + (int64_t)yw * X;
+            const DataT* Ay = D + (int64_t)P.nn_ch[1] * csz + (int64_t)z * sz + (int64_t)yw * X;
+#pragma unroll
+            for (int r = 0; r < ROWS; ++r) Dc[r] = load_val_stream<DataT>(Ax, (int64_t)min(r, rmax) * X + xcl);
+            XDc = load_val<DataT>(Ax, (int64_t)min(min(lane, ROWS - 1), rmax) * X + xhc);
+#pragma unroll
+            for (int r = 1; r <= ROWS; ++r) Dyc[r] = load_val_stream<DataT>(Ay, (int64_t)min(r, rmax) * X + xcl);
+        }
+        if (ablate & 8) {
+            uint32_t chk = 0;
+#pragma unroll
+            for (int r = 0; r < ROWS; ++r) chk ^= Lc[r] ^ (uint32_t)Ln[r] ^ __float_as_uint(Dc[r] + Dn[r]);
+            if (chk == 0x9E3779B9u && XLc == 7u) atomicAdd(&C->pad[0], 1ull);
+        } else {
+#pragma unroll
+            for (int r = 0; r < ROWS; ++r) {
+                const uint32_t lc = Lc[r];
+                const uint32_t lx = shl1(lc, (uint32_t)__builtin_amdgcn_readlane((int)XLc, r));
+                const bool xo = (s_xo >> r) & 1u, xg = BATCH && ((s_xg >> r) & 1u);
+                if ((xo || xg) && (!AFF || adj_marks || NNF)) {
+                    const float dx = (BND || NNF) ? __uint_as_float(shl1(__float_as_uint(Dc[r]),
+                                                                         (uint32_t)__builtin_amdgcn_readlane(
+                                                                             (int)__float_as_uint(XDc), r)))
+                                                  : 0.f;
+                    const bool own = xo && lane_xf;
+                    if constexpr (NNF) {
+                        PUSH(lc != lx, m_xf, own, lc, lx, __float_as_uint(dx), NN_MARK);
+                    } else {
+                        PUSH(lc != lx, (xo ? m_xf : 0ull) | (xg ? m_gxf : 0ull), own || (xg && glane_xf), lc, lx,
+                             (own || !BATCH) ? __float_as_uint(Dc[r]) : MARK_ADJ,
+                             (AFF || (BATCH && !own)) ? MARK_ADJ : __float_as_uint(dx));
+                    }
+                }
+                const bool yo = (s_yo >> r) & 1u, yg = BATCH && ((s_yg >> r) & 1u);
+                if ((yo || yg) && (!AFF || adj_marks || NNF)) {
+                    const bool own = yo && lane_yz;
+                    if constexpr (NNF) {
+                        PUSH(lc != Lc[r + 1], m_yz, own, lc, Lc[r + 1], __float_as_uint(Dyc[r + 1]), NN_MARK);
+                    } else {
+                        PUSH(lc != Lc[r + 1], (yo ? m_yz : 0ull) | (yg ? m_gyz : 0ull), own || (yg && glane_yz), lc,
+                             Lc[r + 1],
+                             (own || !BATCH) ? __float_as_uint(Dc[r]) : MARK_ADJ,
+                             (AFF || (BATCH && !own)) ? MARK_ADJ : __float_as_uint(Dc[r + 1]));
+                    }
+                }
+            }
+            if constexpr (AFF) {
+                if (zlo && row_x) {
+                    const int64_t iz = (int64_t)z * sz + (int64_t)yw * X + x;
+                    const int n_loop = MIX ? P.n_loop : P.n_channels;
+                    for (int c0 = 0; c0 < n_loop; c0 += AFF_G) {
+                        constexpr int K = AFF_G * ROWS;
+                        uint32_t lq[K];
+                        float av[K];
+                        bool act[K];
+#pragma unroll
+                        for (int j = 0; j < AFF_G; ++j) {
+                            const bool has = c0 + j < n_loop;
+                            const int c = MIX ? (has ? P.loop_ch[c0 + j] : 0) : c0 + j;
+                            const int qz = has ? z + P.offsets[c][0] : -1, oy = has ? P.offsets[c][1] : 0;
+                            const int qx = has ? x + P.offsets[c][2] : -1;
+                            const bool okzx = lane_yz && qz >= 0 && qz < Z && qx >= 0 && qx < X;
+#pragma unroll
+                            for (int r = 0; r < ROWS; ++r) {
+                                const int k = j * ROWS + r;
+                                const int qy = yw + r + oy;
+                                act[k] = (row_x >> r & 1u) && okzx && qy >= 0 && qy < Y;
+                                lq[k] = Lc[r];
+                                av[k] = 0.f;
+                                if (act[k]) {
+                                    lq[k] = load_lo(L, (int64_t)qz * sz + (int64_t)qy * X + qx);
+                                    av[k] = load_val_stream<DataT>(D, (int64_t)c * Z * sz + iz + (int64_t)r * X);
+                                }
+                            }
+                        }
+#pragma unroll
+                        for (int k = 0; k < K; ++k) act[k] = act[k] && lq[k] != Lc[k % ROWS];
+                        const uint32_t glr = MIX ? (1u << AFF_G) - 1u : (P.lr_mask >> c0) & ((1u << AFF_G) - 1u);
+                        if (glr && P.bloom != nullptr && !(ablate & 512)) {
+                            uint64_t hb[K];
+                            unsigned long long wb[K];
+                            uint32_t blk[ROWS];
+#pragma unroll
+                            for (int r = 0; r < ROWS; ++r) blk[r] = bloom_block(Lc[r], P.bloom_mask);
+#pragma unroll
+                            for (int k = 0; k < K; ++k) {
+                                hb[k] = bloom_hash(((uint64_t)Lc[k % ROWS] << 32) | lq[k]);
+                                wb[k] = (act[k] && (glr >> (k / ROWS) & 1u)) ? P.bloom[bloom_word(blk[k % ROWS], hb[k])]
+                                                                             : ~0ull;
+                            }
+#pragma unroll
+                            for (int k = 0; k < K; ++k)
+                                act[k] = act[k] && (wb[k] & bloom_bits(hb[k])) == bloom_bits(hb[k]);
+                        }
+#pragma unroll
+                        for (int j = 0; j < AFF_G; ++j) {
+                            if (c0 + j >= n_loop) break;
+                            const uint32_t mk = (P.bloom != nullptr && !(glr >> j & 1u)) ? MARK_ONE_ADJ : MARK_ONE;
+                            if (mk == MARK_ONE && P.bloom != nullptr) {
+#pragma unroll
+                                for (int r = 0; r < ROWS; ++r) {
+                                    const int k = j * ROWS + r;
+                                    const uint32_t sv = __float_as_uint(av[k]);
+                                    const uint32_t nq = swap1(lq[k]), ns = swap1(sv), nact = swap1(act[k] ? 1u : 0u);
+                                    const bool pair = act[k] && nact && nq == lq[k] && ns < MARK_ONE_ADJ &&
+                                                      sv < MARK_ONE_ADJ;
+                                    const bool lead = (lane & 1) == 0;
+                                    const bool same_c = swap1(Lc[r]) == Lc[r];
+                                    const bool pr = pair && same_c;
+                                    PUSH(act[k] && !(pr && !lead), ~0ull, true, Lc[r], lq[k], sv,
+                                         (pr && lead) ? ns : MARK_ONE);
+                                }
+                            } else {
+#pragma unroll
+                                for (int r = 0; r < ROWS; ++r)
+                                    PUSH(act[j * ROWS + r], ~0ull, true, Lc[r], lq[j * ROWS + r],
+                                         __float_as_uint(av[j * ROWS + r]), mk);
+                            }
+                        }
+                    }
+                }
+            }
+            if constexpr (MIX) {
+                const int rmax = Y - 1 - yw;
+                const DataT* Az = D + (int64_t)P.nn_ch[0] * csz + (int64_t)(hz ? z + 1 : z) * sz + (int64_t)yw * X;
+#pragma unroll
+                for (int r = 0; r < ROWS; ++r) Dzn[r] = load_val_stream<DataT>(Az, (int64_t)min(r, rmax) * X + xcl);
+            }
+            if (stamps) {
+                const uint64_t tw = stamp_now();
+                __builtin_amdgcn_s_waitcnt(0x0F70);
+                t_wait += stamp_now() - tw;
+            }
+            if ((s_zo | s_zg) && (!AFF || adj_marks || NNF)) {
+#pragma unroll
+                for (int r = 0; r < ROWS; ++r) {
+                    const bool zo = (s_zo >> r) & 1u, zgr = BATCH && ((s_zg >> r) & 1u);
+                    if (zo || zgr) {
+                        const bool own = zo && lane_yz;
+                        const uint32_t ln = (uint32_t)Ln[r];
+                        if constexpr (NNF) {
+                            PUSH(Lc[r] != ln, m_yz, own, Lc[r], ln, __float_as_uint(Dzn[r]), NN_MARK);
+                        } else {
+                            PUSH(Lc[r] != ln, (zo ? m_yz : 0ull) | (zgr ? m_gyz : 0ull), own || (zgr && glane_yz),
+                                 Lc[r], ln, (own || !BATCH) ? __float_as_uint(Dc[r]) : MARK_ADJ,
+                                 (AFF || (BATCH && !own)) ? MARK_ADJ : __float_as_uint(Dn[r]));
+                        }
+                    }
+                }
+            }
+        }
+        poll();
+        __builtin_amdgcn_s_waitcnt(0x0F70);
+#pragma unroll
+        for (int r = 0; r <= ROWS; ++r) {
+            Lc[r] = narrow(Ln[r]);
+            Dc[r] = Dn[r];
+            if constexpr (NN3) {
+                if (r >= 1) Dyc[r] = Dyn[r];
+            }
+        }
+        XLc = narrow(XLn);
+        XDc = XDn;
+    }
+}
diff --git a/cluster_tools_amd/rag.py b/cluster_tools_amd/rag.py
--- a/cluster_tools_amd/rag.py
+++ b/cluster_tools_amd/rag.py
@@ -1099,3 +1099,9 @@
     return dict(path=SORT_PATHS[v[0]] if v[0] >= 0 else None, packed=v[1], group_tried=v[2], group_done=v[3],
                 group_decline=SORT_DECLINES[v[4]], group_shift=v[5], group_buckets=v[6], largest_bucket=v[7],
                 ib=v[8], nb=v[9], ub=v[10], n=v[11])
+
+
+def last_scan():
+    buf = (ctypes.c_int64 * L.CTG_SCAN_WORDS)()
+    L.check(L.load().ctg_last_scan(buf, L.CTG_SCAN_WORDS), 'ctg_last_scan')
+    return dict(zip(['waves', 'interior_waves', 'narrow_waves', 'narrow_interior_waves'], list(buf)))
diff --git a/include/ctg.h b/include/ctg.h
--- a/include/ctg.h
+++ b/include/ctg.h
@@ -230,6 +230,13 @@
 #define CTG_SORT_PATH_GROUP 5
 int ctg_last_sort(int64_t* out, int n);
 
+#define CTG_SCAN_WAVES 0
+#define CTG_SCAN_INTERIOR_WAVES 1
+#define CTG_SCAN_NARROW_WAVES 2
+#define CTG_SCAN_NARROW_INTERIOR_WAVES 3
+#define CTG_SCAN_WORDS 4
+int ctg_last_scan(int64_t* out, int n);
+
 int ctg_diag_bounds(uint64_t* out);
 
 #ifdef __cplusplus
```

New measurement: 308.6 Gvoxels/s (median of 6 runs). +4.4%, better.
